# mmaker/c-lwe-snarks

Hardware: AMD Instinct MI355X
Metric: snark_proofs_per_sec (higher is better)
Workload: dtype u32 limbs (704-bit integers mod 2^704) + AES-256 bytes; int8 digits on the matrix cores, int32 accumulation (exact)

## Files before the change

### c-lwe-snarks_amd/__init__.py

```python
from __future__ import annotations

import ctypes
import os
from dataclasses import dataclass

import numpy as np

_HERE = os.path.dirname(os.path.abspath(__file__))
LIB_PATH = os.environ.get("MFHIP_LIB") or os.path.join(_HERE, "libmfhip.so")
P = 0xFFFFFFFB


class MfhError(RuntimeError):
    pass


@dataclass(frozen=True)
class Params:

    n: int = 1470
    logq: int = 736
    d: int = 1 << 15
    m: int = 21845

    @property
    def L(self):
        return (self.logq + 63) // 64

    @property
    def K(self):
        return self.logq // 64

    @property
    def lanes(self):
        return (64 * self.K + 55) // 56

    @property
    def ctb(self):
        return self.logq // 8

    @property
    def ctr_ct(self):
        return self.ctb * self.n

    @property
    def ctr_s(self):
        return 0

    @property
    def ctr_as(self):
        return self.ctr_ct * self.d

    @property
    def ctr_bt(self):
        return 2 * self.ctr_ct * self.d

    @property
    def ctr_bv(self):
        return 2 * self.ctr_ct * self.d + self.ctr_ct

    @property
    def ct_limbs(self):
        return (self.n + 1) * self.L


DEBUG = Params(d=256, m=64)
DEFAULT = Params()


class _CParams(ctypes.Structure):
    _fields_ = [("n", ctypes.c_uint32), ("logq", ctypes.c_uint32), ("d", ctypes.c_uint32), ("m", ctypes.c_uint32)]


_lib = None

EXPORTS = [
    "mfh_ctx_create", "mfh_ctx_destroy", "mfh_set_stream", "mfh_sync", "mfh_scrub_staging", "mfh_last_error", "mfh_set_seed",
    "mfh_keystream", "mfh_sample_rows", "mfh_ct_add", "mfh_ct_mul_ui", "mfh_ct_addmul_ui", "mfh_eval_rows",
    "mfh_encrypt_rows", "mfh_decrypt", "mfh_ct_smudge", "mfh_ssp_upload", "mfh_witness_poly", "mfh_version",
    "mfh_workspace_bytes", "mfh_last_kernel_ms", "mfh_set_timing", "mfh_set_overlap", "mfh_eval_rows_multi", "mfh_prove_batch", "mfh_crs_mm_image_bytes", "mfh_crs_expand_mm", "mfh_crs_set_resident_mm", "mfh_witness_poly_multi", "mfh_witness_poly_mm", "mfh_poly_h_multi", "mfh_poly_mul", "mfh_poly_add", "mfh_poly_prepare_t",
    "mfh_ssp_prepare", "mfh_poly_h", "mfh_setup_messages", "mfh_setup", "mfh_setup_image", "mfh_crs_image_set_b", "mfh_prove",
    "mfh_prove_partial", "mfh_prove_finish", "mfh_ct_to_lanes", "mfh_ct_from_lanes", "mfh_lanes_per_value", "mfh_digest128", "mfh_timing_drain", "mfh_timing_busy_ms", "mfh_timing_work_rows", "mfh_set_batch_image", "mfh_set_batch_slabs", "mfh_set_expand_path", "mfh_set_encrypt_path", "mfh_set_batch_launch", "mfh_set_batch_bw", "mfh_set_mm_chunk_rows", "mfh_set_mm_pack", "mfh_set_poly_exact", "mfh_poly_exact_fallbacks", "mfh_poly_exact_points", "mfh_set_poly_exact_points", "mfh_set_mm_stream", "mfh_add_dotp", "mfh_set_encrypt_chunks", "mfh_set_witness_per", "mfh_set_eval_path", "mfh_set_decrypt_path", "mfh_decrypt_rows",
    "mfh_crs_mm_share_bytes", "mfh_crs_expand_mm_share", "mfh_crs_set_resident_mm_share", "mfh_batch_chain", "mfh_batch_witness_cols", "mfh_batch_chain_from_w", "mfh_witness_poly_mm_cols", "mfh_prove_batch_partial", "mfh_prove_batch_finish",
    "mfh_resident_row_bytes", "mfh_crs_expand", "mfh_eval_rows_resident", "mfh_crs_set_resident",
    "mfh_witness_lanes", "mfh_witness_from_lanes", "mfh_prove_partial_w", "mfh_verify",
    "mfh_ssp_set_prg", "mfh_ssp_prg_make_t", "mfh_ssp_prg_fill",
    "mfh_resident_share_rows", "mfh_crs_expand_share", "mfh_crs_set_resident_share", "mfh_crs_set_resident_prefix",
    "mfh_prove_batch_supergroup", "mfh_prove_batch_stream_wait", "mfh_set_mm_width",
    "mfh_setup_public", "mfh_prove_public", "mfh_prove_batch_public", "mfh_vk_derive", "mfh_verify_public",
    "mfh_ssp_from_rows", "mfh_ssp_set_rows", "mfh_ssp_rows_fill", "mfh_circuit_create", "mfh_circuit_destroy", "mfh_circuit_assign",
    "mfh_circuit_create_global", "mfh_circuit_create_ex", "mfh_circuit_create_out", "mfh_circuit_create_sum",
]


def load_library():
    global _lib
    if _lib is not None:
        return _lib
    if not os.path.exists(LIB_PATH):
        raise MfhError(f"{LIB_PATH} is missing: run `python -c 'import __graft_entry__ as g; g.build()'` "
                       "(hipcc --offload-arch=gfx950).  There is no CPU fallback.")
    lib = ctypes.CDLL(LIB_PATH)
    vp, u64, sz, i32, u32 = ctypes.c_void_p, ctypes.c_uint64, ctypes.c_size_t, ctypes.c_int, ctypes.c_uint32
    sig = {
        "mfh_ctx_create": (i32, [ctypes.POINTER(vp), i32, ctypes.POINTER(_CParams)]),
        "mfh_ctx_destroy": (None, [vp]),
        "mfh_set_stream": (i32, [vp, vp]),
        "mfh_sync": (i32, [vp]),
        "mfh_scrub_staging": (i32, [vp]),
        "mfh_last_error": (ctypes.c_char_p, [vp]),
        "mfh_set_seed": (i32, [vp, ctypes.c_char_p]),
        "mfh_keystream": (i32, [vp, u64, vp, sz]),
        "mfh_sample_rows": (i32, [vp, u64, sz, vp]),
        "mfh_ct_add": (i32, [vp, vp, vp, vp, sz]),
        "mfh_ct_mul_ui": (i32, [vp, vp, vp, u32, sz]),
        "mfh_ct_addmul_ui": (i32, [vp, vp, vp, u32, sz]),
        "mfh_eval_rows": (i32, [vp, u64, sz, vp, vp, vp, vp, vp, i32]),
        "mfh_encrypt_rows": (i32, [vp, u64, sz, vp, vp, vp, vp]),
        "mfh_decrypt": (i32, [vp, vp, vp, sz, vp]),
        "mfh_ct_smudge": (i32, [vp, vp, sz, ctypes.c_char_p, sz, ctypes.c_char_p]),
        "mfh_ssp_upload": (i32, [vp, vp, vp, sz, sz]),
        "mfh_witness_poly": (i32, [vp, vp, ctypes.c_char_p, u32, vp]),
        "mfh_version": (ctypes.c_char_p, []),
        "mfh_workspace_bytes": (sz, [vp]),
        "mfh_last_kernel_ms": (ctypes.c_float, [vp, ctypes.c_char_p]),
        "mfh_set_timing": (i32, [vp, i32]),
        "mfh_set_overlap": (i32, [vp, i32]),
        "mfh_eval_rows_multi": (i32, [vp, u64, sz, vp, vp, u32, u32, vp, i32]),
        "mfh_poly_h_multi": (i32, [vp, vp, vp, u32]),
        "mfh_witness_poly_mm": (i32, [vp, vp, u32, ctypes.c_char_p, sz, vp, vp]),
        "mfh_witness_poly_multi": (i32, [vp, vp, u32, ctypes.c_char_p, sz, vp, vp]),
        "mfh_crs_mm_image_bytes": (sz, [vp]),
        "mfh_crs_expand_mm": (i32, [vp, vp, vp]),
        "mfh_crs_set_resident_mm": (i32, [vp, vp]),
        "mfh_prove_batch": (i32, [vp, vp, vp, u32, ctypes.c_char_p, sz, vp, ctypes.c_char_p, sz, ctypes.c_char_p, vp]),
        "mfh_prove_batch_supergroup": (u32, [vp]),
        "mfh_set_mm_width": (i32, [vp, u32, i32]),
        "mfh_prove_batch_stream_wait": (i32, [vp, u32, vp]),
        "mfh_poly_mul": (i32, [vp, vp, sz, vp, sz, vp]),
        "mfh_poly_add": (i32, [vp, vp, vp, sz, vp]),
        "mfh_poly_prepare_t": (i32, [vp, vp]),
        "mfh_ssp_prepare": (i32, [vp, vp]),
        "mfh_poly_h": (i32, [vp, vp, vp]),
        "mfh_setup_messages": (i32, [vp, vp, u32, u32, u32, vp]),
        "mfh_setup": (i32, [vp, vp, u32, u32, u32, vp, vp, vp]),
        "mfh_setup_image": (i32, [vp, vp, u32, u32, u32, vp, vp, vp, vp]),
        "mfh_prove": (i32, [vp, vp, vp, ctypes.c_char_p, u32, ctypes.c_char_p, sz, ctypes.c_char_p, vp]),
        "mfh_prove_partial": (i32, [vp, vp, vp, ctypes.c_char_p, u32, u32, u32, vp]),
        "mfh_prove_finish": (i32, [vp, vp, ctypes.c_char_p, sz, ctypes.c_char_p]),
        "mfh_lanes_per_value": (u32, [vp]),
        "mfh_digest128": (i32, [vp, vp, sz, vp]),
        "mfh_ct_to_lanes": (i32, [vp, vp, sz, vp]),
        "mfh_ct_from_lanes": (i32, [vp, vp, sz, vp]),
        "mfh_add_dotp": (i32, [vp, vp, vp, vp, sz]),
        "mfh_crs_set_resident_prefix": (i32, [vp, vp, sz]),
        "mfh_resident_share_rows": (sz, [vp, u32, u32]),
        "mfh_crs_expand_share": (i32, [vp, vp, u32, u32, vp]),
        "mfh_crs_set_resident_share": (i32, [vp, vp, u32, u32]),
        "mfh_ssp_set_prg": (i32, [vp, u64, vp]),
        "mfh_ssp_prg_make_t": (i32, [vp, u64, ctypes.c_char_p, vp]),
        "mfh_ssp_prg_fill": (i32, [vp, u64, sz, sz, vp]),
        "mfh_verify": (i32, [vp, vp, u32, u32, u32, vp, vp, sz, vp]),
        "mfh_witness_lanes": (i32, [vp, vp, ctypes.c_char_p, u32, u32, vp]),
        "mfh_witness_from_lanes": (i32, [vp, vp, vp, u32, vp]),
        "mfh_prove_partial_w": (i32, [vp, vp, vp, ctypes.c_char_p, u32, u32, u32, vp, vp]),
        "mfh_resident_row_bytes": (sz, [vp]),
        "mfh_crs_expand": (i32, [vp, u64, sz, vp, vp]),
        "mfh_crs_image_set_b": (i32, [vp, sz, sz, vp, vp]),
        "mfh_eval_rows_resident": (i32, [vp, vp, sz, sz, vp, vp, vp, vp, i32]),
        "mfh_crs_set_resident": (i32, [vp, vp]),
        "mfh_timing_drain": (i32, [vp, ctypes.c_char_p, ctypes.POINTER(u64), ctypes.POINTER(ctypes.c_double), ctypes.POINTER(u64),
                                   ctypes.POINTER(ctypes.c_float)]),
        "mfh_timing_busy_ms": (ctypes.c_double, [vp]),
        "mfh_timing_work_rows": (u64, [vp]),
        "mfh_set_batch_image": (i32, [vp, i32]),
        "mfh_set_mm_chunk_rows": (i32, [vp, u32]),
        "mfh_set_mm_pack": (i32, [vp, i32]),
        "mfh_set_poly_exact": (i32, [vp, i32]),
        "mfh_poly_exact_fallbacks": (ctypes.c_long, [vp]),
        "mfh_poly_exact_points": (i32, [vp, ctypes.POINTER(u32)]),
        "mfh_set_poly_exact_points": (i32, [vp, ctypes.POINTER(u32)]),
        "mfh_set_mm_stream": (i32, [vp, i32, i32, i32, u32]),
        "mfh_set_batch_launch": (i32, [vp, u32, i32]),
        "mfh_set_batch_bw": (i32, [vp, i32]),
        "mfh_set_encrypt_path": (i32, [vp, i32]),
        "mfh_set_expand_path": (i32, [vp, i32]),
        "mfh_set_batch_slabs": (i32, [vp, u32]),
        "mfh_set_encrypt_chunks": (i32, [vp, u32]),
        "mfh_set_eval_path": (i32, [vp, i32]),
        "mfh_set_decrypt_path": (i32, [vp, i32]),
        "mfh_decrypt_rows": (i32, [vp, u64, sz, vp, vp, vp]),
        "mfh_set_witness_per": (i32, [vp, u32]),
        "mfh_crs_mm_share_bytes": (sz, [vp, u32, u32]),
        "mfh_crs_expand_mm_share": (i32, [vp, vp, u32, u32, vp]),
        "mfh_crs_set_resident_mm_share": (i32, [vp, vp, u32, u32]),
        "mfh_batch_chain": (i32, [vp, vp, u32, ctypes.c_char_p, sz, vp, vp, vp, vp]),
        "mfh_batch_witness_cols": (i32, [vp, vp, u32, ctypes.c_char_p, sz, vp, u32, u32, vp, sz]),
        "mfh_batch_chain_from_w": (i32, [vp, vp, u32, vp, vp, vp]),
        "mfh_witness_poly_mm_cols": (i32, [vp, vp, u32, ctypes.c_char_p, sz, vp, u32, u32, vp, sz]),
        "mfh_prove_batch_partial": (i32, [vp, vp, u32, u32, u32, ctypes.c_char_p, sz, vp, vp, vp, sz, vp]),
        "mfh_prove_batch_finish": (i32, [vp, vp, u32, vp, ctypes.c_char_p, sz, ctypes.c_char_p, vp]),
        "mfh_setup_public": (i32, [vp, vp, u32, u32, u32, u32, vp, vp, vp, vp]),
        "mfh_prove_public": (i32, [vp, vp, vp, u32, ctypes.c_char_p, u32, ctypes.c_char_p, sz, ctypes.c_char_p, vp]),
        "mfh_prove_batch_public": (i32, [vp, vp, vp, u32, u32, ctypes.c_char_p, sz, vp, ctypes.c_char_p, sz, ctypes.c_char_p, vp]),
        "mfh_vk_derive": (i32, [vp, vp, u32, u32, vp]),
        "mfh_verify_public": (i32, [vp, vp, u32, u32, u32, vp, vp, ctypes.c_char_p, sz, sz, vp]),
        "mfh_ssp_from_rows": (i32, [vp, u32, vp, vp, vp, vp]),
        "mfh_ssp_set_rows": (i32, [vp, u32, vp, vp, vp, u32]),
        "mfh_ssp_rows_fill": (i32, [vp, sz, sz, vp]),
        "mfh_circuit_create": (i32, [vp, u32, u32, vp, u32, vp, ctypes.POINTER(vp)]),
        "mfh_circuit_create_global": (i32, [vp, u32, u32, vp, u32, vp, ctypes.POINTER(vp)]),
        "mfh_circuit_create_ex": (i32, [vp, u32, u32, vp, u32, vp, u32, vp, u32, ctypes.POINTER(vp)]),
        "mfh_circuit_create_out": (i32, [vp, u32, u32, vp, u32, vp, u32, vp, u32, vp, u32, ctypes.POINTER(vp)]),
        "mfh_circuit_create_sum": (i32, [vp, u32, u32, vp, u32, vp, u32, vp, u32, vp, u32, vp, u32, ctypes.POINTER(vp)]),
        "mfh_circuit_destroy": (None, [vp]),
        "mfh_circuit_assign": (i32, [vp, vp, u32, vp, sz, vp, sz, vp]),
    }
    for name, (res, args) in sig.items():
        fn = getattr(lib, name)
        fn.restype = res
        fn.argtypes = args
    _lib = lib
    return lib


def rows_to_csr(rows):
    if isinstance(rows, tuple) and len(rows) == 3 and all(isinstance(a, np.ndarray) for a in rows):
        row_ptr, wire, coef = rows
    else:
        lens = [len(r) for r in rows]
        row_ptr = np.zeros(len(lens) + 1, dtype=np.int64)
        np.cumsum(lens, out=row_ptr[1:])
        flat = [(int(w), int(a) % P) for r in rows for (w, a) in r]
        wire = np.array([w for w, _ in flat], dtype=np.int64)
        coef = np.array([a for _, a in flat], dtype=np.int64)
    if len(row_ptr) == 0 or min(np.min(row_ptr), np.min(wire, initial=0), np.min(coef, initial=0)) < 0:
        raise MfhError("rows: row_ptr needs nrows + 1 entries, and no entry may be negative")
    if max(np.max(row_ptr), np.max(wire, initial=0), np.max(coef, initial=0)) > 0xFFFFFFFF:
        raise MfhError("rows: entries must fit 32 bits")
    return tuple(np.ascontiguousarray(a, dtype=np.uint32) for a in (row_ptr, wire, coef))


def _ptr(t):
    return ctypes.c_void_p(t.data_ptr()) if t is not None else ctypes.c_void_p(0)


CIRCUIT_MAX_WIRES = 32767
CIRCUIT_GLOBAL = 1


class CircuitProgram:

    def __init__(self, ctx, nin, ngates, handle, state="lds", extended=False, outputs=0, sums=False):
        self._ctx, self.nin, self.ngates, self._h, self.state, self.extended, self.outputs = ctx, nin, ngates, handle, state, extended, outputs
        self.sums = sums

    def close(self):
        if self._h:
            self._ctx.lib.mfh_circuit_destroy(self._h)
            self._h = ctypes.c_void_p()

    def __del__(self):
        try:
            self.close()
        except Exception:
            pass


class Context:

    def __init__(self, params: Params = DEFAULT, device: int = 0):
        import torch

        if not torch.cuda.is_available():
            raise MfhError("no HIP device visible: the MI355X path has no CPU fallback")
        self.torch = torch
        self.lib = load_library()
        self.params = params
        self.device = torch.device("cuda", device)
        self._h = ctypes.c_void_p()
        cp = _CParams(params.n, params.logq, params.d, params.m)
        rc = self.lib.mfh_ctx_create(ctypes.byref(self._h), device, ctypes.byref(cp))
        if rc != 0:
            raise MfhError(f"mfh_ctx_create failed ({rc})")
        self._chk(self.lib.mfh_set_stream(self._h, ctypes.c_void_p(torch.cuda.current_stream(self.device).cuda_stream)))

    def close(self):
        if self._h:
            self.lib.mfh_ctx_destroy(self._h)
            self._h = ctypes.c_void_p()

    def __del__(self):
        try:
            self.close()
        except Exception:
            pass

    def _chk(self, rc):
        if rc != 0:
            raise MfhError(f"libmfhip error {rc}: {self.lib.mfh_last_error(self._h).decode()}")

    def empty(self, nbytes):
        return self.torch.empty(int(nbytes), dtype=self.torch.uint8, device=self.device)

    def zeros(self, nbytes):
        return self.torch.zeros(int(nbytes), dtype=self.torch.uint8, device=self.device)

    def to_device(self, arr):
        a = np.ascontiguousarray(arr)
        if not a.flags.writeable:
            import warnings

            with warnings.catch_warnings():
                warnings.simplefilter("ignore", UserWarning)
                return self.torch.from_numpy(a.view(np.uint8).reshape(-1)).to(self.device)
        return self.torch.from_numpy(a.view(np.uint8).reshape(-1)).to(self.device)

    def to_host(self, t, dtype=np.uint8):
        return t.cpu().numpy().view(dtype)

    def sync(self):
        self._chk(self.lib.mfh_sync(self._h))

    def set_timing(self, on=True):
        self._chk(self.lib.mfh_set_timing(self._h, 1 if on else 0))

    def set_overlap(self, mode=1):
        self._chk(self.lib.mfh_set_overlap(self._h, int(mode)))

    def set_batch_image(self, on=True):
        self._chk(self.lib.mfh_set_batch_image(self._h, 1 if on else 0))

    def set_batch_slabs(self, nslabs=0):
        self._chk(self.lib.mfh_set_batch_slabs(self._h, int(nslabs)))

    def set_expand_path(self, path=0):
        self._chk(self.lib.mfh_set_expand_path(self._h, int(path)))

    def set_encrypt_path(self, path=0):
        self._chk(self.lib.mfh_set_encrypt_path(self._h, int(path)))

    def set_eval_path(self, path=0):
        self._chk(self.lib.mfh_set_eval_path(self._h, int(path)))

    def set_encrypt_chunks(self, chunks=0):
        self._chk(self.lib.mfh_set_encrypt_chunks(self._h, int(chunks)))

    def set_witness_per(self, statements=0):
        self._chk(self.lib.mfh_set_witness_per(self._h, int(statements)))

    def set_batch_launch(self, groups_per_launch=4, merge_regions=True):
        self._chk(self.lib.mfh_set_batch_launch(self._h, int(groups_per_launch), 1 if merge_regions else 0))

    def set_batch_bw(self, merged=True):
        self._chk(self.lib.mfh_set_batch_bw(self._h, 1 if merged else 0))

    def set_mm_stream(self, map=0, persistent=False, sync_mode=0, spin_max=64):
        self._chk(self.lib.mfh_set_mm_stream(self._h, int(map), int(persistent), int(sync_mode), int(spin_max)))

    def set_mm_width(self, per_xcd=32, early_chain=False):
        self._chk(self.lib.mfh_set_mm_width(self._h, int(per_xcd), 1 if early_chain else 0))

    def set_mm_pack(self, on=True):
        self._chk(self.lib.mfh_set_mm_pack(self._h, 1 if on else 0))

    def set_poly_exact(self, mode=1):
        self._chk(self.lib.mfh_set_poly_exact(self._h, int(mode)))

    def poly_exact_fallbacks(self):
        return int(self.lib.mfh_poly_exact_fallbacks(self._h))

    def exact_points(self):
        out = (ctypes.c_uint32 * 4)()
        self._chk(self.lib.mfh_poly_exact_points(self._h, out))
        return [int(x) for x in out]

    def set_exact_points(self, pts):
        if pts is None:
            self._chk(self.lib.mfh_set_poly_exact_points(self._h, None))
            return
        pts = [int(x) for x in pts]
        if len(pts) != 4 or not all(0 <= x < 2**32 for x in pts):
            raise MfhError(f"set_exact_points: four uint32 values, got {pts!r}")
        self._chk(self.lib.mfh_set_poly_exact_points(self._h, (ctypes.c_uint32 * 4)(*pts)))

    def set_mm_chunk_rows(self, rows=0):
        self._chk(self.lib.mfh_set_mm_chunk_rows(self._h, int(rows)))

    def timing_drain(self, which):
        n, rows, ms, last = ctypes.c_uint64(), ctypes.c_uint64(), ctypes.c_double(), ctypes.c_float()
        self._chk(self.lib.mfh_timing_drain(self._h, which.encode(), ctypes.byref(n), ctypes.byref(ms), ctypes.byref(rows), ctypes.byref(last)))
        return n.value, ms.value, rows.value

    def timing_busy_ms(self):
        return float(self.lib.mfh_timing_busy_ms(self._h))

    def timing_work_rows(self):
        return int(self.lib.mfh_timing_work_rows(self._h))

    def last_kernel_ms(self, which):
        return float(self.lib.mfh_last_kernel_ms(self._h, which.encode()))

    def set_seed(self, seed: bytes):
        assert len(seed) == 40
        self._chk(self.lib.mfh_set_seed(self._h, bytes(seed)))

    def keystream(self, off, nbytes, out=None):
        out = self.empty(nbytes) if out is None else out
        self._chk(self.lib.mfh_keystream(self._h, off, _ptr(out), nbytes))
        return out

    def sample_rows(self, off, nrows):
        p = self.params
        out = self.empty(nrows * p.n * p.L * 8)
        self._chk(self.lib.mfh_sample_rows(self._h, off, nrows, _ptr(out)))
        return out

    def ct_add(self, a, b, count=1, out=None):
        out = self.empty(a.numel()) if out is None else out
        self._chk(self.lib.mfh_ct_add(self._h, _ptr(out), _ptr(a), _ptr(b), count))
        return out

    def ct_mul_ui(self, a, x, count=1, out=None):
        out = self.empty(a.numel()) if out is None else out
        self._chk(self.lib.mfh_ct_mul_ui(self._h, _ptr(out), _ptr(a), x, count))
        return out

    def ct_addmul_ui(self, rop, a, x, count=1):
        self._chk(self.lib.mfh_ct_addmul_ui(self._h, _ptr(rop), _ptr(a), x, count))
        return rop

    def eval_rows(self, off, nrows, c8, coeff0, coeff1=None, rop0=None, rop1=None, accumulate=False):
        p = self.params
        if rop0 is None:
            rop0 = self.empty(p.ct_limbs * 8)
        if coeff1 is not None and rop1 is None:
            rop1 = self.empty(p.ct_limbs * 8)
        self._chk(self.lib.mfh_eval_rows(self._h, off, nrows, _ptr(c8), _ptr(coeff0), _ptr(coeff1), _ptr(rop0), _ptr(rop1),
                                         1 if accumulate else 0))
        return rop0, rop1

    def eval_rows_multi(self, off, nrows, c8, coeffs, nvec, out=None, accumulate=False, coeff_bytes=4):
        out = self.empty(nvec * self.params.ct_limbs * 8) if out is None else out
        self._chk(self.lib.mfh_eval_rows_multi(self._h, off, nrows, _ptr(c8), _ptr(coeffs), nvec, coeff_bytes, _ptr(out), 1 if accumulate else 0))
        return out

    def encrypt_rows(self, off, nrows, sk, msg, err, out=None):
        p = self.params
        out = self.empty(nrows * p.ctb) if out is None else out
        self._chk(self.lib.mfh_encrypt_rows(self._h, off, nrows, _ptr(sk), _ptr(msg), _ptr(err), _ptr(out)))
        return out

    def decrypt(self, sk, cts, count, out=None):
        out = self.empty(4 * count) if out is None else out
        self._chk(self.lib.mfh_decrypt(self._h, _ptr(sk), _ptr(cts), count, _ptr(out)))
        return out

    def set_decrypt_path(self, path=0):
        self._chk(self.lib.mfh_set_decrypt_path(self._h, int(path)))

    def decrypt_rows(self, off, nrows, sk, c8, out=None):
        out = self.empty(4 * nrows) if out is None else out
        self._chk(self.lib.mfh_decrypt_rows(self._h, off, nrows, _ptr(sk), _ptr(c8), _ptr(out)))
        return out

    def ct_smudge(self, cts, count, mag: bytes, maglen, sign: bytes):
        self._chk(self.lib.mfh_ct_smudge(self._h, _ptr(cts), count, bytes(mag), maglen, bytes(sign)))
        return cts

    def ssp_upload(self, ssp_host_u64: np.ndarray, d_ssp=None, first_slot=0, nslots=None):
        p = self.params
        nslots = p.m + 3 if nslots is None else nslots
        if d_ssp is None:
            d_ssp = self.empty((p.m + 3) * p.d * 4)
        a = np.ascontiguousarray(ssp_host_u64)
        self._chk(self.lib.mfh_ssp_upload(self._h, ctypes.c_void_p(a.ctypes.data), _ptr(d_ssp), first_slot, nslots))
        return d_ssp

    def ssp_from_rows(self, rows, d_ssp=None):
        p = self.params
        row_ptr, wire, coef = rows_to_csr(rows)
        if d_ssp is None:
            d_ssp = self.empty((p.m + 3) * p.d * 4)
        self._chk(self.lib.mfh_ssp_from_rows(self._h, len(row_ptr) - 1, ctypes.c_void_p(row_ptr.ctypes.data), ctypes.c_void_p(wire.ctypes.data),
                                             ctypes.c_void_p(coef.ctypes.data), _ptr(d_ssp)))
        return d_ssp

    def ssp_set_rows(self, rows, lu_max=0):
        if rows is None:
            self._chk(self.lib.mfh_ssp_set_rows(self._h, 0, None, None, None, 0))
            return
        row_ptr, wire, coef = rows_to_csr(rows)
        self._chk(self.lib.mfh_ssp_set_rows(self._h, len(row_ptr) - 1, ctypes.c_void_p(row_ptr.ctypes.data), ctypes.c_void_p(wire.ctypes.data),
                                            ctypes.c_void_p(coef.ctypes.data), int(lu_max)))

    def ssp_rows_fill(self, first_slot, nslots):
        out = self.empty(max(nslots, 1) * self.params.d * 4)
        self._chk(self.lib.mfh_ssp_rows_fill(self._h, first_slot, nslots, _ptr(out)))
        return out

    def circuit_load(self, compiled, state="lds"):
        if state not in ("lds", "global", "auto"):
            raise MfhError(f"circuit_load: state must be 'lds', 'global' or 'auto', got {state!r}")
        gates = np.ascontiguousarray(compiled.gates, dtype=np.uint32).reshape(-1, 3)
        asserts = np.ascontiguousarray(compiled.asserts, dtype=np.uint32).reshape(-1, 2)
        program = np.ascontiguousarray(getattr(compiled, "program", np.zeros((0, 4))), dtype=np.uint32).reshape(-1, 4)
        equal = np.ascontiguousarray(getattr(compiled, "equal", np.zeros((0, 2))), dtype=np.uint32).reshape(-1, 2)
        outputs = np.ascontiguousarray(getattr(compiled, "outputs", np.zeros((0, 2))), dtype=np.uint32).reshape(-1, 2)
        terms = np.ascontiguousarray(getattr(compiled, "terms", np.zeros((0, 2))), dtype=np.uint32).reshape(-1, 2)
# ... 346 lines not shown
```

### c-lwe-snarks_amd/csrc/ctx.hpp

```cpp
#pragma once
#include <hip/hip_runtime.h>

#include <stdint.h>
#include <string.h>

#include <string>
#include <vector>

#include "aes_dev.hpp"
#include "mfhip.h"
#include "ssp_prg.hpp"

#define HIP_TRY(ctx, expr)                                                        \
  do {                                                                            \
    hipError_t e_ = (expr);                                                       \
    if (e_ != hipSuccess) {                                                       \
      (ctx)->err = std::string(#expr) + ": " + hipGetErrorString(e_);             \
      return MFH_EDEVICE;                                                         \
    }                                                                             \
  } while (0)

struct PolyState;
struct SspInterp;
struct SspRows;
struct RowsTree;

struct PinBuf {
  void *p = nullptr;
  size_t cap = 0;
  hipEvent_t ev = nullptr;
  bool pending = false;
  size_t used = 0;
};

struct DevBuf {
  void *p = nullptr;
  size_t cap = 0;
  template <class T> T *as() const { return static_cast<T *>(p); }
};

struct mfh_ctx {
  mfh_params P{};
  int device = 0;
  hipStream_t own_stream = nullptr;
  hipStream_t stream = nullptr;
  mf::AesKey key{};
  bool have_seed = false;
  uint32_t *d_t0 = nullptr;
  DevBuf ws;
  DevBuf ws2;
  int mm_ws_sel = 0;
  DevBuf ws3;
  std::vector<hipEvent_t> ev_cdone, ev_rdone, ev_wdone;
  std::vector<hipEvent_t> ev_round;
  std::vector<hipEvent_t> ev_sgdone;
  uint32_t last_batch_sg = 0, last_batch_n = 0;
  DevBuf wws;
  DevBuf lazy;
  uint32_t *lazy_cnt = nullptr;
  bool eval_dense = false;
  bool overlap = true;
  int overlap_mode = 1;
  hipStream_t side = nullptr, side2 = nullptr;
  hipEvent_t ev_fork = nullptr, ev_join = nullptr;
  hipEvent_t ev_chain = nullptr, ev_chain_done = nullptr;
  std::string err;
  bool timing = false;
  struct Timed {
    hipEvent_t e0, e1;
    int kind;
    uint64_t rows;
    uint64_t work;
    int sub;
  };
  std::vector<Timed> timed;
  double last_busy_ms = 0;
  uint64_t last_work_rows = 0;
  std::vector<hipEvent_t> ev_pool;
  PolyState *poly = nullptr;
  DevBuf aux;
  DevBuf d_msg;
  DevBuf d_prover;
  std::vector<uint32_t> h_cw;
  const uint8_t *mm_image = nullptr;
  uint32_t mm_rank = 0, mm_world = 1;
  uint64_t mm_off[3] = {0, 0, 0}, mm_rows[3] = {0, 0, 0};
  size_t mm_base[3] = {0, 0, 0};
  DevBuf ssp_frag;
  const uint32_t *ssp_frag_src = nullptr;
  SspInterp *interp = nullptr;
  DevBuf circ_io;
  DevBuf circ_state;
  DevBuf d_batch;
  DevBuf batch_img;
  int batch_image = 1;
  int mm_map = 1;
  bool mm_persist = true;
  bool mm_wave1 = false;
  uint32_t mm_sync_mode = 0, mm_spin = 64;
  uint32_t mm_width = 32;
  size_t early_ws_half = 0;
  bool batch_early_chain = false;
  uint32_t *mm_sync = nullptr;
  int poly_exact = 1;
  bool poly_pts_pinned = false;
  uint32_t poly_pts[4] = {0, 0, 0, 0};
  bool mm_pack = true;
  uint32_t mm_chunk_rows = 131071;
  int expand_path = 0;
  int enc_path = 0;
  uint32_t ncu = 256;
  int dec_path = 0;
  int eval_path = 0;
  uint32_t enc_chunks = 0;
  uint32_t witness_per = 0;
  uint32_t batch_slabs = 0;
  int batch_bw_merged = 1;
  int batch_merge = 1;
  uint32_t batch_ngl = 8;
  PinBuf pin_rows, pin_cw, pin_smudge;
  PinBuf pin_pub;
  DevBuf d_pub;
  PinBuf pin_wring[8];
  uint32_t pin_wnext = 0;
  hipEvent_t ev_sample = nullptr;
  DevBuf sample_tmp;
  void *uploader = nullptr;
  bool prg_on = false;
  uint64_t prg_seed = 0;
  const uint32_t *prg_t = nullptr;
  SspRows *rows = nullptr;
  RowsTree *rows_tree = nullptr;
  const uint32_t *rows_prefix = nullptr;
  uint32_t rows_lu_max = 0;
  const uint8_t *resident_rows = nullptr;
  uint64_t resident_nrows = ~0ull;
  bool resident_sharded = false;
  uint32_t res_rank = 0, res_world = 1;
};

struct Timer {
  mfh_ctx *c;
  mfh_ctx::Timed t{};
  bool on;
  Timer(mfh_ctx *c_, int kind, uint64_t rows, uint64_t work = 0, int sub = 0) : c(c_), on(c_->timing) {
    if (!on) return;
    auto get = [&]() {
      hipEvent_t e;
      if (!c->ev_pool.empty()) { e = c->ev_pool.back(); c->ev_pool.pop_back(); }
      else hipEventCreate(&e);
      return e;
    };
    t.e0 = get(); t.e1 = get(); t.kind = kind; t.rows = rows; t.work = work ? work : rows; t.sub = sub;
    hipEventRecord(t.e0, c->stream);
  }
  ~Timer() {
    if (!on) return;
    hipEventRecord(t.e1, c->stream);
    c->timed.push_back(t);
  }
};

inline void *pin_acquire(mfh_ctx *c, PinBuf &b, size_t bytes) {
  if (b.pending) { hipEventSynchronize(b.ev); b.pending = false; }
  if (bytes > b.cap) {
    if (b.p) hipHostFree(b.p);
    b.cap = (bytes + 4095) & ~(size_t)4095;
    if (hipHostMalloc(&b.p, b.cap, hipHostMallocDefault) != hipSuccess) { b.p = nullptr; b.cap = 0; c->err = "hipHostMalloc failed"; return nullptr; }
  }
  if (!b.ev) hipEventCreateWithFlags(&b.ev, hipEventDisableTiming);
  b.used = bytes;
  return b.p;
}
inline void pin_release(mfh_ctx *c, PinBuf &b) {
  hipEventRecord(b.ev, c->stream);
  b.pending = true;
}
inline void pin_scrub(PinBuf &b) {
  if (b.pending) { hipEventSynchronize(b.ev); b.pending = false; }
  if (b.p && b.used) {
    volatile unsigned char *q = (volatile unsigned char *)b.p;
    memset((void *)q, 0, b.used);
    __asm__ __volatile__("" : : "r"(b.p) : "memory");
  }
  b.used = 0;
}
inline void pin_free(PinBuf &b) {
  if (b.pending) hipEventSynchronize(b.ev);
  if (b.p) hipHostFree(b.p);
  if (b.ev) hipEventDestroy(b.ev);
  b = PinBuf();
}

enum class DevWait { stream, device };
inline void dev_free(DevBuf &b) {
  if (b.p) hipFree(b.p);
  b = DevBuf();
}
inline bool dev_alloc(DevBuf &b, size_t bytes) {
  if (hipMalloc(&b.p, bytes) != hipSuccess) {
    b = DevBuf();
    return false;
  }
  b.cap = bytes;
  return true;
}
inline int dev_reserve(mfh_ctx *c, DevBuf &b, size_t bytes, DevWait wait = DevWait::stream, size_t gran = 1) {
  if (bytes <= b.cap) return MFH_OK;
  if (b.p) {
    if (wait == DevWait::device) hipDeviceSynchronize();
    else hipStreamSynchronize(c->stream);
    dev_free(b);
  }
  if (!dev_alloc(b, (bytes + gran - 1) & ~(gran - 1))) {
    c->err = "hipMalloc(device scratch) failed";
    return MFH_ENOMEM;
  }
  return MFH_OK;
}
inline int batch_img_drop(mfh_ctx *c) {
  if (!c->batch_img.p) return MFH_OK;
  const hipError_t e = hipDeviceSynchronize();
  dev_free(c->batch_img);
  if (e != hipSuccess) {
    c->err = std::string("hipDeviceSynchronize(): ") + hipGetErrorString(e);
    return MFH_EDEVICE;
  }
  return MFH_OK;
}
inline int work_reserve(mfh_ctx *c, DevBuf &b, size_t bytes) { return dev_reserve(c, b, bytes, DevWait::stream, (size_t)1 << 20); }
inline int lazy_reserve(mfh_ctx *c, size_t bytes) {
  if (bytes + 256 <= c->lazy.cap || !bytes) return MFH_OK;
  bytes = ((bytes + 255) & ~(size_t)255) + 256;
  if (int rc = dev_reserve(c, c->lazy, bytes)) return rc;
  if (hipMemsetAsync(c->lazy.p, 0, bytes, c->stream) != hipSuccess) return MFH_EDEVICE;
  c->lazy_cnt = reinterpret_cast<uint32_t *>(c->lazy.as<uint8_t>() + bytes - 256);
  return MFH_OK;
}
inline int ws_reserve(mfh_ctx *c, size_t bytes) { return work_reserve(c, c->ws, bytes); }
inline int wws_reserve(mfh_ctx *c, size_t bytes) { return work_reserve(c, c->wws, bytes); }
inline int ws2_reserve(mfh_ctx *c, size_t bytes) { return work_reserve(c, c->ws2, bytes); }
inline int aux_reserve(mfh_ctx *c, size_t bytes) { return dev_reserve(c, c->aux, bytes); }

inline int ssp_src(mfh_ctx *c, const uint32_t *d_ssp, mf::SspSrc &src, bool rows_ok = false) {
  if (d_ssp) { src = mf::SspSrc{d_ssp, d_ssp, 0}; return MFH_OK; }
  if (c->rows_prefix) {
    if (!rows_ok) { c->err = "this entry point does not take the row SSP (mfh_ssp_set_rows): pass a dense d_ssp"; return MFH_EUNSUPPORTED; }
    src = mf::SspSrc{c->rows_prefix, c->rows_prefix, 0, c->rows_lu_max + 2};
    return MFH_OK;
  }
  if (!c->prg_on || !c->prg_t) { c->err = "d_ssp is NULL and no generator-defined SSP is registered (mfh_ssp_set_prg)"; return MFH_EINVAL; }
  src = mf::SspSrc{nullptr, c->prg_t, c->prg_seed};
  return MFH_OK;
}

void mfh_poly_destroy(mfh_ctx *c);
void ssp_interp_free(mfh_ctx *c);
void ssp_rows_free(mfh_ctx *c, bool tree);
int ssp_rows_check(mfh_ctx *c, const char *who, uint32_t nrows, const uint32_t *h_row_ptr, const uint32_t *h_wire, const uint32_t *h_coef);
int ssp_rows_tree(mfh_ctx *c, const char *who, const uint32_t *&d_t, const uint32_t *&h_w);
int ssp_rows_witness(mfh_ctx *c, uint32_t nstmt, const uint8_t *h_bits, size_t bits_stride, const uint32_t *h_delta, uint32_t *d_w, size_t w_stride);
int ssp_rows_msg_evals(mfh_ctx *c, uint32_t s, uint32_t beta, uint32_t *d_msg_evals);
inline bool ssp_is_rows(const mfh_ctx *c, const uint32_t *d_ssp) { return !d_ssp && c->rows_prefix; }
inline int ssp_rows_lu_check(mfh_ctx *c, const uint32_t *d_ssp, uint32_t lu) {
  if (ssp_is_rows(c, d_ssp) && lu > c->rows_lu_max) { c->err = "lu exceeds the lu_max the row SSP was registered with (mfh_ssp_set_rows)"; return MFH_EINVAL; }
  return MFH_OK;
}
extern "C" int mfh_witness_poly_mm(mfh_ctx *c, const uint32_t *d_ssp, uint32_t nstmt, const uint8_t *h_bits, size_t bits_stride, const uint32_t *h_delta,
                                   uint32_t *d_w);
extern "C" int mfh_witness_poly_mm_cols(mfh_ctx *c, const uint32_t *d_ssp, uint32_t nstmt, const uint8_t *h_bits, size_t bits_stride, const uint32_t *h_delta,
                                        uint32_t col0, uint32_t ncols, uint32_t *d_w, size_t w_stride);
extern "C" int mfh_poly_h_multi(mfh_ctx *c, const uint32_t *d_v, uint32_t *d_h, uint32_t nb);
int expand_mm_region(mfh_ctx *c, uint64_t off, uint32_t nrows, const uint8_t *c8, uint8_t *image);
int encrypt_rows_mm(mfh_ctx *c, uint64_t off, size_t nrows, const uint64_t *sk, const uint32_t *msg, const uint64_t *err, uint8_t *c8);
int decrypt_mm(mfh_ctx *c, const uint64_t *sk, const uint64_t *cts, size_t count, uint32_t *out);
int decrypt_rows_mm(mfh_ctx *c, uint64_t off, size_t nrows, const uint64_t *sk, const uint8_t *c8, uint32_t *out);

struct MmIo {
  const uint32_t *coef[2];
  uint32_t csplit;
  uint64_t *out[2];
  uint32_t osplit;
  uint64_t ostride;
  const uint8_t *bits;
  uint32_t bits_stride;
  int64_t *sc_zeroed;
  uint64_t cstride;
  uint32_t bits_row0;
  const uint64_t *add_ct;
  const uint32_t *add_scale;
  uint32_t sa_from1;
};
int eval_rows_multi_io(mfh_ctx *c, uint64_t off, size_t nrows, const uint8_t *d_c8, const MmIo &io, uint32_t nvec, uint32_t coeff_bytes, int accumulate);
int eval_rows_multi_io_set(mfh_ctx *c, uint64_t off, size_t nrows, const uint8_t *d_c8, const MmIo *ios, const uint32_t *nvecs, uint32_t ng,
                           uint32_t coeff_bytes);
struct MmRegion { uint64_t off; const uint8_t *c8; };
int eval_rows_multi_io_regions(mfh_ctx *c, const MmRegion *regs, uint32_t nreg, size_t nrows, const MmIo *ios, const uint32_t *nvecs, uint32_t ng,
                               uint32_t coeff_bytes, int accumulate);
bool mm_image_covers(const mfh_ctx *c, uint64_t off, size_t nrows);
struct MmsPlan {
  uint32_t ng, ngt, ND, nrows, nchunks, rpc, rpad, ntiles, mtiles;
  size_t cd_bytes, part_bytes;
  const uint8_t *img[2];
  int8_t *cd;
  int *part;
};
bool mms_plan(mfh_ctx *c, const MmRegion *regs, uint32_t nreg, size_t nrows, const MmIo *ios, const uint32_t *nvecs, uint32_t ng, uint32_t coeff_bytes,
              MmsPlan &P);
size_t mms_ws_bytes(const MmsPlan &P);
void mms_bind(MmsPlan &P, void *ws);
int mms_digits(mfh_ctx *c, const MmsPlan &P, const MmIo *ios, const uint32_t *nvecs);
int mms_stream(mfh_ctx *c, const MmsPlan &P);
int mms_finish(mfh_ctx *c, const MmsPlan &P, const MmIo *ios, const uint32_t *nvecs, int accumulate);
```

### c-lwe-snarks_amd/csrc/evalmm.hip

```cpp
#include <algorithm>
#include <cstring>

#include "ctx.hpp"

namespace {

using mf::AesKey;

constexpr int CT = 4;
constexpr int SB = 88;
constexpr int VB = 92;
constexpr int MB = CT * SB;
constexpr int MT = MB / 32;
constexpr int RT = 128;
constexpr int TSTRIDE = 384;
constexpr int BLK_PER_ROW = 24;
static_assert(MB % 32 == 0 && CT * VB + 15 <= TSTRIDE, "tile geometry");

typedef int v4i __attribute__((ext_vector_type(4)));
typedef int v16i __attribute__((ext_vector_type(16)));

__device__ __forceinline__ uint32_t coef_at(const MmIo &io, uint32_t v, uint32_t nrows, uint32_t i) {
  if (io.bits) {
    const uint32_t a = io.bits_row0 + i;
// ... 778 lines not shown
  for (uint32_t k = 0; k < nblk * nchunks; k++) {
    uint32_t grp, tg;
    mms_item(xcd, (k % nblk) * 32 + cu, ngt, ngr, map, grp, tg);
    mmstream_body_w(imgs, mtiles, KS, nrows, rows_per_chunk, cdv, part, grp, tg, k / nblk, cd_stride, part_stride);
  }
}

template <int ND, int KWM ,
          bool PK >
__device__ __forceinline__ void evalmm_finish_body(const int *__restrict__ part, const int64_t *__restrict__ sc, uint32_t nchunks, uint32_t ntiles, uint32_t N,
                                                   uint32_t nvec, uint32_t n, uint32_t nrows, uint32_t ct, uint32_t MBv, uint32_t sby, uint32_t LL,
                                                   const MmIo &io, int accumulate, const int *__restrict__ sa_part, uint32_t sa_col) {
  __shared__ uint32_t sv[KWM][3][64];
  const uint32_t vl = threadIdx.x & 63, lq = threadIdx.x >> 6;
  const uint32_t v = blockIdx.y * 64 + vl, j = blockIdx.x;
  const uint32_t tile = j / ct, jj = j % ct;
  const uint32_t KWv = sby / 4;
  if (v < nvec) {
    int64_t corr[ND];
#pragma unroll
    for (int w = 0; w < ND; w++) corr[w] = 128 * sc[ND * v + w] + 16384ll * nrows;
    if (PK) {
      const uint64_t M4 = (uint64_t)ntiles * MBv / 4;
      unsigned __int128 corrsum = 0;
#pragma unroll
      for (int w = 0; w < ND; w++) corrsum += (unsigned __int128)((uint64_t)corr[w] * 0x01010101ull) << (8 * w);
      for (uint32_t l = lq; l < KWv; l += 4) {
        const uint64_t m4 = ((uint64_t)tile * MBv + jj * sby) / 4 + l;
        __int128 U = 0, SA = 0;
        for (uint32_t ch = 0; ch < nchunks; ch++) {
          const uint64_t at = (uint64_t)ch * M4 + m4;
          if (ND == 4) {
            const uint4 r = reinterpret_cast<const uint4 *>(part)[at * (N / 4) + v], q = reinterpret_cast<const uint4 *>(sa_part)[at * (N / 4) + sa_col / 4];
            U += (__int128)(((unsigned __int128)(uint64_t)(int64_t)(int32_t)r.z << 64) | ((uint64_t)r.y << 32) | r.x);
            SA += (__int128)(((unsigned __int128)(uint64_t)(int64_t)(int32_t)q.z << 64) | ((uint64_t)q.y << 32) | q.x);
          } else {
            U += reinterpret_cast<const long long *>(part)[at * N + v];
            SA += reinterpret_cast<const long long *>(sa_part)[at * N + sa_col];
          }
        }
        const unsigned __int128 val = (unsigned __int128)(U + SA * (__int128)(ND == 4 ? 128ll * 0x01010101ll : 128ll)) + corrsum;
        sv[l][0][vl] = (uint32_t)val;
        sv[l][1][vl] = (uint32_t)(val >> 32);
        sv[l][2][vl] = (uint32_t)(val >> 64);
      }
    } else
    for (uint32_t l = lq; l < KWv; l += 4) {
      unsigned __int128 val = 0;
      int g0[4][ND], sa0[4];
#pragma unroll
      for (int k = 0; k < 4; k++) {
        const int *row = part + ((uint64_t)tile * MBv + (jj * sby + 4 * l + k)) * N;
#pragma unroll
        for (int w = 0; w < ND; w++) g0[k][w] = row[ND * v + w];
        sa0[k] = (sa_part + ((uint64_t)tile * MBv + (jj * sby + 4 * l + k)) * N)[sa_col];
      }
#pragma unroll
      for (int k = 0; k < 4; k++) {
        const uint32_t mm = jj * sby + 4 * l + k;
        int64_t g[ND], sa = sa0[k];
#pragma unroll
        for (int w = 0; w < ND; w++) g[w] = g0[k][w];
        for (uint32_t ch = 1; ch < nchunks; ch++) {
          const int *row = part + (((uint64_t)ch * ntiles + tile) * MBv + mm) * N;
#pragma unroll
          for (int w = 0; w < ND; w++) g[w] += row[ND * v + w];
          sa += (sa_part + (((uint64_t)ch * ntiles + tile) * MBv + mm) * N)[sa_col];
        }
        uint64_t t = 0;
#pragma unroll
        for (int w = 0; w < ND; w++) t += (uint64_t)(g[w] + 128 * sa + corr[w]) << (8 * w);
        val += (unsigned __int128)t << (8 * k);
      }
      sv[l][0][vl] = (uint32_t)val;
      sv[l][1][vl] = (uint32_t)(val >> 32);
      sv[l][2][vl] = (uint32_t)(val >> 64);
    }
  }
  __syncthreads();
  if (lq != 0 || v >= nvec) return;
  uint32_t *out = reinterpret_cast<uint32_t *>((v < io.osplit ? io.out[0] + (uint64_t)v * io.ostride : io.out[1] + (uint64_t)(v - io.osplit) * io.ostride) +
                                               (uint64_t)j * LL);
  const bool wide4 = (LL & 1) == 0 && (io.ostride & 1) == 0 && ((reinterpret_cast<uintptr_t>(io.out[0]) | reinterpret_cast<uintptr_t>(io.out[1])) & 15) == 0;
  uint32_t pend[4] = {0, 0, 0, 0};
  uint64_t carry = 0;
  const uint32_t *actw = io.add_ct ? reinterpret_cast<const uint32_t *>(io.add_ct + (uint64_t)j * LL) : nullptr;
  const uint64_t ax = io.add_ct ? io.add_scale[v] : 0;
  uint64_t acarry = 0;
  for (uint32_t l = 0; l < KWv; l++) {
    uint64_t word = carry + sv[l][0][vl];
    if (l >= 1) word += sv[l - 1][1][vl];
    if (l >= 2) word += sv[l - 2][2][vl];
    if (accumulate) word += out[l];
    if (actw) {
      const uint64_t t = (uint64_t)actw[l] * ax + acarry;
      word += (uint32_t)t;
      acarry = t >> 32;
    }
    carry = word >> 32;
    pend[l & 3] = (uint32_t)word;
    if (wide4 ? (l & 3) == 3 : (l & 1) == 1) {
      if (wide4) *reinterpret_cast<uint4 *>(out + (l & ~3u)) = uint4{pend[0], pend[1], pend[2], pend[3]};
      else *reinterpret_cast<uint2 *>(out + (l & ~1u)) = uint2{pend[(l & 2)], pend[(l & 2) + 1]};
    }
  }
  if (wide4) {
    if (KWv & 3) *reinterpret_cast<uint4 *>(out + (KWv & ~3u)) = uint4{pend[0], (KWv & 3) > 1 ? pend[1] : 0u, (KWv & 3) > 2 ? pend[2] : 0u, 0u};
    for (uint32_t l = (KWv + 3) & ~3u; l < 2 * LL; l += 4) *reinterpret_cast<uint4 *>(out + l) = uint4{0u, 0u, 0u, 0u};
  } else {
    if (KWv & 1) *reinterpret_cast<uint2 *>(out + (KWv & ~1u)) = uint2{pend[(KWv & 2)], 0u};
    for (uint32_t l = (KWv + 1) & ~1u; l < 2 * LL; l += 2) *reinterpret_cast<uint2 *>(out + l) = uint2{0u, 0u};
  }
}

template <int ND, int KWM, bool PK>
__global__ __launch_bounds__(256) void k_evalmm_finish(const int *__restrict__ part, const int64_t *__restrict__ sc, uint32_t nchunks, uint32_t ntiles,
                                                        uint32_t N, uint32_t nvec, uint32_t n, uint32_t nrows, uint32_t ct, uint32_t MBv, uint32_t sby,
                                                        uint32_t LL, MmIo io, int accumulate) {
  evalmm_finish_body<ND, KWM, PK>(part, sc, nchunks, ntiles, N, nvec, n, nrows, ct, MBv, sby, LL, io, accumulate, part, ND * nvec);
}
template <int ND, int KWM, bool PK>
__global__ __launch_bounds__(256) void k_evalmm_finish_groups(const int *__restrict__ part, uint64_t part_stride, uint32_t nchunks, uint32_t ntiles, uint32_t N,
                                                               uint32_t n, uint32_t nrows, uint32_t ct, uint32_t MBv, uint32_t sby, uint32_t LL, MmGroupArgs A,
                                                               int accumulate) {
  const uint32_t g = blockIdx.z, lender = A.io[g].sa_from1 ? A.io[g].sa_from1 - 1 : g;
  evalmm_finish_body<ND, KWM, PK>(part + g * part_stride, A.io[g].sc_zeroed, nchunks, ntiles, N, A.nvec[g], n, nrows, ct, MBv, sby, LL, A.io[g], accumulate,
                                  part + lender * part_stride, ND * A.nvec[lender]);
}

__global__ void k_ssp_frag(const uint32_t *__restrict__ ssp, uint32_t nrowsel, uint32_t d, uint32_t *__restrict__ frag) {
  const uint64_t gid = (uint64_t)blockIdx.x * blockDim.x + threadIdx.x;
  const uint32_t KT = d / 32;
  const uint32_t lane = gid & 63, eg = (gid >> 6) & 3;
  const uint64_t tile = gid >> 8;
  const uint32_t kt = (uint32_t)(tile % KT), K = (uint32_t)(tile / KT);
  const uint32_t KSt = (nrowsel + 31) / 32;
  if (K >= KSt) return;
  const uint32_t k = kt * 32 + (lane & 31), rb = K * 32 + 16 * (lane >> 5) + 4 * eg;
  uint32_t x[4];
#pragma unroll
  for (int e = 0; e < 4; e++) x[e] = rb + e < nrowsel ? ssp[(uint64_t)(rb + e + 2) * d + k] ^ 0x80808080u : 0u;
#pragma unroll
  for (int w = 0; w < 4; w++) {
    const uint32_t lo = __builtin_amdgcn_perm(x[1], x[0], 0x0c0c0400u + 0x00000101u * w);
    const uint32_t hi = __builtin_amdgcn_perm(x[3], x[2], 0x04000c0cu + 0x01010000u * w);
    frag[(((((uint64_t)kt * KSt + K) * 4 + w) * 64 + lane) << 2) + eg] = lo | hi;
  }
}
struct WCols {
  uint32_t kt0;
  uint32_t KS;
  uint64_t wstride;
};
template <int MT>
__global__ __launch_bounds__(256) void k_witness_mm(const v4i *__restrict__ sspfrag, const v4i *__restrict__ bitfrag, uint32_t nrowsel ,
                                                    uint32_t ksteps_per_chunk, uint32_t d, int *__restrict__ part, WCols wc) {
  const uint32_t lane = threadIdx.x & 63, wave = threadIdx.x >> 6;
  const uint32_t r32 = lane & 31, h = lane >> 5;
  const uint32_t ktl = blockIdx.x * 4 + wave, kt = wc.kt0 + ktl;
  const uint32_t k = ktl * 32 + r32;
  const uint32_t K0 = blockIdx.y * ksteps_per_chunk, K1 = min((nrowsel + 31) / 32, K0 + ksteps_per_chunk);
  v16i acc[MT][4];
#pragma unroll
  for (int t = 0; t < MT; t++)
#pragma unroll
    for (int w = 0; w < 4; w++)
#pragma unroll
      for (int e = 0; e < 16; e++) acc[t][w][e] = 0;
  if (K0 >= K1) return;
  constexpr int PF = 3;
  v4i bq[PF][4], aq[PF][MT];
  auto fetch = [&](int slot, uint32_t K) {
    K = min(K, K1 - 1);
    const v4i *src = sspfrag + (((uint64_t)kt * wc.KS + K) * 4) * 64 + lane;
#pragma unroll
    for (int w = 0; w < 4; w++) bq[slot][w] = src[64 * w];
#pragma unroll
    for (int t = 0; t < MT; t++) aq[slot][t] = bitfrag[((uint64_t)K * MT + t) * 64 + lane];
  };
#pragma unroll
  for (int i = 0; i < PF; i++) fetch(i, K0 + i);
  for (uint32_t K = K0; K < K1; K += PF) {
#pragma unroll
    for (int i = 0; i < PF; i++) {
      if (K + i < K1) {
#pragma unroll
        for (int t = 0; t < MT; t++)
#pragma unroll
          for (int w = 0; w < 4; w++) acc[t][w] = __builtin_amdgcn_mfma_i32_32x32x32_i8(aq[i][t], bq[i][w], acc[t][w], 0, 0, 0);
        fetch(i, K + i + PF);
      }
    }
  }
#pragma unroll
  for (int t = 0; t < MT; t++)
#pragma unroll
    for (int w = 0; w < 4; w++)
#pragma unroll
      for (int e = 0; e < 16; e++) {
        const uint32_t stmt = 32 * t + (e & 3) + 8 * (e >> 2) + 4 * h;
        part[(((uint64_t)blockIdx.y * 4 + w) * (32 * MT) + stmt) * d + k] = acc[t][w][e];
      }
}
__global__ void k_prg_rowkeys(uint64_t seed, uint32_t nrows_pad, uint32_t *__restrict__ rk) {
  const uint32_t r = blockIdx.x * blockDim.x + threadIdx.x;
  if (r < nrows_pad) rk[r] = mf::ssp_prg_rowkey(seed, r + 2);
}
template <int MT>
__global__ __launch_bounds__(256) void k_witness_mm_prg(const uint32_t *__restrict__ rowkeys, const v4i *__restrict__ bitfrag, uint32_t nrowsel ,
                                                        uint32_t ksteps_per_chunk, uint32_t d, int *__restrict__ part, WCols wc) {
  const uint32_t lane = threadIdx.x & 63, wave = threadIdx.x >> 6;
  const uint32_t r32 = lane & 31, h = lane >> 5;
  const uint32_t kt = blockIdx.x * 4 + wave;
  const uint32_t k = kt * 32 + r32;
  const uint32_t K0 = blockIdx.y * ksteps_per_chunk, K1 = min((nrowsel + 31) / 32, K0 + ksteps_per_chunk);
  v16i acc[MT][4];
#pragma unroll
  for (int t = 0; t < MT; t++)
#pragma unroll
    for (int w = 0; w < 4; w++)
#pragma unroll
      for (int e = 0; e < 16; e++) acc[t][w][e] = 0;
  if (K0 >= K1) return;
  const uint32_t kc = wc.kt0 * 32 + k + 0x632BE5ABu;
  constexpr int PF = 2;
  v4i aqr[PF][MT];
  uint4 rkr[PF][4];
  auto fetch = [&](uint32_t K, int slot) {
    K = min(K, K1 - 1);
#pragma unroll
    for (int t = 0; t < MT; t++) aqr[slot][t] = bitfrag[((uint64_t)K * MT + t) * 64 + lane];
    const uint4 *rk4 = reinterpret_cast<const uint4 *>(rowkeys + 32 * (uint64_t)K + 16 * h);
#pragma unroll
    for (int q = 0; q < 4; q++) rkr[slot][q] = rk4[q];
  };
  fetch(K0, 0);
  fetch(K0 + 1, 1);
  auto step = [&](uint32_t K, int slot) {
    v4i aq[MT];
#pragma unroll
    for (int t = 0; t < MT; t++) aq[t] = aqr[slot][t];
    uint32_t x[16];
#pragma unroll
    for (int q = 0; q < 4; q++) {
      const uint4 r = rkr[slot][q];
      x[4 * q] = r.x; x[4 * q + 1] = r.y; x[4 * q + 2] = r.z; x[4 * q + 3] = r.w;
    }
    fetch(K + PF, slot);
#pragma unroll
    for (int e = 0; e < 16; e++) {
      uint32_t y = kc * x[e];
      y ^= y >> 16;
      y *= 0x7FEB352Du;
      y ^= y >> 15;
      y *= 0x846CA68Bu;
      y ^= y >> 16;
      x[e] = y;
    }
    v4i bq[4];
#pragma unroll
    for (int w = 0; w < 4; w++)
#pragma unroll
      for (int j = 0; j < 4; j++) {
        const uint32_t lo = __builtin_amdgcn_perm(x[4 * j + 1], x[4 * j], 0x0c0c0400u + 0x00000101u * w);
        const uint32_t hi = __builtin_amdgcn_perm(x[4 * j + 3], x[4 * j + 2], 0x04000c0cu + 0x01010000u * w);
        bq[w][j] = (int)((lo | hi) ^ 0x80808080u);
      }
#pragma unroll
    for (int t = 0; t < MT; t++)
#pragma unroll
      for (int w = 0; w < 4; w++) acc[t][w] = __builtin_amdgcn_mfma_i32_32x32x32_i8(aq[t], bq[w], acc[t][w], 0, 0, 0);
  };
  uint32_t K = K0;
  for (; K + 2 <= K1; K += 2) {
    step(K, 0);
    step(K + 1, 1);
  }
  if (K < K1) step(K, 0);
#pragma unroll
  for (int t = 0; t < MT; t++)
#pragma unroll
    for (int w = 0; w < 4; w++)
#pragma unroll
      for (int e = 0; e < 16; e++) {
        const uint32_t stmt = 32 * t + (e & 3) + 8 * (e >> 2) + 4 * h;
        part[(((uint64_t)blockIdx.y * 4 + w) * (32 * MT) + stmt) * d + k] = acc[t][w][e];
      }
}
__global__ __launch_bounds__(512) void k_witness_mm8q_prg(const uint32_t *__restrict__ rowkeys, const v4i *__restrict__ bitfrag, uint32_t nrowsel ,
                                                          uint32_t ksteps_per_chunk, uint32_t d, int *__restrict__ part, WCols wc) {
  constexpr int MT = 8, RING = 4;
  __shared__ v4i bits[RING][MT][64];
  __shared__ uint32_t xch[3][2][4][64][4];
  const uint32_t tid = threadIdx.x, lane = tid & 63, wave = tid >> 6;
  const uint32_t r32 = lane & 31, h = lane >> 5;
  const uint32_t tile = wave >> 2, pl = wave & 3;
  const uint32_t sh = pl >> 1, pp = pl & 1;
  const uint32_t pos = (pl + (lane >> 4)) & 3;
  const uint32_t ktl = blockIdx.x * 2 + tile, kt = wc.kt0 + ktl;
  const uint32_t kc = kt * 32 + r32 + 0x632BE5ABu;
  const uint32_t K0 = blockIdx.y * ksteps_per_chunk, K1 = min((nrowsel + 31) / 32, K0 + ksteps_per_chunk);
  v16i acc[4][2];
#pragma unroll
  for (int t = 0; t < 4; t++)
#pragma unroll
    for (int q = 0; q < 2; q++)
#pragma unroll
      for (int e = 0; e < 16; e++) acc[t][q][e] = 0;
  if (K0 >= K1) return;
  auto bits_load = [&](uint32_t K) -> v4i { return bitfrag[(uint64_t)min(K, K1 - 1) * MT * 64 + tid]; };
  auto bits_store = [&](uint32_t K, v4i st) { (&bits[K % RING][0][0])[tid] = st; };
  auto rk_load = [&](uint32_t K) -> uint4 { return *reinterpret_cast<const uint4 *>(rowkeys + 32 * (uint64_t)min(K, K1 - 1) + 16 * h + 4 * pos); };
  auto hash1 = [&](uint32_t rowkey) -> uint32_t {
#ifdef WPRG_NOHASH
    return kc ^ rowkey;
#endif
    uint32_t y = kc * rowkey;
    y ^= y >> 16;
    y *= 0x7FEB352Du;
    y ^= y >> 15;
    y *= 0x846CA68Bu;
    y ^= y >> 16;
    return y;
  };
  auto publish = [&](uint32_t K, const uint32_t (&x)[4]) {
#pragma unroll
    for (int w = 0; w < 4; w++) {
      const uint32_t lo = __builtin_amdgcn_perm(x[1], x[0], 0x0c0c0400u + 0x00000101u * w);
      const uint32_t hi = __builtin_amdgcn_perm(x[3], x[2], 0x04000c0cu + 0x01010000u * w);
      xch[K % 3][tile][w][lane][pos] = (lo | hi) ^ 0x80808080u;
    }
  };
  auto fragment = [&](uint32_t K, uint32_t q) -> v4i { return *reinterpret_cast<const v4i *>(&xch[K % 3][tile][2 * pp + q][lane][0]); };
  uint4 rkr[4];
  v4i sta, stb;
  sta = bits_load(K0);
  bits_store(K0, sta);
  sta = bits_load(K0 + 1);
  stb = bits_load(K0 + 2);
  {
    const uint4 r0 = rk_load(K0), r1 = rk_load(K0 + 1);
    const uint32_t x0[4] = {hash1(r0.x), hash1(r0.y), hash1(r0.z), hash1(r0.w)};
    const uint32_t x1[4] = {hash1(r1.x), hash1(r1.y), hash1(r1.z), hash1(r1.w)};
    publish(K0, x0);
    publish(K0 + 1, x1);
  }
#pragma unroll
  for (int i = 2; i <= 5; i++) rkr[i & 3] = rk_load(K0 + i);
  __syncthreads();
  v4i bq0 = fragment(K0, 0), bq1 = fragment(K0, 1);
  uint32_t K = K0;
  auto step = [&](int slot, v4i &st) {
    const v4i bn0 = fragment(K + 1, 0), bn1 = fragment(K + 1, 1);
    const uint4 rk = rkr[(slot + 2) & 3];
    const uint32_t hr[4] = {rk.x, rk.y, rk.z, rk.w};
    uint32_t hx[4];
    bits_store(K + 1, st);
    const v4i *aq = &bits[K % RING][4 * sh][lane];
#pragma unroll
    for (int t = 0; t < 4; t++) {
      const v4i a = aq[t * 64];
#ifdef WPRG_NOMFMA
      acc[t][0][0] += a[0] ^ bq0[t];
      acc[t][1][0] += a[1] ^ bq1[t];
#else
      acc[t][0] = __builtin_amdgcn_mfma_i32_32x32x32_i8(a, bq0, acc[t][0], 0, 0, 0);
      acc[t][1] = __builtin_amdgcn_mfma_i32_32x32x32_i8(a, bq1, acc[t][1], 0, 0, 0);
#endif
      hx[t] = hash1(hr[t]);
    }
    publish(K + 2, hx);
    rkr[(slot + 2) & 3] = rk_load(K + 6);
    bq0 = bn0;
    bq1 = bn1;
    st = bits_load(K + 3);
#ifndef WPRG_NOSYNC
    __syncthreads();
#endif
    K++;
  };
  while (K + 4 <= K1) {
    step(0, sta);
    step(1, stb);
    step(2, sta);
    step(3, stb);
  }
  if (K < K1) step(0, sta);
  if (K < K1) step(1, stb);
  if (K < K1) step(2, sta);
  uint32_t dd = d;
  asm volatile("" : "+s"(dd));
#pragma unroll
  for (int q = 0; q < 2; q++) {
    int *dst = part + (((uint64_t)blockIdx.y * 4 + 2 * pp + q) * (32 * MT) + 128 * sh) * dd + ktl * 32 + r32 + (uint64_t)(4 * h) * dd;
#pragma unroll
    for (int t = 0; t < 4; t++) {
#pragma unroll
      for (int e = 0; e < 16; e++) dst[(uint64_t)((e & 3) + 8 * (e >> 2)) * dd] = acc[t][q][e];
      dst += (uint64_t)32 * dd;
    }
  }
}
__global__ __launch_bounds__(512) void k_witness_mm8q(const v4i *__restrict__ sspfrag, const v4i *__restrict__ bitfrag, uint32_t nrowsel ,
                                                      uint32_t ksteps_per_chunk, uint32_t d, int *__restrict__ part, const uint32_t *__restrict__ tpoly ,
                                                      const uint32_t *__restrict__ cnt_delta, uint32_t nstmt, uint32_t *__restrict__ w_out, WCols wc) {
  constexpr int MT = 8, RING = 4, PF = 4;
  __shared__ v4i bits[RING][MT][64];
  __shared__ uint32_t xch[2][3][16][64];
  const uint32_t tid = threadIdx.x, lane = tid & 63, wave = tid >> 6;
  const uint32_t r32 = lane & 31, h = lane >> 5;
  const uint32_t tile = wave >> 2, pl = wave & 3;
  const uint32_t ktl = blockIdx.x * 2 + tile, kt = wc.kt0 + ktl;
  const uint32_t K0 = blockIdx.y * ksteps_per_chunk, K1 = min((nrowsel + 31) / 32, K0 + ksteps_per_chunk);
  v16i acc[MT];
#pragma unroll
  for (int t = 0; t < MT; t++)
#pragma unroll
    for (int e = 0; e < 16; e++) acc[t][e] = 0;
  if (K0 >= K1) return;
  auto bits_load = [&](uint32_t K) -> v4i { return bitfrag[(uint64_t)min(K, K1 - 1) * MT * 64 + tid]; };
  auto bits_store = [&](uint32_t K, v4i st) { (&bits[K % RING][0][0])[tid] = st; };
  auto ssp_load = [&](uint32_t K) -> v4i { return sspfrag[(((uint64_t)kt * wc.KS + min(K, K1 - 1)) * 4 + pl) * 64 + lane]; };
  v4i stg[PF], bq[PF];
  {
    const v4i s0 = bits_load(K0), s1 = bits_load(K0 + 1);
    __builtin_amdgcn_sched_barrier(0);
#pragma unroll
    for (int i = 0; i < PF; i++) {
      bq[i] = ssp_load(K0 + i);
      stg[i] = bits_load(K0 + 2 + i);
      __builtin_amdgcn_sched_barrier(0);
    }
    bits_store(K0, s0);
    bits_store(K0 + 1, s1);
  }
  __syncthreads();
  v4i acur[MT];
#pragma unroll
  for (int t = 0; t < MT; t++) acur[t] = bits[K0 % RING][t][lane];
  uint32_t K = K0;
  auto step = [&](int slot) {
    bits_store(K + 2, stg[slot]);
    v4i anext[MT];
    const v4i *aq = &bits[(K + 1) % RING][0][lane];
#pragma unroll
    for (int t = 0; t < MT; t++) anext[t] = aq[t * 64];
    __builtin_amdgcn_sched_barrier(0);
#pragma unroll
    for (int t = 0; t < MT; t++) acc[t] = __builtin_amdgcn_mfma_i32_32x32x32_i8(acur[t], bq[slot], acc[t], 0, 0, 0);
    __builtin_amdgcn_sched_barrier(0);
    bq[slot] = ssp_load(K + PF);
    stg[slot] = bits_load(K + 2 + PF);
#pragma unroll
    for (int t = 0; t < MT; t++) acur[t] = anext[t];
    __syncthreads();
    K++;
  };
  while (K + PF <= K1) {
#pragma unroll
    for (int i = 0; i < PF; i++) step(i);
  }
#pragma unroll
  for (int i = 0; i + 1 < PF; i++)
    if (K < K1) step(i);
  uint32_t dd = d;
  asm volatile("" : "+s"(dd));
  if (part) {
    int *dst = part + ((uint64_t)blockIdx.y * 4 + pl) * (32 * MT) * dd + ktl * 32 + r32 + (uint64_t)(4 * h) * dd;
#pragma unroll
    for (int t = 0; t < MT; t++) {
#pragma unroll
      for (int e = 0; e < 16; e++) dst[(uint64_t)((e & 3) + 8 * (e >> 2)) * dd] = acc[t][e];
      dst += (uint64_t)32 * dd;
    }
    return;
  }
  asm volatile("" : "+s"(cnt_delta), "+s"(tpoly));
  const uint32_t k = ktl * 32 + r32;
  const uint64_t tk = tpoly[k], ws = wc.wstride, P = MFH_P;
#pragma unroll
  for (int t = 0; t < MT; t++) {
    const uint32_t owner = t >> 1;
    uint32_t mine[16];
#pragma unroll
    for (int e = 0; e < 16; e++) {
      const uint32_t b = 32 * t + (e & 3) + 8 * (e >> 2) + 4 * h;
      mine[e] = (uint32_t)acc[t][e] + (b < nstmt ? 128u * cnt_delta[2 * b] : 0u);
    }
    if (pl != owner) {
      const uint32_t sidx = pl - (pl > owner);
#pragma unroll
      for (int e = 0; e < 16; e++) xch[tile][sidx][e][lane] = mine[e];
    }
    __syncthreads();
    if (pl == owner) {
#pragma unroll
      for (int e = 0; e < 16; e++) {
        const uint32_t b = 32 * t + (e & 3) + 8 * (e >> 2) + 4 * h;
        if (b < nstmt) {
          uint64_t val = (uint64_t)mine[e] << (8 * owner);
#pragma unroll
          for (int o = 0; o < 4; o++)
            if (o != (int)owner) val += (uint64_t)xch[tile][o - (o > (int)owner)][e][lane] << (8 * o);
          w_out[(uint64_t)b * ws + k] = (uint32_t)((val % P + tk * cnt_delta[2 * b + 1] % P) % P);
        }
      }
    }
    __syncthreads();
  }
}
__global__ void k_witness_bits(const uint8_t *__restrict__ bits, size_t bits_stride, uint32_t nstmt, uint32_t nrowsel, uint32_t ksteps, uint32_t MT,
                               int8_t *__restrict__ bitfrag) {
  const uint32_t i = blockIdx.x * blockDim.x + threadIdx.x;
  if (i >= ksteps * MT * 64) return;
  const uint32_t lane = i & 63, t = (i >> 6) % MT, K = (i >> 6) / MT, stmt = 32 * t + (lane & 31), h = lane >> 5;
  const uint32_t r0 = K * 32 + 16 * h;
  uint32_t w = 0;
  if (stmt < nstmt && r0 < nrowsel) {
    const uint8_t *b = bits + (size_t)stmt * bits_stride + (r0 >> 3);
    w = b[0];
    if (r0 + 8 < nrowsel) w |= (uint32_t)b[1] << 8;
    if (nrowsel - r0 < 16) w &= (1u << (nrowsel - r0)) - 1;
  }
  uint32_t o[4];
#pragma unroll
  for (int q = 0; q < 4; q++) {
    const uint32_t n4 = (w >> (4 * q)) & 15;
    o[q] = (n4 & 1) | ((n4 & 2) << 7) | ((n4 & 4) << 14) | ((n4 & 8) << 21);
  }
  reinterpret_cast<uint4 *>(bitfrag)[i] = uint4{o[0], o[1], o[2], o[3]};
}
__global__ void k_witness_mm_finish(const int *__restrict__ part, uint32_t nchunks, const uint32_t *__restrict__ t, const uint32_t *__restrict__ cnt_delta,
                                    uint32_t nstmt, uint32_t mrows , uint32_t d, uint32_t *__restrict__ w_out, uint64_t wstride) {
  const uint32_t k = blockIdx.x * blockDim.x + threadIdx.x, b = blockIdx.y;
  if (k >= d || b >= nstmt) return;
  const uint64_t corr = 128ull * cnt_delta[2 * b];
  const uint32_t delta = cnt_delta[2 * b + 1];
  uint64_t val = 0;
#pragma unroll
  for (int w = 0; w < 4; w++) {
    int64_t g = 0;
    for (uint32_t ch = 0; ch < nchunks; ch++) g += part[(((uint64_t)ch * 4 + w) * mrows + b) * d + k];
    val += (uint64_t)(g + (int64_t)corr) << (8 * w);
  }
  const uint64_t P = MFH_P;
  w_out[(uint64_t)b * wstride + k] = (uint32_t)((val % P + (uint64_t)t[k] * delta % P) % P);
}

}

extern "C" {

struct WideGeom { uint32_t ct, sby, vby, mt, mbp, LL; };
static WideGeom wide_geom(const mfh_ctx *c) {
  if (c->P.logq == 736) return {W16<736>::CT, W16<736>::SBY, W16<736>::VBY, W16<736>::MT, W16<736>::MBP, W16<736>::LL};
  return {W16<1472>::CT, W16<1472>::SBY, W16<1472>::VBY, W16<1472>::MT, W16<1472>::MBP, W16<1472>::LL};
}

#define FINISH_LAUNCH(kern, ND_, PK_, grid, ...)                                                                         \
  do {                                                                                                                   \
    if ((PK_) && wg.sby / 4 <= 22) hipLaunchKernelGGL((kern<ND_, 22, true>), grid, dim3(256), 0, c->stream, __VA_ARGS__);  \
    else if (PK_) hipLaunchKernelGGL((kern<ND_, 46, true>), grid, dim3(256), 0, c->stream, __VA_ARGS__);                 \
    else if (wg.sby / 4 <= 22) hipLaunchKernelGGL((kern<ND_, 22, false>), grid, dim3(256), 0, c->stream, __VA_ARGS__);   \
    else hipLaunchKernelGGL((kern<ND_, 46, false>), grid, dim3(256), 0, c->stream, __VA_ARGS__);                         \
  } while (0)

int mfh_eval_rows_multi(mfh_ctx *c, uint64_t off, size_t nrows, const uint8_t *d_c8, const uint32_t *d_coeffs, uint32_t nvec, uint32_t coeff_bytes,
                        uint64_t *d_rops, int accumulate) {
  if (!c || !d_rops || !nvec || (nrows && (!d_c8 || !d_coeffs)) || (coeff_bytes != 1 && coeff_bytes != 4)) return MFH_EINVAL;
  const MmIo io = {{d_coeffs, nullptr}, nvec, {d_rops, nullptr}, nvec, (uint64_t)(c->P.n + 1) * wide_geom(c).LL, nullptr, 0, nullptr};
  return eval_rows_multi_io(c, off, nrows, d_c8, io, nvec, coeff_bytes, accumulate);
}

}

int eval_rows_multi_io(mfh_ctx *c, uint64_t off, size_t nrows, const uint8_t *d_c8, const MmIo &io, uint32_t nvec, uint32_t coeff_bytes, int accumulate) {
  if (!c || !nvec || !io.out[0] || (io.osplit < nvec && !io.out[1]) || (coeff_bytes != 1 && coeff_bytes != 4)) return MFH_EINVAL;
  if (nrows && (!d_c8 || (!io.bits && (!io.coef[0] || (io.csplit < nvec && !io.coef[1]))) || (io.bits && coeff_bytes != 1))) return MFH_EINVAL;
  const uint32_t ND = coeff_bytes;
  const uint32_t n = c->P.n;
  const bool q736 = c->P.logq == 736;
  const WideGeom wg = wide_geom(c);
  const uint8_t *img_region = nullptr;
  for (int r = 0; r < 3 && c->mm_image; r++)
    if (c->mm_off[r] == off && c->mm_rows[r] == nrows && nrows) img_region = c->mm_image + c->mm_base[r];
  const bool wide = img_region || !q736 || nvec * ND + 1 > 128;
  if (nvec * ND + 1 > 256) { c->err = "mfh_eval_rows_multi: at most 63 four-byte (255 one-byte) coefficient vectors per call (256 digit columns)"; return MFH_EINVAL; }
  if (wide && ((off & 7) || (((uint64_t)n * wg.vby) & 7))) {
    c->err = "mfh_eval_rows_multi: the 256-column kernel needs off and the row length to be multiples of 8";
    return MFH_EINVAL;
  }
  if (!c->have_seed) { c->err = "mfh_set_seed has not been called"; return MFH_EINVAL; }
  if (nrows > 0xffffffffu - 256) return MFH_EINVAL;
  HIP_TRY(c, hipSetDevice(c->device));
  const size_t ctl = (size_t)(n + 1) * wg.LL;
  if (io.ostride < ctl) return MFH_EINVAL;
  if (nrows == 0) {
    const uint32_t n0 = std::min(nvec, io.osplit);
    if (!accumulate) {
      HIP_TRY(c, hipMemset2DAsync(io.out[0], io.ostride * 8, 0, ctl * 8, n0, c->stream));
      if (n0 < nvec) HIP_TRY(c, hipMemset2DAsync(io.out[1], io.ostride * 8, 0, ctl * 8, nvec - n0, c->stream));
    }
    return MFH_OK;
  }
  const uint32_t ct = wide ? wg.ct : CT, mb = wide ? wg.mbp : CT * SB, rt = wide ? RT2 : RT;
  const uint32_t NT = wide ? NQ2 : (nvec * ND + 1 <= 64 ? 2 : 4), N = wide ? N2 : 32 * NT;
  const uint32_t ntiles = (n + 1 + ct - 1) / ct;
  uint32_t nchunks = (!wide && nrows >= 8 * rt) ? 2 : 1;
  const uint32_t lim = std::max(rt, c->mm_chunk_rows / rt * rt);
  nchunks = std::max<uint32_t>(nchunks, ((uint32_t)nrows + lim - 1) / lim);
  uint32_t rpc = ((uint32_t)nrows + nchunks - 1) / nchunks;
  rpc = (rpc + rt - 1) / rt * rt;
  nchunks = ((uint32_t)nrows + rpc - 1) / rpc;
  const uint32_t rpad = nchunks * rpc;
  const size_t cd_bytes = ((size_t)N * rpad + 255) & ~(size_t)255;
  const size_t sc_bytes = 256 * 8;
  const size_t part_bytes = (size_t)nchunks * ntiles * mb * N * 4;
  int rc = c->mm_ws_sel ? ws2_reserve(c, cd_bytes + sc_bytes + part_bytes) : ws_reserve(c, cd_bytes + sc_bytes + part_bytes);
  if (rc) return rc;
  uint8_t *wsp = (c->mm_ws_sel ? c->ws2 : c->ws).as<uint8_t>();
  int8_t *cd = (int8_t *)wsp;
  int64_t *sc = io.sc_zeroed ? io.sc_zeroed : (int64_t *)(wsp + cd_bytes);
  int *part = (int *)(wsp + cd_bytes + sc_bytes);
  if (!io.sc_zeroed) HIP_TRY(c, hipMemsetAsync(sc, 0, sc_bytes, c->stream));
  if (wide && ND == 4 && !io.bits)
    hipLaunchKernelGGL(k_mm_digits4w, dim3((rpad / 16 + DG4 - 1) / DG4), dim3(256), 0, c->stream, io, nvec, (uint32_t)nrows, rpad, cd, sc);
  else
    hipLaunchKernelGGL(k_mm_digits, dim3((rpad / 16 + DG_RG - 1) / DG_RG), dim3(N), 0, c->stream, io, nvec, ND, (uint32_t)nrows, rpad, NT, wide ? 1 : 0, cd, sc);
  AesKey keyx = c->key;
  for (int i = 56; i < 60; i++) keyx.rk[i] ^= 0x80808080u;
  const uint32_t pk = img_region && c->mm_pack ? ND : 0u;
  {
    Timer t(c, img_region ? 8 : 7, nrows);
    if (img_region) {
      const uint32_t mtiles = ntiles * wg.mt, KS = ((uint32_t)nrows + RT2 - 1) / RT2 * (RT2 / 64);
      MmsImages imgs{};
      imgs.image[0] = (const v4i *)img_region;
      hipLaunchKernelGGL(k_mmstream1, dim3(((mtiles + TPW - 1) / TPW + 7) / 8 * 8, nchunks), dim3(SW * 64), 0, c->stream, imgs,
                         mtiles, KS, (uint32_t)nrows, rpc, (const v4i *)cd, part, pk);
    } else if (wide && q736)
      hipLaunchKernelGGL((k_evalmm16<0, 736>), dim3(ntiles, nchunks), dim3(1024), 0, c->stream, keyx, c->d_t0, off, n, (uint32_t)nrows, rpc, d_c8, cd, part,
                         (uint8_t *)nullptr);
    else if (wide)
      hipLaunchKernelGGL((k_evalmm16<0, 1472>), dim3(ntiles, nchunks), dim3(1024), 0, c->stream, keyx, c->d_t0, off, n, (uint32_t)nrows, rpc, d_c8, cd, part,
                         (uint8_t *)nullptr);
    else if (NT == 2)
      hipLaunchKernelGGL(k_evalmm<2>, dim3(ntiles, nchunks), dim3(1024), 0, c->stream, keyx, c->d_t0, off, n, (uint32_t)nrows, rpc, d_c8, cd, rpad,
                         part);
    else
      hipLaunchKernelGGL(k_evalmm<4>, dim3(ntiles, nchunks), dim3(1024), 0, c->stream, keyx, c->d_t0, off, n, (uint32_t)nrows, rpc, d_c8, cd, rpad,
                         part);
  }
  HIP_TRY(c, hipGetLastError());
  const uint32_t sby = wide ? wg.sby : SB;
  const dim3 fgrid(n + 1, (nvec + 63) / 64);
  if (ND == 4)
    FINISH_LAUNCH(k_evalmm_finish, 4, pk, fgrid, part, sc, nchunks, ntiles, N, nvec, n, (uint32_t)nrows, ct, mb, sby, wg.LL, io, accumulate);
  else
    FINISH_LAUNCH(k_evalmm_finish, 1, pk, fgrid, part, sc, nchunks, ntiles, N, nvec, n, (uint32_t)nrows, ct, mb, sby, wg.LL, io, accumulate);
  HIP_TRY(c, hipGetLastError());
  return MFH_OK;
}

bool mms_plan(mfh_ctx *c, const MmRegion *regs, uint32_t nreg, size_t nrows, const MmIo *ios, const uint32_t *nvecs, uint32_t ng, uint32_t coeff_bytes,
              MmsPlan &P) {
  if (!c || !regs || !ios || !nvecs || !ng || !nreg || nreg > 2 || nreg * ng > 16) return false;
  bool ok = nreg * ng > 1 && c->have_seed && nrows && nrows <= 0xffffffffu - 256;
  for (uint32_t q = 0; q < nreg && ok; q++) {
    P.img[q] = nullptr;
    for (int r = 0; r < 3 && c->mm_image; r++)
      if (c->mm_off[r] == regs[q].off && c->mm_rows[r] == nrows) P.img[q] = c->mm_image + c->mm_base[r];
    ok = P.img[q] != nullptr;
  }
  P.ng = ng;
  P.ngt = nreg * ng;
  for (uint32_t g = 0; g < P.ngt && ok; g++) {
    ok = nvecs[g] && nvecs[g] * coeff_bytes + (ios[g].sa_from1 ? 0 : 1) <= 256 && ios[g].out[0] && ios[g].sc_zeroed && (ios[g].bits || ios[g].coef[0]);
    if (ok && ios[g].sa_from1) {
      const uint32_t l = ios[g].sa_from1 - 1;
      ok = l < P.ngt && l / ng == g / ng && !ios[l].sa_from1 && coeff_bytes == 4;
      for (uint32_t x = 0; x < P.ngt && ok; x++) ok = !ios[x].bits;
    }
  }
  if (!ok) return false;
  const WideGeom wg = wide_geom(c);
  P.ND = coeff_bytes;
  P.nrows = (uint32_t)nrows;
  P.ntiles = (c->P.n + 1 + wg.ct - 1) / wg.ct;
  P.mtiles = P.ntiles * wg.mt;
  const uint32_t lim = std::max<uint32_t>(RT2, c->mm_chunk_rows / RT2 * RT2);
  uint32_t nchunks = ((uint32_t)nrows + lim - 1) / lim;
  P.rpc = (((uint32_t)nrows + nchunks - 1) / nchunks + RT2 - 1) / RT2 * RT2;
  P.nchunks = ((uint32_t)nrows + P.rpc - 1) / P.rpc;
  P.rpad = P.nchunks * P.rpc;
  P.cd_bytes = ((size_t)N2 * P.rpad + 255) & ~(size_t)255;
  P.part_bytes = ((size_t)P.nchunks * P.ntiles * wg.mbp * N2 * 4 + 255) & ~(size_t)255;
  P.cd = nullptr;
  P.part = nullptr;
  return true;
// ... 75 lines not shown
  if (mms_group_args(P, ios, nvecs, A)) {
    uint32_t nvmax = 0;
    for (uint32_t g = 0; g < P.ngt; g++) nvmax = std::max(nvmax, nvecs[g]);
    FINISH_LAUNCH(k_evalmm_finish_groups, 4, pk, dim3(n + 1, (nvmax + 63) / 64, P.ngt), P.part, (uint64_t)(P.part_bytes / 4), P.nchunks, P.ntiles, (uint32_t)N2, n, P.nrows,
                  wg.ct, wg.mbp, wg.sby, wg.LL, A, accumulate);
    HIP_TRY(c, hipGetLastError());
    return MFH_OK;
  }
  for (uint32_t g = 0; g < P.ngt; g++) {
    const dim3 fgrid(n + 1, (nvecs[g] + 63) / 64);
    int *pg = P.part + g * (P.part_bytes / 4);
    if (P.ND == 4)
      FINISH_LAUNCH(k_evalmm_finish, 4, pk, fgrid, pg, ios[g].sc_zeroed, P.nchunks, P.ntiles, (uint32_t)N2, nvecs[g], n, P.nrows, wg.ct, wg.mbp, wg.sby, wg.LL, ios[g],
                    accumulate);
    else
      FINISH_LAUNCH(k_evalmm_finish, 1, pk, fgrid, pg, ios[g].sc_zeroed, P.nchunks, P.ntiles, (uint32_t)N2, nvecs[g], n, P.nrows, wg.ct, wg.mbp, wg.sby, wg.LL, ios[g],
                    accumulate);
  }
  HIP_TRY(c, hipGetLastError());
  return MFH_OK;
}
int eval_rows_multi_io_regions(mfh_ctx *c, const MmRegion *regs, uint32_t nreg, size_t nrows, const MmIo *ios, const uint32_t *nvecs, uint32_t ng,
                               uint32_t coeff_bytes, int accumulate) {
  if (!c || !regs || !ios || !nvecs || !ng || !nreg || nreg * ng > 16) return MFH_EINVAL;
  MmsPlan P;
  if (!mms_plan(c, regs, nreg, nrows, ios, nvecs, ng, coeff_bytes, P)) {
    for (uint32_t g = 0; g < nreg * ng; g++) {
      int rc = eval_rows_multi_io(c, regs[g / ng].off, nrows, regs[g / ng].c8, ios[g], nvecs[g], coeff_bytes, accumulate);
      if (rc) return rc;
    }
    return MFH_OK;
  }
  HIP_TRY(c, hipSetDevice(c->device));
  int rc = c->mm_ws_sel ? ws2_reserve(c, mms_ws_bytes(P)) : ws_reserve(c, mms_ws_bytes(P));
  if (rc) return rc;
  mms_bind(P, (c->mm_ws_sel ? c->ws2 : c->ws).p);
  rc = mms_digits(c, P, ios, nvecs);
  if (!rc) rc = mms_stream(c, P);
  if (!rc) rc = mms_finish(c, P, ios, nvecs, accumulate);
  return rc;
}
int eval_rows_multi_io_set(mfh_ctx *c, uint64_t off, size_t nrows, const uint8_t *d_c8, const MmIo *ios, const uint32_t *nvecs, uint32_t ng,
                           uint32_t coeff_bytes) {
  const MmRegion reg = {off, d_c8};
  return eval_rows_multi_io_regions(c, &reg, 1, nrows, ios, nvecs, ng, coeff_bytes, 0);
}
bool mm_image_covers(const mfh_ctx *c, uint64_t off, size_t nrows) {
  for (int r = 0; r < 3 && c->mm_image; r++)
    if (c->mm_off[r] == off && c->mm_rows[r] == nrows && nrows) return true;
  return false;
}

extern "C" {

static size_t mm_region_bytes(const mfh_ctx *c, uint64_t rows) {
  const WideGeom wg = wide_geom(c);
  const uint64_t mtiles = (uint64_t)((c->P.n + 1 + wg.ct - 1) / wg.ct) * wg.mt, ksteps = (rows + RT2 - 1) / RT2 * (RT2 / 64);
  return (size_t)(mtiles * ksteps * 1024);
}
struct MmShare { uint64_t row0[3], rows[3]; };
static MmShare mm_share(const mfh_ctx *c, uint32_t rank, uint32_t world) {
  const uint64_t d = c->P.d, m = c->P.m;
  const uint64_t loS = d * rank / world, cS = d * (rank + 1) / world - loS, lo = m * rank / world, cnt = m * (rank + 1) / world - lo;
  return MmShare{{loS, d + loS, 2 * d + lo}, {cS, cS, cnt}};
}
size_t mfh_crs_mm_share_bytes(const mfh_ctx *c, uint32_t rank, uint32_t world) {
  if (!c || !world || rank >= world) return 0;
  const MmShare sh = mm_share(c, rank, world);
  return mm_region_bytes(c, sh.rows[0]) + mm_region_bytes(c, sh.rows[1]) + mm_region_bytes(c, sh.rows[2]);
}
size_t mfh_crs_mm_image_bytes(const mfh_ctx *c) { return mfh_crs_mm_share_bytes(c, 0, 1); }
int mfh_crs_expand_mm_share(mfh_ctx *c, const uint8_t *d_crs_c8, uint32_t rank, uint32_t world, uint8_t *d_image) {
  if (!c || !d_crs_c8 || !d_image || !world || rank >= world) return MFH_EINVAL;
  if (!c->have_seed) { c->err = "mfh_set_seed has not been called"; return MFH_EINVAL; }
  const WideGeom wg = wide_geom(c);
  const uint32_t n = c->P.n;
  if (((uint64_t)n * wg.vby) & 7) { c->err = "mfh_crs_expand_mm: the row length must be a multiple of 8"; return MFH_EUNSUPPORTED; }
  HIP_TRY(c, hipSetDevice(c->device));
  const uint64_t ctr_ct = (uint64_t)wg.vby * n;
  const MmShare sh = mm_share(c, rank, world);
  AesKey keyx = c->key;
  for (int i = 56; i < 60; i++) keyx.rk[i] ^= 0x80808080u;
  const uint32_t ntiles = (n + 1 + wg.ct - 1) / wg.ct;
  size_t base = 0;
  for (int r = 0; r < 3; r++) {
    if (!sh.rows[r]) continue;
    const uint32_t units = (uint32_t)((sh.rows[r] + RT2 - 1) / RT2);
    const uint32_t nchunks = std::max(1u, std::min(units, 4u));
    const uint32_t rpc = (units + nchunks - 1) / nchunks * RT2;
    Timer t(c, 9, sh.rows[r]);
    const dim3 grid(ntiles, (uint32_t)((sh.rows[r] + rpc - 1) / rpc));
    const uint8_t *c8 = d_crs_c8 + (size_t)sh.row0[r] * wg.vby;
    if (c->expand_path == 0 && ((ctr_ct * sh.row0[r]) & 7) == 0) {
      int rc = expand_mm_region(c, ctr_ct * sh.row0[r], (uint32_t)sh.rows[r], c8, d_image + base);
      if (rc) return rc;
      base += mm_region_bytes(c, sh.rows[r]);
      continue;
    }
    if (c->P.logq == 736)
      hipLaunchKernelGGL((k_evalmm16<1, 736>), grid, dim3(1024), 0, c->stream, keyx, c->d_t0, ctr_ct * sh.row0[r], n, (uint32_t)sh.rows[r], rpc, c8,
                         (const int8_t *)nullptr, (int *)nullptr, d_image + base);
    else
      hipLaunchKernelGGL((k_evalmm16<1, 1472>), grid, dim3(1024), 0, c->stream, keyx, c->d_t0, ctr_ct * sh.row0[r], n, (uint32_t)sh.rows[r], rpc, c8,
                         (const int8_t *)nullptr, (int *)nullptr, d_image + base);
    base += mm_region_bytes(c, sh.rows[r]);
  }
  HIP_TRY(c, hipGetLastError());
  return MFH_OK;
}
int mfh_crs_expand_mm(mfh_ctx *c, const uint8_t *d_crs_c8, uint8_t *d_image) { return mfh_crs_expand_mm_share(c, d_crs_c8, 0, 1, d_image); }
int mfh_set_mm_stream(mfh_ctx *c, int map, int persistent, int sync_mode, uint32_t spin_max) {
  if (!c || map < 0 || map > 1 || sync_mode < 0 || sync_mode > 2 || persistent < 0 || persistent > 2) return MFH_EINVAL;
  c->mm_map = map;
  c->mm_persist = persistent != 0;
  c->mm_wave1 = persistent == 2;
  c->mm_sync_mode = (uint32_t)sync_mode;
  c->mm_spin = spin_max;
  return MFH_OK;
}
int mfh_set_mm_width(mfh_ctx *c, uint32_t per_xcd, int early_chain) {
  if (!c || per_xcd < 1 || per_xcd > 32) return MFH_EINVAL;
  c->mm_width = per_xcd;
  c->batch_early_chain = early_chain != 0;
  return MFH_OK;
}
int mfh_set_mm_pack(mfh_ctx *c, int on) {
  if (!c) return MFH_EINVAL;
  c->mm_pack = on != 0;
  return MFH_OK;
}
int mfh_set_mm_chunk_rows(mfh_ctx *c, uint32_t rows) {
  if (!c || rows > 131071) return MFH_EINVAL;
  c->mm_chunk_rows = rows ? rows : 131071;
  return MFH_OK;
}
int mfh_crs_set_resident_mm_share(mfh_ctx *c, const uint8_t *d_image, uint32_t rank, uint32_t world) {
  if (!c || !world || rank >= world) return MFH_EINVAL;
  c->mm_image = d_image;
  c->mm_rank = rank;
  c->mm_world = world;
  const uint64_t ctr_ct = (uint64_t)wide_geom(c).vby * c->P.n;
  const MmShare sh = mm_share(c, rank, world);
  size_t base = 0;
  for (int r = 0; r < 3; r++) {
    c->mm_off[r] = ctr_ct * sh.row0[r];
    c->mm_rows[r] = sh.rows[r];
    c->mm_base[r] = base;
    base += mm_region_bytes(c, sh.rows[r]);
  }
  return MFH_OK;
}
int mfh_crs_set_resident_mm(mfh_ctx *c, const uint8_t *d_image) { return mfh_crs_set_resident_mm_share(c, d_image, 0, 1); }

int mfh_witness_poly_mm_cols(mfh_ctx *c, const uint32_t *d_ssp, uint32_t nstmt, const uint8_t *h_bits, size_t bits_stride, const uint32_t *h_delta,
                             uint32_t col0, uint32_t ncols, uint32_t *d_w, size_t w_stride) {
  if (!c || !h_bits || !h_delta || !d_w || nstmt == 0 || nstmt > 256) return MFH_EINVAL;
  mf::SspSrc src;
  {
    int rc0 = ssp_src(c, d_ssp, src);
    if (rc0) return rc0;
  }
  const uint32_t MT = nstmt > 128 ? 8 : nstmt > 64 ? 4 : nstmt > 32 ? 2 : 1;
  const uint32_t d = c->P.d, m = c->P.m;
  if (d % 128 || m < 2) { c->err = "mfh_witness_poly_mm: d must be a multiple of 128"; return MFH_EUNSUPPORTED; }
  if ((uint64_t)col0 + ncols > d || w_stride < ncols) return MFH_EINVAL;
  if (ncols == 0) return MFH_OK;
  if (col0 % 128 || ncols % 128) { c->err = "mfh_witness_poly_mm_cols: the coefficient range must start and end at multiples of 128"; return MFH_EUNSUPPORTED; }
  const uint32_t nc = ncols;
  const WCols wc = {col0 / 32, (m - 1 + 31) / 32, (uint64_t)w_stride};
  const uint32_t *tpoly = src.t + col0;
  for (uint32_t b = 0; b < nstmt; b++)
    if (h_delta[b] >= MFH_P) { c->err = "delta must be < p"; return MFH_EINVAL; }
  HIP_TRY(c, hipSetDevice(c->device));
  const uint32_t nrowsel = m - 1, ksteps = (nrowsel + 31) / 32;
  const bool fused = MT == 8 && src.dense && m < 65536 && (nc >= 16384 || ksteps <= 64);
  const uint32_t nchunks = fused ? 1u : std::min(ksteps, 4u), kpc = (ksteps + nchunks - 1) / nchunks;
  const size_t sfrag_b = (size_t)ksteps * 32 * d * 4;
  if (src.dense && (c->ssp_frag_src != d_ssp || c->ssp_frag.cap < sfrag_b)) {
    if (int rc0 = dev_reserve(c, c->ssp_frag, sfrag_b)) return rc0;
    const uint64_t nthreads = (uint64_t)ksteps * (d / 32) * 256;
    hipLaunchKernelGGL(k_ssp_frag, dim3((uint32_t)((nthreads + 255) / 256)), dim3(256), 0, c->stream, d_ssp, nrowsel, d, c->ssp_frag.as<uint32_t>());
    HIP_TRY(c, hipGetLastError());
    c->ssp_frag_src = d_ssp;
  }
  const size_t packed = (size_t)nstmt * bits_stride, head_b = ((packed + 8 + 256 * 8 + 255) & ~(size_t)255);
  const size_t frag_b = (size_t)ksteps * MT * 1024, part_b = (size_t)nchunks * 4 * 32 * MT * nc * 4;
  const size_t rk_b = src.dense ? 0 : (((size_t)ksteps * 32 * 4 + 255) & ~(size_t)255);
  int rc = wws_reserve(c, head_b + frag_b + part_b + rk_b);
  if (rc) return rc;
  PinBuf &wpin = c->pin_wring[c->pin_wnext++ % 8];
  uint8_t *stage = (uint8_t *)pin_acquire(c, wpin, head_b);
  if (!stage) return MFH_ENOMEM;
  memcpy(stage, h_bits, packed);
  uint32_t *cd = (uint32_t *)(stage + packed + ((8 - packed % 8) % 8));
  for (uint32_t b = 0; b < nstmt; b++) {
    uint32_t cnt = 0;
    const uint8_t *hb = h_bits + (size_t)b * bits_stride;
    for (uint32_t r = 0; r + 8 <= nrowsel; r += 8) cnt += (uint32_t)__builtin_popcount(hb[r >> 3]);
    for (uint32_t r = nrowsel & ~7u; r < nrowsel; r++) cnt += (hb[r >> 3] >> (r & 7)) & 1;
    cd[2 * b] = cnt;
    cd[2 * b + 1] = h_delta[b];
  }
  uint8_t *dev = c->wws.as<uint8_t>();
  HIP_TRY(c, hipMemcpyAsync(dev, stage, head_b, hipMemcpyHostToDevice, c->stream));
  pin_release(c, wpin);
  const uint32_t *d_cd = (const uint32_t *)(dev + packed + ((8 - packed % 8) % 8));
  int8_t *d_frag = (int8_t *)(dev + head_b);
  int *d_part = (int *)(dev + head_b + frag_b);
  hipLaunchKernelGGL(k_witness_bits, dim3((uint32_t)((frag_b / 16 + 255) / 256)), dim3(256), 0, c->stream, dev, bits_stride, nstmt, nrowsel, ksteps, MT, d_frag);
  if (!src.dense) {
    uint32_t *d_rk = (uint32_t *)(dev + head_b + frag_b + part_b);
    const dim3 grid(nc / 128, (ksteps + kpc - 1) / kpc);
    hipLaunchKernelGGL(k_prg_rowkeys, dim3((ksteps * 32 + 255) / 256), dim3(256), 0, c->stream, src.seed, ksteps * 32, d_rk);
    if (MT == 8)
      hipLaunchKernelGGL(k_witness_mm8q_prg, dim3(nc / 64, (ksteps + kpc - 1) / kpc), dim3(512), 0, c->stream, d_rk, (const v4i *)d_frag, nrowsel, kpc, nc, d_part, wc);
    else if (MT == 1) hipLaunchKernelGGL(k_witness_mm_prg<1>, grid, dim3(256), 0, c->stream, d_rk, (const v4i *)d_frag, nrowsel, kpc, nc, d_part, wc);
    else if (MT == 2) hipLaunchKernelGGL(k_witness_mm_prg<2>, grid, dim3(256), 0, c->stream, d_rk, (const v4i *)d_frag, nrowsel, kpc, nc, d_part, wc);
    else hipLaunchKernelGGL(k_witness_mm_prg<4>, grid, dim3(256), 0, c->stream, d_rk, (const v4i *)d_frag, nrowsel, kpc, nc, d_part, wc);
  } else if (MT == 8) {
    hipLaunchKernelGGL(k_witness_mm8q, dim3(nc / 64, (ksteps + kpc - 1) / kpc), dim3(512), 0, c->stream, c->ssp_frag.as<const v4i>(), (const v4i *)d_frag, nrowsel, kpc, nc,
                       fused ? (int *)nullptr : d_part, tpoly, d_cd, nstmt, d_w, wc);
    if (fused) {
      HIP_TRY(c, hipGetLastError());
      return MFH_OK;
    }
  } else if (MT == 1)
    hipLaunchKernelGGL(k_witness_mm<1>, dim3(nc / 128, (ksteps + kpc - 1) / kpc), dim3(256), 0, c->stream, c->ssp_frag.as<const v4i>(), (const v4i *)d_frag,
                       nrowsel, kpc, nc, d_part, wc);
  else if (MT == 2)
    hipLaunchKernelGGL(k_witness_mm<2>, dim3(nc / 128, (ksteps + kpc - 1) / kpc), dim3(256), 0, c->stream, c->ssp_frag.as<const v4i>(), (const v4i *)d_frag,
                       nrowsel, kpc, nc, d_part, wc);
  else
    hipLaunchKernelGGL(k_witness_mm<4>, dim3(nc / 128, (ksteps + kpc - 1) / kpc), dim3(256), 0, c->stream, c->ssp_frag.as<const v4i>(), (const v4i *)d_frag,
                       nrowsel, kpc, nc, d_part, wc);
  hipLaunchKernelGGL(k_witness_mm_finish, dim3((nc + 255) / 256, nstmt), dim3(256), 0, c->stream, d_part, (ksteps + kpc - 1) / kpc, tpoly, d_cd, nstmt, 32 * MT,
                     nc, d_w, (uint64_t)w_stride);
  HIP_TRY(c, hipGetLastError());
  return MFH_OK;
}

int mfh_witness_poly_mm(mfh_ctx *c, const uint32_t *d_ssp, uint32_t nstmt, const uint8_t *h_bits, size_t bits_stride, const uint32_t *h_delta,
                        uint32_t *d_w) {
  if (!c) return MFH_EINVAL;
  if (ssp_is_rows(c, d_ssp)) {
    if (!h_bits || !h_delta || !d_w || nstmt == 0 || nstmt > 256) return MFH_EINVAL;
    return ssp_rows_witness(c, nstmt, h_bits, bits_stride, h_delta, d_w, c->P.d);
  }
  return mfh_witness_poly_mm_cols(c, d_ssp, nstmt, h_bits, bits_stride, h_delta, 0, c->P.d, d_w, c->P.d);
}

}
```

### c-lwe-snarks_amd/csrc/mfhip.hip

```cpp
#include <hip/hip_runtime.h>

#include <stdint.h>
#include <stdio.h>
#include <string.h>

#include <algorithm>
#include <string>
#include <thread>
#include <vector>

#include "aes_dev.hpp"
#include "mfhip.h"

using mf::AesKey;

template <int LOGQ>
struct PS {
  static constexpr int CTB = LOGQ / 8;
  static constexpr int EW = CTB / 4;
  static constexpr int L = (LOGQ + 63) / 64;
  static constexpr int K = LOGQ / 64;
  static constexpr int KW = 2 * K;
  static constexpr int TILE = LOGQ == 736 ? 512 : 256;
  static constexpr int ROWS = 2;
// ... 924 lines not shown
  uint64_t s = 0;
  for (uint32_t g = 0; g < G; g++) s = (s + partial[(uint64_t)g * d + k] % MFH_P) % MFH_P;
  lanes[k] = s;
}

extern "C" {

const char *mfh_version(void) { return "mfhip 0.1 (gfx950)"; }

int mfh_ctx_create(mfh_ctx **out, int device, const mfh_params *P) {
  if (!out || !P) return MFH_EINVAL;
  *out = nullptr;
  if (P->logq != 736 && P->logq != 1472) return MFH_EUNSUPPORTED;
  if (P->n == 0 || P->n > (1u << 20)) return MFH_EINVAL;
  int ndev = 0;
  if (hipGetDeviceCount(&ndev) != hipSuccess || ndev <= 0 || device < 0 || device >= ndev) return MFH_EDEVICE;
  if (hipSetDevice(device) != hipSuccess) return MFH_EDEVICE;
  mfh_ctx *c = new mfh_ctx();
  c->P = *P;
  c->device = device;
  {
    int ncu = 0;
    if (hipDeviceGetAttribute(&ncu, hipDeviceAttributeMultiprocessorCount, device) == hipSuccess && ncu > 0) c->ncu = (uint32_t)ncu;
  }
  if (hipStreamCreateWithFlags(&c->own_stream, hipStreamNonBlocking) != hipSuccess) {
    delete c;
    return MFH_EDEVICE;
  }
  c->stream = c->own_stream;
  uint32_t t0[512];
  mf::make_t0_le(t0);
  for (int a = 0; a < 256; a++) t0[256 + a] = (t0[a] << 24) | (t0[a] >> 8);
  if (hipMalloc(&c->d_t0, sizeof t0) != hipSuccess || hipMemcpy(c->d_t0, t0, sizeof t0, hipMemcpyHostToDevice) != hipSuccess) {
    mfh_ctx_destroy(c);
    return MFH_EDEVICE;
  }
  *out = c;
  return MFH_OK;
}

void mfh_ctx_destroy(mfh_ctx *c) {
  if (!c) return;
  hipSetDevice(c->device);
  if (c->stream) hipStreamSynchronize(c->stream);
  mfh_poly_destroy(c);
  ssp_interp_free(c);
  ssp_rows_free(c, true);
  upload_free(c);
  if (c->ev_sample) hipEventDestroy(c->ev_sample);
  pin_free(c->pin_rows);
  for (auto &b : c->pin_wring) pin_free(b);
  pin_free(c->pin_cw);
  pin_free(c->pin_smudge);
  pin_free(c->pin_pub);
  if (c->side) hipStreamSynchronize(c->side);
  if (c->mm_sync) hipFree(c->mm_sync);
  for (hipEvent_t e : c->ev_round) hipEventDestroy(e);
  for (hipEvent_t e : c->ev_sgdone) hipEventDestroy(e);
  for (hipEvent_t e : c->ev_cdone) hipEventDestroy(e);
  for (hipEvent_t e : c->ev_rdone) hipEventDestroy(e);
  for (hipEvent_t e : c->ev_wdone) hipEventDestroy(e);
  if (c->ev_fork) hipEventDestroy(c->ev_fork);
  if (c->ev_join) hipEventDestroy(c->ev_join);
  if (c->ev_chain) hipEventDestroy(c->ev_chain);
  if (c->ev_chain_done) hipEventDestroy(c->ev_chain_done);
  if (c->side) hipStreamDestroy(c->side);
  if (c->side2) hipStreamDestroy(c->side2);
  for (DevBuf *b : {&c->ws, &c->ws2, &c->ws3, &c->wws, &c->lazy, &c->aux, &c->d_msg, &c->d_prover, &c->d_pub, &c->d_batch, &c->batch_img, &c->circ_io,
                    &c->circ_state, &c->ssp_frag, &c->sample_tmp})
    dev_free(*b);
  if (c->d_t0) hipFree(c->d_t0);
  for (auto &t : c->timed) { hipEventDestroy(t.e0); hipEventDestroy(t.e1); }
  for (auto e : c->ev_pool) hipEventDestroy(e);
  if (c->own_stream) hipStreamDestroy(c->own_stream);
  delete c;
}

int mfh_set_stream(mfh_ctx *c, void *s) {
  if (!c) return MFH_EINVAL;
  c->stream = (hipStream_t)s;
  return MFH_OK;
}

int mfh_sync(mfh_ctx *c) {
  if (!c) return MFH_EINVAL;
  HIP_TRY(c, hipStreamSynchronize(c->stream));
  return MFH_OK;
}

int mfh_scrub_staging(mfh_ctx *c) {
  if (!c) return MFH_EINVAL;
  pin_scrub(c->pin_rows);
  pin_scrub(c->pin_cw);
  pin_scrub(c->pin_smudge);
  for (auto &b : c->pin_wring) pin_scrub(b);
  return MFH_OK;
}

const char *mfh_last_error(const mfh_ctx *c) { return c ? c->err.c_str() : "null context"; }
size_t mfh_workspace_bytes(const mfh_ctx *c) { return c ? c->ws.cap : 0; }
int mfh_set_overlap(mfh_ctx *c, int en) {
  if (!c) return MFH_EINVAL;
  c->overlap = en != 0;
  c->overlap_mode = en > 1 ? en : 1;
  return MFH_OK;
}

int mfh_set_expand_path(mfh_ctx *c, int path) {
  if (!c || path < 0 || path > 1) return MFH_EINVAL;
  c->expand_path = path;
  return MFH_OK;
}

int mfh_set_encrypt_path(mfh_ctx *c, int path) {
  if (!c || path < 0 || path > 2) return MFH_EINVAL;
  c->enc_path = path;
  return MFH_OK;
}

int mfh_set_eval_path(mfh_ctx *c, int path) {
  if (!c || path < 0 || path > 1) return MFH_EINVAL;
  c->eval_path = path;
  return MFH_OK;
}
int mfh_set_encrypt_chunks(mfh_ctx *c, uint32_t chunks) {
  if (!c || chunks > 64) return MFH_EINVAL;
  c->enc_chunks = chunks;
  return MFH_OK;
}
int mfh_set_witness_per(mfh_ctx *c, uint32_t statements) {
  if (!c || (statements && (statements < 32 || statements > 256))) return MFH_EINVAL;
  c->witness_per = statements;
  return MFH_OK;
}
int mfh_set_batch_slabs(mfh_ctx *c, uint32_t nslabs) {
  if (!c || nslabs > 256) return MFH_EINVAL;
  c->batch_slabs = nslabs;
  return MFH_OK;
}

int mfh_set_batch_launch(mfh_ctx *c, uint32_t groups_per_launch, int merge_regions) {
  if (!c || groups_per_launch < 1 || groups_per_launch > 8) return MFH_EINVAL;
  c->batch_ngl = groups_per_launch;
  c->batch_merge = merge_regions != 0;
  return MFH_OK;
}

int mfh_set_batch_bw(mfh_ctx *c, int merged) {
  if (!c) return MFH_EINVAL;
  c->batch_bw_merged = merged != 0;
  return MFH_OK;
}

int mfh_set_batch_image(mfh_ctx *c, int en) {
  if (!c) return MFH_EINVAL;
  c->batch_image = en != 0;
  return en ? MFH_OK : batch_img_drop(c);
}

int mfh_set_timing(mfh_ctx *c, int en) {
  if (!c) return MFH_EINVAL;
  c->timing = en != 0;
  return MFH_OK;
}
static int timing_kind(const char *which) {
  if (!strcmp(which, "keystream")) return 0;
  if (!strcmp(which, "eval1")) return 1;
  if (!strcmp(which, "eval2")) return 2;
  if (!strcmp(which, "encrypt")) return 3;
  if (!strcmp(which, "eval")) return 12;
  if (!strcmp(which, "expand")) return 4;
  if (!strcmp(which, "mac1")) return 5;
  if (!strcmp(which, "mac2")) return 6;
  if (!strcmp(which, "evalmm")) return 7;
  if (!strcmp(which, "evalmm_resident")) return 8;
  if (!strcmp(which, "expandmm")) return 9;
  if (!strcmp(which, "decrypt")) return 11;
  if (!strcmp(which, "decrypt_rows")) return 13;
  if (!strcmp(which, "mmstream_bw")) return 14;
  if (!strcmp(which, "mmstream_rounds")) return 10;
  if (!strcmp(which, "mmstream_rounds_persistent")) return 110;
  if (!strcmp(which, "mmstream_bw_persistent")) return 114;
  if (!strcmp(which, "ssp_interp")) return 15;
  if (!strcmp(which, "circuit_assign")) return 16;
  if (!strcmp(which, "circuit_assign_global")) return 17;
  if (!strcmp(which, "circuit_assign_ex")) return 18;
  if (!strcmp(which, "circuit_assign_global_ex")) return 19;
  if (!strcmp(which, "circuit_assign_out")) return 20;
  if (!strcmp(which, "circuit_assign_global_out")) return 21;
  if (!strcmp(which, "circuit_assign_sum")) return 22;
  if (!strcmp(which, "circuit_assign_global_sum")) return 23;
  return -1;
}

int mfh_timing_drain(mfh_ctx *c, const char *which, uint64_t *count, double *total_ms, uint64_t *total_rows, float *last_ms) {
  if (!c || !which) return MFH_EINVAL;
  const int kind = timing_kind(which);
  if (kind < 0) return MFH_EINVAL;
  HIP_TRY(c, hipStreamSynchronize(c->stream));
  if (c->side) HIP_TRY(c, hipStreamSynchronize(c->side));
  uint64_t n = 0, rows = 0, work = 0;
  double tot = 0;
  float last = -1.f;
  std::vector<mfh_ctx::Timed> keep;
  std::vector<std::pair<float, float>> spans;
  hipEvent_t base = nullptr;
  for (auto &t : c->timed) {
    const bool match = t.kind == kind || (kind == 12 && (t.kind == 1 || t.kind == 2)) || (kind == 8 && (t.kind == 10 || t.kind == 14)) || (kind >= 100 && t.kind == kind - 100 && t.sub == 1);
    if (!match) { keep.push_back(t); continue; }
    float ms = 0;
    if (hipEventElapsedTime(&ms, t.e0, t.e1) == hipSuccess) {
      n++; tot += ms; rows += t.rows; work += t.work; last = ms;
      if (!base) base = t.e0;
      float s0 = 0;
      if (hipEventElapsedTime(&s0, base, t.e0) == hipSuccess) spans.emplace_back(s0, s0 + ms);
    }
  }
  std::sort(spans.begin(), spans.end());
  double busy = 0;
  float hi = -1e30f;
  for (auto &sp : spans) {
    if (sp.second <= hi) continue;
    busy += sp.second - std::max(sp.first, hi);
    hi = sp.second;
  }
  c->last_busy_ms = busy;
  c->last_work_rows = work;
  for (auto &t : c->timed) {
    const bool match = t.kind == kind || (kind == 12 && (t.kind == 1 || t.kind == 2)) || (kind == 8 && (t.kind == 10 || t.kind == 14)) || (kind >= 100 && t.kind == kind - 100 && t.sub == 1);
    if (!match) continue;
    c->ev_pool.push_back(t.e0);
    c->ev_pool.push_back(t.e1);
  }
  c->timed.swap(keep);
  if (count) *count = n;
  if (total_ms) *total_ms = tot;
  if (total_rows) *total_rows = rows;
  if (last_ms) *last_ms = last;
  return MFH_OK;
}

double mfh_timing_busy_ms(const mfh_ctx *c) { return c ? c->last_busy_ms : -1.0; }
uint64_t mfh_timing_work_rows(const mfh_ctx *c) { return c ? c->last_work_rows : 0; }

float mfh_last_kernel_ms(mfh_ctx *c, const char *which) {
  float last = -1.f;
  if (mfh_timing_drain(c, which, nullptr, nullptr, nullptr, &last) != MFH_OK) return -1.f;
  return last;
}

int mfh_set_seed(mfh_ctx *c, const uint8_t seed[40]) {
  if (!c || !seed) return MFH_EINVAL;
  mf::expand_key(c->key, seed);
  c->have_seed = true;
  return MFH_OK;
}

#define NEED_SEED(c)                                  \
  do {                                                \
    if (!(c)->have_seed) {                            \
      (c)->err = "mfh_set_seed has not been called";  \
      return MFH_EINVAL;                              \
    }                                                 \
  } while (0)

#define DISPATCH_LOGQ(c, CALL736, CALL1472) \
  do {                                      \
    if ((c)->P.logq == 736) {               \
      CALL736;                              \
    } else {                                \
      CALL1472;                             \
    }                                       \
  } while (0)

int mfh_digest128(mfh_ctx *c, const void *d_buf, size_t nbytes, uint64_t h_digest[2]) {
  if (!c || (!d_buf && nbytes) || !h_digest || (reinterpret_cast<uintptr_t>(d_buf) & 3)) return MFH_EINVAL;
  HIP_TRY(c, hipSetDevice(c->device));
  int rc = aux_reserve(c, 16);
  if (rc) return rc;
  HIP_TRY(c, hipMemsetAsync(c->aux.p, 0, 16, c->stream));
  const uint64_t nwords = (nbytes + 3) / 4;
  const uint32_t grid = (uint32_t)std::min<uint64_t>(2048, (nwords + 255) / 256);
  if (grid) hipLaunchKernelGGL(k_digest128, dim3(grid), dim3(256), 0, c->stream, (const uint8_t *)d_buf, (uint64_t)nbytes, c->aux.as<unsigned long long>());
  HIP_TRY(c, hipGetLastError());
  HIP_TRY(c, hipMemcpyAsync(h_digest, c->aux.p, 16, hipMemcpyDeviceToHost, c->stream));
  HIP_TRY(c, hipStreamSynchronize(c->stream));
  return MFH_OK;
}

int mfh_keystream(mfh_ctx *c, uint64_t off, void *d_out, size_t nbytes) {
  if (!c || (!d_out && nbytes)) return MFH_EINVAL;
  NEED_SEED(c);
  if (!nbytes) return MFH_OK;
  HIP_TRY(c, hipSetDevice(c->device));
  uint64_t nblk = ((off & 15) + nbytes + 15) >> 4;
  uint32_t grid = (uint32_t)std::min<uint64_t>((nblk + 1023) / 1024, 256 * 2);
  {
    Timer t(c, 0, nblk);
    hipLaunchKernelGGL(k_keystream, dim3(grid), dim3(1024), 0, c->stream, c->key, c->d_t0, off, (uint8_t *)d_out, (uint64_t)nbytes);
  }
  HIP_TRY(c, hipGetLastError());
  return MFH_OK;
}

int mfh_sample_rows(mfh_ctx *c, uint64_t off, size_t nrows, uint64_t *d_out) {
  if (!c || (!d_out && nrows)) return MFH_EINVAL;
// ... 665 lines not shown
```

### c-lwe-snarks_amd/csrc/snark.hip

```cpp
#include <algorithm>
#include <cstdlib>
#include <cstring>
#include <vector>

#include "ctx.hpp"
#include "p32.hpp"

namespace {

__device__ __forceinline__ uint32_t ssp_coef(const mf::SspSrc &src, uint32_t slot, uint32_t rowkey, uint32_t d, uint32_t k) {
  if (src.dense) return src.dense[(uint64_t)slot * d + k];
  return slot == 0 ? src.t[k] : mf::ssp_prg_coeff(rowkey, k);
}

__global__ void k_powers(uint32_t s, uint32_t d, uint32_t *__restrict__ pw) {
  uint32_t k = blockIdx.x * blockDim.x + threadIdx.x;
  if (k >= d) return;
  uint32_t r = 1, b = s, e = k;
  while (e) {
    if (e & 1) r = mulp(r, b);
    b = mulp(b, b);
    e >>= 1;
  }
  pw[k] = r;
// ... 385 lines not shown
  pin_release(c, c->pin_cw);
  const uint64_t ctr_ct = (uint64_t)ctb * n;
  uint32_t lo, cnt;
  share(m, lo, cnt);
  const void *res = c->resident_rows;
  if (res && c->resident_sharded && (c->res_rank != rank || c->res_world != world)) {
    c->err = "the resident CRS image holds the shares of a different (rank, world)";
    return MFH_EINVAL;
  }
  auto eval_region = [&](size_t abs_row, size_t img_row, uint32_t cnt, const uint32_t *c0, const uint32_t *c1, uint64_t *r0, uint64_t *r1) -> int {
    size_t nres = 0;
    if (res) nres = c->resident_sharded ? cnt : (abs_row >= c->resident_nrows ? 0 : std::min<uint64_t>(cnt, c->resident_nrows - abs_row));
    int rc2 = MFH_OK;
    if (nres) rc2 = mfh_eval_rows_resident(c, res, c->resident_sharded ? img_row : abs_row, nres, c0, c1, r0, r1, 0);
    if (rc2 || nres == cnt) return rc2;
    return mfh_eval_rows(c, ctr_ct * (abs_row + nres), cnt - nres, d_crs_c8 + (abs_row + nres) * ctb, c0 + nres, c1 ? c1 + nres : nullptr, r0, r1,
                         nres ? 1 : 0);
  };
  uint32_t loS, cS;
  share(d, loS, cS);
  auto run_bw = [&]() -> int { return eval_region((size_t)2 * d + lo, (size_t)2 * cS, cnt, cw + lo, nullptr, pi_b_w, nullptr); };
  auto run_chain = [&]() -> int {
    StreamSwap on_side(c, fork ? c->side : main_stream);
    int r = d_wlanes ? mfh_witness_from_lanes(c, d_ssp, d_wlanes, delta, w) : mfh_witness_poly(c, d_ssp, h_witness_bits, delta, w);
    if (r) return r;
    if (lu) {
      const uint32_t ub = (lu + 7) / 8;
      uint8_t *st = (uint8_t *)pin_acquire(c, c->pin_pub, ub);
      if (!st) return MFH_ENOMEM;
      memcpy(st, h_stmt, ub);
      HIP_TRY(c, hipMemcpyAsync(ubits, st, ub, hipMemcpyHostToDevice, c->stream));
      pin_release(c, c->pin_pub);
      hipLaunchKernelGGL(k_add_public<1>, g1(d), dim3(256), 0, c->stream, w, src, d, lu, ubits, ub, 1u, nullptr, v);
    } else {
      hipLaunchKernelGGL(k_add_slot, g1(d), dim3(256), 0, c->stream, w, src, 1u, d, v);
    }
    HIP_TRY(c, hipGetLastError());
    r = mfh_poly_h(c, v, h);
    if (r) return r;
    if (fork) HIP_TRY(c, hipEventRecord(c->ev_join, c->side));
    return MFH_OK;
  };
  const bool bw_first = c->overlap_mode == 2 || (c->overlap_mode == 1 && !res && (uint64_t)cnt * 2 >= m);
  if (bw_first) {
    rc = run_bw();
    if (!rc) rc = run_chain();
  } else {
    rc = run_chain();
    if (!rc) rc = run_bw();
  }
  if (rc) return rc;
  if (fork) HIP_TRY(c, hipStreamWaitEvent(main_stream, c->ev_join, 0));
  c->eval_dense = true;
  rc = eval_region(loS, 0, cS, w + loS, h + loS, pi_v_w, pi_h);
  if (!rc) rc = eval_region((size_t)d + loS, cS, cS, v + loS, h + loS, pi_hat_v, pi_hat_h);
  c->eval_dense = false;
  return rc;
}

int mfh_prove_partial(mfh_ctx *c, const uint8_t *d_crs_c8, const uint32_t *d_ssp, const uint8_t *h_witness_bits, uint32_t delta,
                      uint32_t rank, uint32_t world, uint64_t *d_partial) {
  return prove_partial_impl(c, d_crs_c8, d_ssp, h_witness_bits, delta, rank, world, nullptr, d_partial);
}

int mfh_prove_partial_w(mfh_ctx *c, const uint8_t *d_crs_c8, const uint32_t *d_ssp, const uint8_t *h_witness_bits, uint32_t delta,
                        uint32_t rank, uint32_t world, const uint64_t *d_wlanes, uint64_t *d_partial) {
  if (!d_wlanes) return MFH_EINVAL;
  return prove_partial_impl(c, d_crs_c8, d_ssp, h_witness_bits, delta, rank, world, d_wlanes, d_partial);
}

int mfh_prove_finish(mfh_ctx *c, uint64_t *d_proof, const uint8_t *h_smudge_mag, size_t maglen, const uint8_t *h_smudge_sign) {
  if (!c || !d_proof || !h_smudge_mag || !h_smudge_sign) return MFH_EINVAL;
  const size_t ctl = (size_t)(c->P.n + 1) * ((c->P.logq + 63) / 64);
  int rc = mfh_ct_smudge(c, d_proof, 4, h_smudge_mag, maglen, h_smudge_sign);
  if (rc) return rc;
  return mfh_ct_smudge(c, d_proof + 3 * ctl, 1, h_smudge_mag + 4 * maglen, maglen, h_smudge_sign + 4);
}

int mfh_prove_public(mfh_ctx *c, const uint8_t *d_crs_c8, const uint32_t *d_ssp, uint32_t lu, const uint8_t *h_bits, uint32_t delta,
                     const uint8_t *h_smudge_mag, size_t maglen, const uint8_t *h_smudge_sign, uint64_t *d_proof) {
  if (!c || !h_smudge_mag || !h_smudge_sign) return MFH_EINVAL;
  if (lu >= c->P.m) { c->err = "lu must be < m (the m - 1 wires of the SSP)"; return MFH_EINVAL; }
  int rc = prove_partial_impl(c, d_crs_c8, d_ssp, h_bits, delta, 0, 1, nullptr, d_proof, lu);
  if (rc) return rc;
  return mfh_prove_finish(c, d_proof, h_smudge_mag, maglen, h_smudge_sign);
}

int mfh_prove(mfh_ctx *c, const uint8_t *d_crs_c8, const uint32_t *d_ssp, const uint8_t *h_witness_bits, uint32_t delta,
              const uint8_t *h_smudge_mag, size_t maglen, const uint8_t *h_smudge_sign, uint64_t *d_proof) {
  if (!h_smudge_mag || !h_smudge_sign) return MFH_EINVAL;
  int rc = mfh_prove_partial(c, d_crs_c8, d_ssp, h_witness_bits, delta, 0, 1, d_proof);
  if (rc) return rc;
  return mfh_prove_finish(c, d_proof, h_smudge_mag, maglen, h_smudge_sign);
}

}

namespace {

constexpr uint32_t BG = 31;
constexpr uint32_t BSG = 255;
constexpr uint32_t BSG_REGEN = 248;

struct OnStream {
  mfh_ctx *c;
  hipStream_t keep;
  OnStream(mfh_ctx *c_, hipStream_t s) : c(c_), keep(c_->stream) { c->stream = s; }
  ~OnStream() { c->stream = keep; }
};
struct OnSide {
  mfh_ctx *c;
  hipStream_t keep;
  OnSide(mfh_ctx *c_, hipStream_t s) : c(c_), keep(c_->stream) { c->stream = s; c->mm_ws_sel = 1; }
  ~OnSide() { c->stream = keep; c->mm_ws_sel = 0; }
};

struct BatchScratch {
  uint32_t *WHV;
  uint8_t *CW;
  size_t cw_stride, cw_delta_off;
  uint32_t *SMU;
  uint8_t *SMS;
  uint32_t *ONE;
  uint64_t *CT_T;
  int64_t *SCZ;
  size_t nslots;
};
int batch_scratch(mfh_ctx *c, uint32_t nproofs, uint32_t whv , BatchScratch &B, uint32_t ncw = 1,
                  uint32_t nsmudge = 0 ) {
  const uint32_t d = c->P.d, m = c->P.m, n = c->P.n;
  const size_t ctl = (size_t)(n + 1) * ((c->P.logq + 63) / 64);
  const size_t nsg = ((size_t)nproofs + BSG_REGEN - 1) / BSG_REGEN;
  B.nslots = nsg * (2 + 2 * ((BSG + BG - 1) / BG));
  const size_t whv_b = (size_t)whv * 3 * BSG * d * 4;
  const size_t packed = ((size_t)BSG * ((m + 6) / 8) + 3) & ~(size_t)3;
  const size_t cw_b = packed + (size_t)BSG * 4;
  const size_t cw_pad = (cw_b + 255) & ~(size_t)255;
  const size_t KW = 2 * (c->P.logq / 64);
  const size_t sm_b = ((size_t)nsmudge * 5 * (KW * 4 + 1) + 255) & ~(size_t)255;
  const size_t need = whv_b + cw_pad * ncw + sm_b + 256 + ctl * 8 + B.nslots * 2048;
  if (int rc = dev_reserve(c, c->d_batch, need, DevWait::device)) return rc;
  uint8_t *base = c->d_batch.as<uint8_t>();
  B.WHV = (uint32_t *)base;
  B.CW = base + whv_b;
  B.cw_stride = cw_pad;
  B.cw_delta_off = packed;
  B.SMU = (uint32_t *)(base + whv_b + cw_pad * ncw);
  B.SMS = (uint8_t *)B.SMU + (size_t)nsmudge * 5 * KW * 4;
  B.ONE = (uint32_t *)(base + whv_b + cw_pad * ncw + sm_b);
  B.CT_T = (uint64_t *)(base + whv_b + cw_pad * ncw + sm_b + 256);
  B.SCZ = (int64_t *)(base + whv_b + cw_pad * ncw + sm_b + 256 + ctl * 8);
  return MFH_OK;
}
int batch_stage_host(mfh_ctx *c, const BatchScratch &B, uint32_t nproofs, const uint8_t *h_bits, size_t bits_stride, const uint32_t *h_delta,
                     const uint8_t *h_mag, size_t maglen, const uint8_t *h_sign, uint32_t SG) {
  const uint32_t m = c->P.m, nsg = (nproofs + SG - 1) / SG;
  const uint32_t bstride = (m + 6) / 8, KW = 2 * (c->P.logq / 64);
  if (maglen + 4 > (size_t)KW * 4) { c->err = "smudge magnitude too wide"; return MFH_EINVAL; }
  const size_t total = (size_t)((uint8_t *)B.SMS - B.CW) + (size_t)nproofs * 5;
  uint8_t *st = (uint8_t *)pin_acquire(c, c->pin_cw, total);
  if (!st) return MFH_ENOMEM;
  for (uint32_t g = 0; g < nsg; g++) {
    const uint32_t s0 = g * SG, sg = std::min(SG, nproofs - s0);
    uint8_t *a = st + (size_t)g * B.cw_stride;
    for (uint32_t b = 0; b < sg; b++) memcpy(a + (size_t)b * bstride, h_bits + (size_t)(s0 + b) * bits_stride, bstride);
    memcpy(a + B.cw_delta_off, h_delta + s0, (size_t)sg * 4);
  }
  uint32_t *up = (uint32_t *)(st + ((uint8_t *)B.SMU - B.CW));
  for (size_t i = 0; i < (size_t)nproofs * 5; i++) {
    uint64_t carry = 0;
    for (uint32_t l = 0; l < KW; l++) {
      uint32_t w = 0;
      const size_t o = (size_t)l * 4;
      if (o < maglen) memcpy(&w, h_mag + i * maglen + o, std::min<size_t>(4, maglen - o));
      const uint64_t t = (uint64_t)w * P32 + carry;
      up[i * KW + l] = (uint32_t)t;
      carry = t >> 32;
    }
  }
  memcpy(st + ((uint8_t *)B.SMS - B.CW), h_sign, (size_t)nproofs * 5);
  HIP_TRY(c, hipMemcpyAsync(B.CW, st, total, hipMemcpyHostToDevice, c->stream));
  pin_release(c, c->pin_cw);
  return MFH_OK;
}
__global__ void k_smudge_batch(uint64_t *cts, uint32_t n, uint32_t L, uint32_t KW, const uint32_t *__restrict__ up, const uint8_t *__restrict__ sign,
                               uint32_t count, uint32_t per, uint32_t slot0, uint32_t uslot0) {
  const uint32_t i = blockIdx.x * blockDim.x + threadIdx.x;
  if (i >= count) return;
  const uint32_t pb = i / per, j = i % per;
  uint32_t *b = reinterpret_cast<uint32_t *>(cts + ((uint64_t)(pb * 5 + slot0 + j) * (n + 1) + n) * L);
  const uint32_t *u = up + (uint64_t)(pb * 5 + uslot0 + j) * KW;
  if (sign[pb * 5 + uslot0 + j] & 1) {
    uint32_t borrow = 0;
    for (uint32_t l = 0; l < KW; l++) {
      const uint64_t t = (uint64_t)b[l] - u[l] - borrow;
      b[l] = (uint32_t)t;
      borrow = (uint32_t)(t >> 63);
    }
  } else {
    uint32_t carry = 0;
    for (uint32_t l = 0; l < KW; l++) {
      const uint64_t t = (uint64_t)b[l] + u[l] + carry;
      b[l] = (uint32_t)t;
      carry = (uint32_t)(t >> 32);
    }
  }
  for (uint32_t l = KW; l < 2 * L; l++) b[l] = 0;
}
int batch_smudge_staged(mfh_ctx *c, const BatchScratch &B, uint64_t *sproofs, uint32_t s0, uint32_t sg) {
  const uint32_t L = (c->P.logq + 63) / 64, KW = 2 * (c->P.logq / 64);
  const uint32_t *up = B.SMU + (size_t)s0 * 5 * KW;
  const uint8_t *sn = B.SMS + (size_t)s0 * 5;
  hipLaunchKernelGGL(k_smudge_batch, dim3((sg * 4 + 63) / 64), dim3(64), 0, c->stream, sproofs, c->P.n, L, KW, up, sn, sg * 4, 4u, 0u, 0u);
  hipLaunchKernelGGL(k_smudge_batch, dim3((sg + 63) / 64), dim3(64), 0, c->stream, sproofs, c->P.n, L, KW, up, sn, sg, 1u, 3u, 4u);
  HIP_TRY(c, hipGetLastError());
  return MFH_OK;
}
int batch_streams(mfh_ctx *c) {
  if (!c->side) {
    HIP_TRY(c, hipStreamCreateWithFlags(&c->side, hipStreamNonBlocking));
    HIP_TRY(c, hipEventCreateWithFlags(&c->ev_fork, hipEventDisableTiming));
    HIP_TRY(c, hipEventCreateWithFlags(&c->ev_join, hipEventDisableTiming));
  }
  if (!c->ev_chain) {
    HIP_TRY(c, hipStreamCreateWithFlags(&c->side2, hipStreamNonBlocking));
    HIP_TRY(c, hipEventCreateWithFlags(&c->ev_chain, hipEventDisableTiming));
    HIP_TRY(c, hipEventCreateWithFlags(&c->ev_chain_done, hipEventDisableTiming));
  }
  return MFH_OK;
}

constexpr uint32_t kPubDirect = 64;
constexpr int kPubNB = 16;
struct PubBatch {
  uint32_t lu;
  const uint8_t *d_ubits;
  uint32_t ub;
  const uint8_t *h_pub;
  size_t pub_stride;
  const uint32_t *h_zero;
  PubBatch at(uint32_t s0) const {
    PubBatch p = *this;
    p.d_ubits += (size_t)s0 * ub;
    if (h_pub) p.h_pub += (size_t)s0 * pub_stride;
    if (h_zero) p.h_zero += s0;
    return p;
  }
};

int batch_chain_launch(mfh_ctx *c, const mf::SspSrc &src, const uint32_t *d_ssp, uint32_t sg, const uint8_t *h_bits, size_t bits_stride,
                       const uint32_t *h_delta, uint32_t *W, uint32_t *H, uint32_t *V, hipEvent_t ev_witness = nullptr, const PubBatch *pub = nullptr) {
  const uint32_t d = c->P.d;
  int rc = MFH_OK;
  auto witness_pass = [&](const uint8_t *bits, size_t stride, const uint32_t *delta, uint32_t *out) -> int {
    if (d % 128 == 0) {
      const uint32_t per = c->witness_per ? c->witness_per : 256u;
      for (uint32_t b0 = 0; b0 < sg; b0 += per) {
        int r = mfh_witness_poly_mm(c, d_ssp, std::min(per, sg - b0), bits + (size_t)b0 * stride, stride, delta + b0, out + (size_t)b0 * d);
        if (r) return r;
      }
    } else {
      for (uint32_t b0 = 0; b0 < sg; b0 += 12) {
        int r = mfh_witness_poly_multi(c, d_ssp, std::min(12u, sg - b0), bits + (size_t)b0 * stride, stride, delta + b0, out + (size_t)b0 * d);
        if (r) return r;
      }
    }
    return MFH_OK;
  };
  rc = witness_pass(h_bits, bits_stride, h_delta, W);
  if (rc) return rc;
  const bool pub_pass = pub && pub->lu > kPubDirect;
  if (pub_pass) {
    rc = witness_pass(pub->h_pub, pub->pub_stride, pub->h_zero, H);
    if (rc) return rc;
  }
  if (ev_witness) HIP_TRY(c, hipEventRecord(ev_witness, c->stream));
  if (pub)
    hipLaunchKernelGGL(k_add_public<kPubNB>, dim3((d + 255) / 256, (sg + kPubNB - 1) / kPubNB), dim3(256), 0, c->stream, W, src, d, pub_pass ? 0u : pub->lu,
                       pub->d_ubits, pub->ub, sg, pub_pass ? H : nullptr, V);
  else
    hipLaunchKernelGGL(k_add_slot_multi, dim3((d + 255) / 256, sg), dim3(256), 0, c->stream, W, src, 1u, d, V);
  HIP_TRY(c, hipGetLastError());
  return mfh_poly_h_multi(c, V, H, sg);
}

struct BatchCoef {
  const uint32_t *w, *h, *v;
  uint64_t stride;
};

int batch_bw(mfh_ctx *c, const uint8_t *d_crs_c8, uint32_t rank, uint32_t world, uint32_t sg, const uint8_t *d_cw, bool has_delta, uint64_t *sproofs,
             const BatchScratch &B, size_t &slot, int accumulate) {
  const uint32_t d = c->P.d, m = c->P.m, n = c->P.n;
  const uint32_t ctb = c->P.logq / 8;
  const size_t ctl = (size_t)(n + 1) * ((c->P.logq + 63) / 64);
  const uint64_t ctr_ct = (uint64_t)ctb * n;
  const uint64_t pstride = 5 * ctl;
  const uint32_t lo = (uint32_t)((uint64_t)m * rank / world), cnt = (uint32_t)((uint64_t)m * (rank + 1) / world) - lo;
  const uint32_t bstride = (m + 6) / 8;
  MmIo io_bw = {{nullptr, nullptr}, sg, {sproofs + 4 * ctl, nullptr}, sg, pstride, d_cw, bstride, B.SCZ + 256 * slot++};
  io_bw.bits_row0 = lo;
  if (has_delta) {
    io_bw.add_ct = B.CT_T;
    io_bw.add_scale = (const uint32_t *)(d_cw + B.cw_delta_off);
  }
  return eval_rows_multi_io(c, ctr_ct * ((uint64_t)2 * d + lo), cnt, d_crs_c8 + ((size_t)2 * d + lo) * ctb, io_bw, sg, 1, accumulate);
}
int batch_rows_supergroup(mfh_ctx *c, const uint8_t *d_crs_c8, uint32_t rank, uint32_t world, uint32_t sg, const uint8_t *h_bits,
                          size_t bits_stride, const BatchCoef &co, uint64_t *sproofs, const BatchScratch &B, size_t &slot,
                          const uint32_t *h_delta, hipEvent_t wait_ev, int accumulate = 0, const uint8_t *d_cw = nullptr, bool bw_done = false,
                          uint32_t ws_slot = 0 , bool *tail_on_side = nullptr ) {
  const uint32_t d = c->P.d, m = c->P.m, n = c->P.n;
  const uint32_t ctb = c->P.logq / 8;
  const size_t ctl = (size_t)(n + 1) * ((c->P.logq + 63) / 64);
  const uint64_t ctr_ct = (uint64_t)ctb * n;
  const uint64_t pstride = 5 * ctl;
  hipStream_t const main_stream = c->stream, side_stream = c->side;
  const uint32_t loS = (uint32_t)((uint64_t)d * rank / world), cS = (uint32_t)((uint64_t)d * (rank + 1) / world) - loS;
  int rc = MFH_OK;
  if (!bw_done) {
    if (!d_cw) {
      const uint32_t bstride = (m + 6) / 8;
      const size_t staged = B.cw_delta_off + (h_delta ? (size_t)sg * 4 : 0);
      uint8_t *h_cw = (uint8_t *)pin_acquire(c, c->pin_cw, staged);
      if (!h_cw) return MFH_ENOMEM;
      for (uint32_t b = 0; b < sg; b++) memcpy(h_cw + (size_t)b * bstride, h_bits + (size_t)b * bits_stride, bstride);
      if (h_delta) memcpy(h_cw + B.cw_delta_off, h_delta, (size_t)sg * 4);
      HIP_TRY(c, hipMemcpyAsync(B.CW, h_cw, staged, hipMemcpyHostToDevice, c->stream));
      pin_release(c, c->pin_cw);
      d_cw = B.CW;
    }
    rc = batch_bw(c, d_crs_c8, rank, world, sg, d_cw, h_delta != nullptr, sproofs, B, slot, accumulate);
    if (rc) return rc;
  }
  if (wait_ev) HIP_TRY(c, hipStreamWaitEvent(main_stream, wait_ev, 0));
  HIP_TRY(c, hipEventRecord(c->ev_fork, main_stream));
  HIP_TRY(c, hipStreamWaitEvent(side_stream, c->ev_fork, 0));
  constexpr uint32_t NGLMAX = 8;
  const uint32_t NGL = c->mm_image ? c->batch_ngl : 1u;
  const MmRegion regs[2] = {{ctr_ct * loS, d_crs_c8 + (size_t)loS * ctb}, {ctr_ct * ((uint64_t)d + loS), d_crs_c8 + ((size_t)d + loS) * ctb}};
  const bool merged = mm_image_covers(c, regs[0].off, cS) && mm_image_covers(c, regs[1].off, cS) && c->batch_merge;
  if (merged) {
    constexpr uint32_t RMAX = (2 * BSG + 62) / 63;
    MmIo io[RMAX][2 * NGLMAX];
    uint32_t nv[RMAX][2 * NGLMAX];
    MmsPlan plan[RMAX];
    uint32_t R = 0;
    size_t ws_need = 0;
    const uint32_t nvtot = 2 * sg;
    auto run_io = [&](int region, uint32_t p, uint32_t cnt, uint32_t lender1) -> MmIo {
      const uint32_t x0 = std::min(p, sg), x1 = std::min(p + cnt, sg), y0 = std::max(p, sg) - sg;
      const uint32_t *X = region == 0 ? co.w : co.h, *Y = region == 0 ? co.h : co.v;
      uint64_t *OX = sproofs + (region == 0 ? 3 : 1) * ctl, *OY = sproofs + (region == 0 ? 0 : 2) * ctl;
      MmIo m = MmIo{{X + (uint64_t)x0 * co.stride, Y + (uint64_t)y0 * co.stride}, x1 - x0, {OX + (uint64_t)x0 * pstride, OY + (uint64_t)y0 * pstride}, x1 - x0, pstride,
                    nullptr, 0, B.SCZ + 256 * slot++, co.stride, 0};
      m.sa_from1 = lender1;
      return m;
    };
    for (uint32_t p0 = 0; p0 < nvtot; R++) {
      uint32_t cnt[NGLMAX], pos[NGLMAX], ng = 0, p = p0;
      for (; ng < NGL && p < nvtot; ng++) {
        pos[ng] = p;
        cnt[ng] = std::min(ng == 0 ? 63u : 64u, nvtot - p);
        p += cnt[ng];
      }
      for (uint32_t k = 0; k < ng; k++) {
        io[R][k] = run_io(0, pos[k], cnt[k], k ? 1 : 0);
        io[R][ng + k] = run_io(1, pos[k], cnt[k], k ? ng + 1 : 0);
        nv[R][k] = nv[R][ng + k] = cnt[k];
      }
      p0 = p;
      if (!mms_plan(c, regs, 2, cS, io[R], nv[R], ng, 4, plan[R])) { c->err = "mfh_prove_batch: the registered image does not serve the S / AS regions"; return MFH_EINVAL; }
      ws_need += (mms_ws_bytes(plan[R]) + 255) & ~(size_t)255;
    }
    const bool early = c->batch_early_chain && tail_on_side;
    if (early && (ws_slot == 0 || c->early_ws_half < ws_need)) {
      if (ws_slot != 0) { c->err = "early chain: a later super-group needs more scratch than the call's first"; return MFH_EINVAL; }
      c->early_ws_half = ws_need;
    }
    rc = work_reserve(c, c->ws3, early ? 2 * c->early_ws_half : ws_need);
    if (rc) return rc;
    size_t wo = early ? (size_t)(ws_slot & 1) * c->early_ws_half : 0;
    for (uint32_t r = 0; r < R; r++) {
      mms_bind(plan[r], c->ws3.as<uint8_t>() + wo);
      wo += (mms_ws_bytes(plan[r]) + 255) & ~(size_t)255;
      rc = mms_digits(c, plan[r], io[r], nv[r]);
      if (rc) return rc;
    }
    for (uint32_t r = 0; r < R; r++) {
      rc = mms_stream(c, plan[r]);
      if (rc) return rc;
      if (early) {
        while (c->ev_round.size() <= r) {
          hipEvent_t e;
          HIP_TRY(c, hipEventCreateWithFlags(&e, hipEventDisableTiming));
          c->ev_round.push_back(e);
        }
        HIP_TRY(c, hipEventRecord(c->ev_round[r], main_stream));
        HIP_TRY(c, hipStreamWaitEvent(side_stream, c->ev_round[r], 0));
        OnStream side(c, side_stream);
        rc = mms_finish(c, plan[r], io[r], nv[r], accumulate);
        if (rc) return rc;
        continue;
      }
      rc = mms_finish(c, plan[r], io[r], nv[r], accumulate);
      if (rc) return rc;
    }
    if (early) {
      *tail_on_side = true;
      return MFH_OK;
    }
  } else {
    for (uint32_t g0 = 0; g0 < sg; g0 += NGL * BG) {
      MmIo io[2 * NGLMAX];
      uint32_t nv[2 * NGLMAX], ng = 0;
      for (uint32_t k = 0; k < NGL && g0 + k * BG < sg; k++) ng++;
      for (uint32_t k = 0; k < ng; k++) {
        const uint32_t gg = g0 + k * BG, g = std::min(BG, sg - gg);
        uint64_t *proofs = sproofs + (size_t)gg * 5 * ctl;
        const uint64_t o = (uint64_t)gg * co.stride;
        io[k] = MmIo{{co.w + o, co.h + o}, g, {proofs + 3 * ctl, proofs}, g, pstride, nullptr, 0, B.SCZ + 256 * slot++, co.stride, 0};
        io[ng + k] = MmIo{{co.h + o, co.v + o}, g, {proofs + ctl, proofs + 2 * ctl}, g, pstride, nullptr, 0, B.SCZ + 256 * slot++, co.stride, 0};
        nv[k] = nv[ng + k] = 2 * g;
      }
      rc = eval_rows_multi_io_regions(c, regs, 1, cS, io, nv, ng, 4, accumulate);
      if (rc) return rc;
      {
        OnSide side(c, side_stream);
        rc = eval_rows_multi_io_regions(c, regs + 1, 1, cS, io + ng, nv + ng, ng, 4, accumulate);
        if (rc) return rc;
      }
    }
  }
  HIP_TRY(c, hipEventRecord(c->ev_join, side_stream));
  HIP_TRY(c, hipStreamWaitEvent(main_stream, c->ev_join, 0));
  return MFH_OK;
}

int batch_smudge(mfh_ctx *c, uint64_t *sproofs, uint32_t sg, const uint8_t *h_smudge_mag, size_t maglen, const uint8_t *h_smudge_sign) {
  std::vector<uint8_t> mags((size_t)sg * 5 * maglen), signs((size_t)sg * 5);
  for (int pass = 0; pass < 2; pass++) {
    std::fill(mags.begin(), mags.end(), 0);
    std::fill(signs.begin(), signs.end(), 0);
    for (uint32_t b = 0; b < sg; b++) {
      const uint8_t *pm = h_smudge_mag + (size_t)b * 5 * maglen, *ps = h_smudge_sign + (size_t)b * 5;
      if (pass == 0) {
        memcpy(&mags[(size_t)b * 5 * maglen], pm, 4 * maglen);
        memcpy(&signs[(size_t)b * 5], ps, 4);
      } else {
        memcpy(&mags[((size_t)b * 5 + 3) * maglen], pm + 4 * maglen, maglen);
        signs[(size_t)b * 5 + 3] = ps[4];
      }
    }
    int rc = mfh_ct_smudge(c, sproofs, (size_t)sg * 5, mags.data(), maglen, signs.data());
    if (rc) return rc;
  }
  return MFH_OK;
}

int batch_ct_t(mfh_ctx *c, const uint8_t *d_crs_c8, const BatchScratch &B) {
  const uint32_t d = c->P.d, ctb = c->P.logq / 8;
  HIP_TRY(c, hipMemsetD32Async((hipDeviceptr_t)B.ONE, 1, 1, c->stream));
  return mfh_eval_rows(c, (uint64_t)ctb * c->P.n * 2 * d, 1, d_crs_c8 + (size_t)2 * d * ctb, B.ONE, nullptr, B.CT_T, nullptr, 0);
}

struct ImageGuard {
  mfh_ctx *c;
  bool on;
  ~ImageGuard() { if (on) mfh_crs_set_resident_mm(c, nullptr); }
};
int batch_transient_image(mfh_ctx *c, const uint8_t *d_crs_c8, uint32_t nproofs, uint32_t rank, uint32_t world, ImageGuard &guard) {
  const uint32_t ctb = c->P.logq / 8;
  if (c->mm_image || !c->batch_image || nproofs <= BG || (((uint64_t)c->P.n * ctb) & 7)) return MFH_OK;
  const size_t ib = mfh_crs_mm_share_bytes(c, rank, world);
  if (c->batch_img.cap < ib) {
    (void)batch_img_drop(c);
    size_t mem_free = 0, mem_total = 0;
    if (hipMemGetInfo(&mem_free, &mem_total) != hipSuccess) mem_free = 0;
    if (ib > mem_free / 4 * 3 || !dev_alloc(c->batch_img, ib)) (void)hipGetLastError();
  }
  if (!c->batch_img.p) return MFH_OK;
  int rc = mfh_crs_expand_mm_share(c, d_crs_c8, rank, world, c->batch_img.as<uint8_t>());
  if (rc) return rc;
  mfh_crs_set_resident_mm_share(c, c->batch_img.as<uint8_t>(), rank, world);
  guard.on = true;
  return MFH_OK;
}

int prove_batch_impl(mfh_ctx *c, const uint8_t *d_crs_c8, const uint32_t *d_ssp, uint32_t nproofs, const uint8_t *h_witness_bits,
                     size_t bits_stride, const uint32_t *h_delta, const uint8_t *h_smudge_mag, size_t maglen, const uint8_t *h_smudge_sign,
                     uint64_t *d_proofs, const PubBatch *pub) {
  if (!c) return MFH_EINVAL;
  if (!nproofs) return MFH_OK;
  if (!d_crs_c8 || !h_witness_bits || !h_delta || !h_smudge_mag || !h_smudge_sign || !d_proofs) return MFH_EINVAL;
  if (c->resident_rows) { c->err = "mfh_prove_batch regenerates the keystream: clear the resident CRS image first"; return MFH_EUNSUPPORTED; }
  if (c->mm_image && c->mm_world != 1) { c->err = "mfh_prove_batch: the registered matrix-core image holds one rank's row shares (use mfh_prove_batch_partial)"; return MFH_EINVAL; }
  mf::SspSrc src;
  {
    int rc0 = ssp_src(c, d_ssp, src, true);
    if (rc0) return rc0;
    if (pub && (rc0 = ssp_rows_lu_check(c, d_ssp, pub->lu))) return rc0;
  }
  const uint32_t d = c->P.d, m = c->P.m, n = c->P.n;
  if (bits_stride < (m + 6) / 8) { c->err = "bits_stride shorter than the m - 1 witness bits"; return MFH_EINVAL; }
  for (uint32_t b = 0; b < nproofs; b++)
    if (h_delta[b] >= P32) { c->err = "delta must be < p"; return MFH_EINVAL; }
  if (maglen + 4 > (size_t)(c->P.logq / 64) * 8) { c->err = "smudge magnitude too wide"; return MFH_EINVAL; }
  const size_t ctl = (size_t)(n + 1) * ((c->P.logq + 63) / 64);
  HIP_TRY(c, hipSetDevice(c->device));
  const bool will_stream = c->mm_image || (c->batch_image && nproofs > BG && (((uint64_t)n * (c->P.logq / 8)) & 7) == 0);
  const uint32_t SG = will_stream ? BSG : BSG_REGEN;
  const uint32_t nsg = (nproofs + SG - 1) / SG;
  uint32_t nsl = 1;
  const uint32_t ctb0 = c->P.logq / 8;
  const bool slabs_ok = !c->mm_image && c->batch_image && nproofs > BG && (((uint64_t)n * ctb0) & 7) == 0;
  if (slabs_ok && c->batch_slabs) nsl = std::min(c->batch_slabs, std::max(1u, std::min(d, m)));
  else if (slabs_ok) {
    size_t mem_free = 0, mem_total = 0;
    if (hipMemGetInfo(&mem_free, &mem_total) == hipSuccess) {
      const size_t ib = mfh_crs_mm_image_bytes(c), avail = mem_free + c->batch_img.cap + c->d_batch.cap;
      if (ib > avail / 4 * 3) {
        const size_t budget = std::max<size_t>(avail / 3, (size_t)1 << 30);
        nsl = (uint32_t)std::min<size_t>(256, (ib + budget - 1) / budget);
        const size_t area = (size_t)3 * BSG * d * 4, maxsg = std::max<size_t>(1, avail / 4 / area);
        if (nsg > maxsg) {
          const size_t ctl0 = (size_t)(n + 1) * ((c->P.logq + 63) / 64);
          for (uint32_t s0 = 0; s0 < nproofs; s0 += (uint32_t)maxsg * SG) {
            const uint32_t cnt = std::min<uint32_t>((uint32_t)maxsg * SG, nproofs - s0);
            const PubBatch sub = pub ? pub->at(s0) : PubBatch{};
            int r = prove_batch_impl(c, d_crs_c8, d_ssp, cnt, h_witness_bits + (size_t)s0 * bits_stride, bits_stride, h_delta + s0,
                                     h_smudge_mag + (size_t)s0 * 5 * maglen, maglen, h_smudge_sign + (size_t)s0 * 5, d_proofs + (size_t)s0 * 5 * ctl0,
                                     pub ? &sub : nullptr);
            if (r) return r;
          }
          c->last_batch_sg = 0;
          return MFH_OK;
        }
      }
    }
  }
  const uint32_t nbuf = nsl > 1 ? nsg : 2;
  while (c->ev_sgdone.size() < nsg) {
    hipEvent_t e;
    HIP_TRY(c, hipEventCreateWithFlags(&e, hipEventDisableTiming));
    c->ev_sgdone.push_back(e);
  }
  c->last_batch_sg = 0;
  BatchScratch B;
  int rc = batch_scratch(c, nproofs, nbuf, B, nsl > 1 ? 1 : nsg, nsl > 1 ? 0 : nproofs);
  if (rc) return rc;
  size_t slot = 0;
  HIP_TRY(c, hipMemsetAsync(B.SCZ, 0, B.nslots * 2048, c->stream));
  rc = batch_streams(c);
  if (rc) return rc;
  while (c->ev_cdone.size() < nbuf) {
    hipEvent_t e0, e1, e2;
    HIP_TRY(c, hipEventCreateWithFlags(&e0, hipEventDisableTiming));
    HIP_TRY(c, hipEventCreateWithFlags(&e1, hipEventDisableTiming));
    HIP_TRY(c, hipEventCreateWithFlags(&e2, hipEventDisableTiming));
    c->ev_cdone.push_back(e0);
    c->ev_rdone.push_back(e1);
    c->ev_wdone.push_back(e2);
  }
  hipStream_t const main_stream = c->stream, chain_stream = c->side2;
  auto whv_of = [&](uint32_t sgi, uint32_t *&W, uint32_t *&H, uint32_t *&V) {
    W = B.WHV + (size_t)(sgi % nbuf) * 3 * BSG * d;
    H = W + (size_t)BSG * d;
    V = H + (size_t)BSG * d;
  };
  auto launch_chain = [&](uint32_t sgi) -> int {
    const uint32_t s0 = sgi * SG, sg = std::min(SG, nproofs - s0);
    uint32_t *WALL, *HALL, *VALL;
    whv_of(sgi, WALL, HALL, VALL);
    OnStream chain(c, chain_stream);
    const PubBatch psg = pub ? pub->at(s0) : PubBatch{};
    int r = batch_chain_launch(c, src, d_ssp, sg, h_witness_bits + (size_t)s0 * bits_stride, bits_stride, h_delta + s0, WALL, HALL, VALL, c->ev_wdone[sgi % nbuf],
                               pub ? &psg : nullptr);
    if (r) return r;
    HIP_TRY(c, hipEventRecord(c->ev_cdone[sgi % nbuf], chain_stream));
    return MFH_OK;
  };
  HIP_TRY(c, hipEventRecord(c->ev_chain, main_stream));
  HIP_TRY(c, hipStreamWaitEvent(chain_stream, c->ev_chain, 0));
  rc = launch_chain(0);
  if (rc) return rc;
  if (nsl > 1) {
    for (uint32_t k = 1; k < nsg; k++) {
      rc = launch_chain(k);
      if (rc) return rc;
    }
    for (;;) {
      size_t ib = 0;
      for (uint32_t r = 0; r < nsl; r++) ib = std::max(ib, mfh_crs_mm_share_bytes(c, r, nsl));
      if (c->batch_img.cap >= ib) break;
      (void)batch_img_drop(c);
      size_t mem_free = 0, mem_total = 0;
      const bool fits = hipMemGetInfo(&mem_free, &mem_total) != hipSuccess || ib + ((size_t)8 << 30) <= mem_free;
      if (fits && dev_alloc(c->batch_img, ib)) break;
      (void)hipGetLastError();
      const uint32_t cap = std::min<uint32_t>(256u, std::max(1u, std::min(d, m)));
      if (nsl >= cap || c->batch_slabs) { c->err = "mfh_prove_batch: no room for a row slab of the CRS image"; return MFH_ENOMEM; }
      nsl = std::min(cap, nsl * 2);
    }
    rc = batch_ct_t(c, d_crs_c8, B);
    if (rc) return rc;
    ImageGuard slab{c, true};
    for (uint32_t r = 0; r < nsl; r++) {
      rc = mfh_crs_expand_mm_share(c, d_crs_c8, r, nsl, c->batch_img.as<uint8_t>());
      if (rc) return rc;
      mfh_crs_set_resident_mm_share(c, c->batch_img.as<uint8_t>(), r, nsl);
      HIP_TRY(c, hipMemsetAsync(B.SCZ, 0, B.nslots * 2048, c->stream));
      slot = 0;
      const uint32_t loS = (uint32_t)((uint64_t)d * r / nsl);
      for (uint32_t s0 = 0, sgi = 0; s0 < nproofs; s0 += SG, sgi++) {
        const uint32_t sg = std::min(SG, nproofs - s0);
        uint32_t *WALL, *HALL, *VALL;
        whv_of(sgi, WALL, HALL, VALL);
        const BatchCoef co = {WALL + loS, HALL + loS, VALL + loS, d};
        rc = batch_rows_supergroup(c, d_crs_c8, r, nsl, sg, h_witness_bits + (size_t)s0 * bits_stride, bits_stride, co, d_proofs + (size_t)s0 * 5 * ctl, B, slot,
                                   r == 0 ? h_delta + s0 : nullptr, r == 0 ? c->ev_cdone[sgi % nbuf] : nullptr, r > 0);
        if (rc) return rc;
      }
    }
    for (uint32_t s0 = 0; s0 < nproofs; s0 += SG) {
      rc = batch_smudge(c, d_proofs + (size_t)s0 * 5 * ctl, std::min(SG, nproofs - s0), h_smudge_mag + (size_t)s0 * 5 * maglen, maglen, h_smudge_sign + (size_t)s0 * 5);
      if (rc) return rc;
      HIP_TRY(c, hipEventRecord(c->ev_sgdone[s0 / SG], c->stream));
    }
    c->last_batch_sg = SG;
    c->last_batch_n = nproofs;
    return MFH_OK;
  }
  ImageGuard transient{c, false};
  rc = batch_transient_image(c, d_crs_c8, nproofs, 0, 1, transient);
  if (rc) return rc;
  rc = batch_stage_host(c, B, nproofs, h_witness_bits, bits_stride, h_delta, h_smudge_mag, maglen, h_smudge_sign, SG);
  if (rc) return rc;
  rc = batch_ct_t(c, d_crs_c8, B);
  if (rc) return rc;
  bool bw_done = false;
  if (c->batch_bw_merged && nsg > 1 && mm_image_covers(c, (uint64_t)ctb0 * n * 2 * d, m)) {
    const uint64_t ctr_ct = (uint64_t)ctb0 * n, pstride = 5 * ctl;
    const uint32_t bstride = (m + 6) / 8;
    const MmRegion reg = {ctr_ct * 2 * d, d_crs_c8 + (size_t)2 * d * ctb0};
    for (uint32_t g0 = 0; g0 < nsg; g0 += 8) {
      MmIo ios[8];
      uint32_t nvs[8];
      const uint32_t ng = std::min(8u, nsg - g0);
      for (uint32_t k = 0; k < ng; k++) {
        const uint32_t sgi = g0 + k, s0 = sgi * SG, sg = std::min(SG, nproofs - s0);
        const uint8_t *d_cw = B.CW + (size_t)sgi * B.cw_stride;
        ios[k] = MmIo{{nullptr, nullptr}, sg, {d_proofs + (size_t)s0 * 5 * ctl + 4 * ctl, nullptr}, sg, pstride, d_cw, bstride, B.SCZ + 256 * slot++};
        ios[k].add_ct = B.CT_T;
        ios[k].add_scale = (const uint32_t *)(d_cw + B.cw_delta_off);
        nvs[k] = sg;
      }
      rc = ng > 1 ? eval_rows_multi_io_regions(c, &reg, 1, m, ios, nvs, ng, 1, 0) : eval_rows_multi_io(c, reg.off, m, reg.c8, ios[0], nvs[0], 1, 0);
      if (rc) return rc;
    }
    bw_done = true;
  }
  const bool early = c->batch_early_chain && bw_done;
  bool any_on_side = false;
  for (uint32_t s0 = 0, sgi = 0; s0 < nproofs; s0 += SG, sgi++) {
    const uint32_t sg = std::min(SG, nproofs - s0);
    uint64_t *sproofs = d_proofs + (size_t)s0 * 5 * ctl;
    uint32_t *WALL, *HALL, *VALL;
    whv_of(sgi, WALL, HALL, VALL);
    const BatchCoef co = {WALL, HALL, VALL, d};
    if (early && sgi + 1 < nsg) {
      if (sgi >= 1) HIP_TRY(c, hipStreamWaitEvent(chain_stream, c->ev_rdone[(sgi - 1) % nbuf], 0));
      rc = launch_chain(sgi + 1);
      if (rc) return rc;
    }
    if (early && sgi >= 2) HIP_TRY(c, hipStreamWaitEvent(main_stream, c->ev_sgdone[sgi - 2], 0));
    HIP_TRY(c, hipStreamWaitEvent(main_stream, c->ev_wdone[sgi % nbuf], 0));
    bool on_side = false;
    rc = batch_rows_supergroup(c, d_crs_c8, 0, 1, sg, h_witness_bits + (size_t)s0 * bits_stride, bits_stride, co, sproofs, B, slot, h_delta + s0,
                               c->ev_cdone[sgi % nbuf], 0, B.CW + (size_t)sgi * B.cw_stride, bw_done, sgi, early ? &on_side : nullptr);
    if (rc) return rc;
    if (early) HIP_TRY(c, hipEventRecord(c->ev_rdone[sgi % nbuf], main_stream));
    else if (sgi + 1 < nsg) {
      HIP_TRY(c, hipEventRecord(c->ev_rdone[sgi % nbuf], main_stream));
      HIP_TRY(c, hipStreamWaitEvent(chain_stream, c->ev_rdone[sgi % nbuf], 0));
      rc = launch_chain(sgi + 1);
      if (rc) return rc;
    }
    {
      OnStream tail(c, on_side ? c->side : main_stream);
      rc = batch_smudge_staged(c, B, sproofs, s0, sg);
      if (rc) return rc;
      HIP_TRY(c, hipEventRecord(c->ev_sgdone[sgi], c->stream));
    }
    any_on_side = any_on_side || on_side;
  }
  if (any_on_side) {
    HIP_TRY(c, hipEventRecord(c->ev_join, c->side));
    HIP_TRY(c, hipStreamWaitEvent(main_stream, c->ev_join, 0));
  }
  c->last_batch_sg = SG;
  c->last_batch_n = nproofs;
  return MFH_OK;
}

}

extern "C" {

int mfh_prove_batch(mfh_ctx *c, const uint8_t *d_crs_c8, const uint32_t *d_ssp, uint32_t nproofs, const uint8_t *h_witness_bits,
                    size_t bits_stride, const uint32_t *h_delta, const uint8_t *h_smudge_mag, size_t maglen, const uint8_t *h_smudge_sign,
                    uint64_t *d_proofs) {
  return prove_batch_impl(c, d_crs_c8, d_ssp, nproofs, h_witness_bits, bits_stride, h_delta, h_smudge_mag, maglen, h_smudge_sign, d_proofs, nullptr);
}

int mfh_prove_batch_public(mfh_ctx *c, const uint8_t *d_crs_c8, const uint32_t *d_ssp, uint32_t lu, uint32_t nproofs, const uint8_t *h_bits,
                           size_t bits_stride, const uint32_t *h_delta, const uint8_t *h_smudge_mag, size_t maglen, const uint8_t *h_smudge_sign,
                           uint64_t *d_proofs) {
  if (!c) return MFH_EINVAL;
  if (lu >= c->P.m) { c->err = "lu must be < m (the m - 1 wires of the SSP)"; return MFH_EINVAL; }
  if (!lu) return mfh_prove_batch(c, d_crs_c8, d_ssp, nproofs, h_bits, bits_stride, h_delta, h_smudge_mag, maglen, h_smudge_sign, d_proofs);
  if (!nproofs) return MFH_OK;
  if (!h_bits) return MFH_EINVAL;
  const uint32_t m = c->P.m, bstride = (m + 6) / 8, ub = (lu + 7) / 8;
  if (bits_stride < bstride) { c->err = "bits_stride shorter than the m - 1 witness bits"; return MFH_EINVAL; }
  std::vector<uint8_t> priv((size_t)nproofs * bstride), pubb;
  std::vector<uint32_t> zero;
  for (uint32_t b = 0; b < nproofs; b++) {
    uint8_t *x = priv.data() + (size_t)b * bstride;
    memcpy(x, h_bits + (size_t)b * bits_stride, bstride);
    memset(x, 0, lu >> 3);
    if (lu & 7) x[lu >> 3] &= (uint8_t)(0xffu << (lu & 7));
  }
  if (lu > kPubDirect) {
    pubb.assign((size_t)nproofs * bstride, 0);
    zero.assign(nproofs, 0);
    for (uint32_t b = 0; b < nproofs; b++) {
      uint8_t *x = pubb.data() + (size_t)b * bstride;
      memcpy(x, h_bits + (size_t)b * bits_stride, ub);
      if (lu & 7) x[ub - 1] &= (uint8_t)((1u << (lu & 7)) - 1);
    }
  }
  HIP_TRY(c, hipSetDevice(c->device));
  const size_t need = (size_t)nproofs * ub;
  if (int rc = dev_reserve(c, c->d_pub, need, DevWait::device)) return rc;
  uint8_t *st = (uint8_t *)pin_acquire(c, c->pin_pub, need);
  if (!st) return MFH_ENOMEM;
  for (uint32_t b = 0; b < nproofs; b++) memcpy(st + (size_t)b * ub, h_bits + (size_t)b * bits_stride, ub);
  HIP_TRY(c, hipMemcpyAsync(c->d_pub.p, st, need, hipMemcpyHostToDevice, c->stream));
  pin_release(c, c->pin_pub);
  const PubBatch pb{lu, c->d_pub.as<uint8_t>(), ub, lu > kPubDirect ? pubb.data() : nullptr, bstride, lu > kPubDirect ? zero.data() : nullptr};
  return prove_batch_impl(c, d_crs_c8, d_ssp, nproofs, priv.data(), bstride, h_delta, h_smudge_mag, maglen, h_smudge_sign, d_proofs, &pb);
}

uint32_t mfh_prove_batch_supergroup(const mfh_ctx *c) { return c ? c->last_batch_sg : 0; }

int mfh_prove_batch_stream_wait(mfh_ctx *c, uint32_t upto, void *hip_stream) {
  if (!c) return MFH_EINVAL;
  if (!c->last_batch_sg || !upto || upto > c->last_batch_n) { c->err = "mfh_prove_batch_stream_wait: no such statements in the last mfh_prove_batch call"; return MFH_EINVAL; }
  HIP_TRY(c, hipStreamWaitEvent((hipStream_t)hip_stream, c->ev_sgdone[(upto - 1) / c->last_batch_sg], 0));
  return MFH_OK;
}

int mfh_batch_chain(mfh_ctx *c, const uint32_t *d_ssp, uint32_t nstmt, const uint8_t *h_witness_bits, size_t bits_stride, const uint32_t *h_delta,
                    uint32_t *d_w, uint32_t *d_h, uint32_t *d_v) {
  if (!c) return MFH_EINVAL;
  if (!nstmt) return MFH_OK;
  if (!h_witness_bits || !h_delta || !d_w || !d_h || !d_v) return MFH_EINVAL;
  mf::SspSrc src;
  int rc = ssp_src(c, d_ssp, src, true);
  if (rc) return rc;
  const uint32_t d = c->P.d, m = c->P.m;
  if (bits_stride < (m + 6) / 8) { c->err = "bits_stride shorter than the m - 1 witness bits"; return MFH_EINVAL; }
  for (uint32_t b = 0; b < nstmt; b++)
    if (h_delta[b] >= P32) { c->err = "delta must be < p"; return MFH_EINVAL; }
  HIP_TRY(c, hipSetDevice(c->device));
  for (uint32_t s0 = 0; s0 < nstmt; s0 += BSG) {
    const size_t o = (size_t)s0 * d;
    rc = batch_chain_launch(c, src, d_ssp, std::min(BSG, nstmt - s0), h_witness_bits + (size_t)s0 * bits_stride, bits_stride, h_delta + s0, d_w + o, d_h + o,
                            d_v + o);
    if (rc) return rc;
  }
  return MFH_OK;
}

int mfh_batch_witness_cols(mfh_ctx *c, const uint32_t *d_ssp, uint32_t nstmt, const uint8_t *h_witness_bits, size_t bits_stride, const uint32_t *h_delta,
                           uint32_t col0, uint32_t ncols, uint32_t *d_w, size_t w_stride) {
  if (!c) return MFH_EINVAL;
  if (!nstmt || !ncols) return MFH_OK;
  if (!h_witness_bits || !h_delta || !d_w) return MFH_EINVAL;
// ... 121 lines not shown
```

### include/mfhip.h

```cpp
#pragma once
#include <stddef.h>
#include <stdint.h>

#ifdef __cplusplus
extern "C" {
#endif

#define MFH_P 0xfffffffbu

enum {
  MFH_OK = 0,
  MFH_EINVAL = -1,
  MFH_EDEVICE = -2,
  MFH_ENOMEM = -3,
  MFH_EUNSUPPORTED = -4
};

typedef struct {
  uint32_t n;
  uint32_t logq;
  uint32_t d;
  uint32_t m;
} mfh_params;

typedef struct mfh_ctx mfh_ctx;

int mfh_ctx_create(mfh_ctx **out, int device, const mfh_params *P);
void mfh_ctx_destroy(mfh_ctx *ctx);
int mfh_set_stream(mfh_ctx *ctx, void *hip_stream);
int mfh_sync(mfh_ctx *ctx);
int mfh_scrub_staging(mfh_ctx *ctx);
const char *mfh_last_error(const mfh_ctx *ctx);
int mfh_set_seed(mfh_ctx *ctx, const uint8_t h_seed[40]);

int mfh_keystream(mfh_ctx *ctx, uint64_t off, void *d_out, size_t nbytes);
int mfh_sample_rows(mfh_ctx *ctx, uint64_t off, size_t nrows, uint64_t *d_out);

int mfh_ct_add(mfh_ctx *ctx, uint64_t *d_rop, const uint64_t *d_a, const uint64_t *d_b, size_t count);
int mfh_ct_mul_ui(mfh_ctx *ctx, uint64_t *d_rop, const uint64_t *d_a, uint32_t b, size_t count);
int mfh_ct_addmul_ui(mfh_ctx *ctx, uint64_t *d_rop, const uint64_t *d_a, uint32_t b, size_t count);

int mfh_eval_rows(mfh_ctx *ctx, uint64_t off, size_t nrows, const uint8_t *d_c8, const uint32_t *d_coeff0,
                  const uint32_t *d_coeff1, uint64_t *d_rop0, uint64_t *d_rop1, int accumulate);

size_t mfh_resident_row_bytes(const mfh_ctx *ctx);
int mfh_crs_expand(mfh_ctx *ctx, uint64_t off, size_t nrows, const uint8_t *d_c8, void *d_rows_out);
int mfh_crs_image_set_b(mfh_ctx *ctx, size_t first_row, size_t nrows, const uint8_t *d_c8, void *d_rows);
int mfh_eval_rows_resident(mfh_ctx *ctx, const void *d_rows, size_t first_row, size_t nrows, const uint32_t *d_coeff0,
                           const uint32_t *d_coeff1, uint64_t *d_rop0, uint64_t *d_rop1, int accumulate);
int mfh_crs_set_resident(mfh_ctx *ctx, const void *d_rows);
int mfh_crs_set_resident_prefix(mfh_ctx *ctx, const void *d_rows, size_t nrows_resident);
size_t mfh_resident_share_rows(const mfh_ctx *ctx, uint32_t rank, uint32_t world);
int mfh_crs_expand_share(mfh_ctx *ctx, const uint8_t *d_crs_c8, uint32_t rank, uint32_t world, void *d_image);
int mfh_crs_set_resident_share(mfh_ctx *ctx, const void *d_image, uint32_t rank, uint32_t world);

int mfh_encrypt_rows(mfh_ctx *ctx, uint64_t off, size_t nrows, const uint64_t *d_sk, const uint32_t *d_msg,
                     const uint64_t *d_err, uint8_t *d_c8_out);
int mfh_set_encrypt_path(mfh_ctx *ctx, int path);

int mfh_decrypt(mfh_ctx *ctx, const uint64_t *d_sk, const uint64_t *d_cts, size_t count, uint32_t *d_out);
int mfh_set_decrypt_path(mfh_ctx *ctx, int path);
int mfh_decrypt_rows(mfh_ctx *ctx, uint64_t off, size_t nrows, const uint64_t *d_sk, const uint8_t *d_c8, uint32_t *d_out);

int mfh_add_dotp(mfh_ctx *ctx, uint64_t *d_rop, const uint64_t *d_a, const uint64_t *d_b, size_t len);

int mfh_ct_smudge(mfh_ctx *ctx, uint64_t *d_cts, size_t count, const uint8_t *h_mag, size_t maglen, const uint8_t *h_sign);

int mfh_ssp_upload(mfh_ctx *ctx, const void *h_ssp_u64, uint32_t *d_ssp, size_t first_slot, size_t nslots);
int mfh_witness_poly(mfh_ctx *ctx, const uint32_t *d_ssp, const uint8_t *h_witness_bits, uint32_t delta, uint32_t *d_w);

int mfh_ssp_set_prg(mfh_ctx *ctx, uint64_t seed, const uint32_t *d_t);
int mfh_ssp_prg_make_t(mfh_ctx *ctx, uint64_t seed, const uint8_t *h_witness_bits, uint32_t *d_t);
int mfh_ssp_prg_fill(mfh_ctx *ctx, uint64_t seed, size_t first_slot, size_t nslots, uint32_t *d_out);

int mfh_ssp_from_rows(mfh_ctx *ctx, uint32_t nrows, const uint32_t *h_row_ptr, const uint32_t *h_wire, const uint32_t *h_coef, uint32_t *d_ssp);

int mfh_ssp_set_rows(mfh_ctx *ctx, uint32_t nrows, const uint32_t *h_row_ptr, const uint32_t *h_wire, const uint32_t *h_coef, uint32_t lu_max);
int mfh_ssp_rows_fill(mfh_ctx *ctx, size_t first_slot, size_t nslots, uint32_t *d_out);

#define MFH_GATE_XOR 0u
#define MFH_GATE_AND 1u
#define MFH_GATE_OR 2u
#define MFH_GATE_NOT 3u
#define MFH_GATE_MAJ 4u
#define MFH_GATE_SUM3 5u
#define MFH_GATE_CONST0 6u
#define MFH_GATE_CONST1 7u
#define MFH_GATE_WSUM 8u
#define MFH_GATE_WSUM_BIT 9u
#define MFH_GATE_LUT2(tt) (16u + (tt))
#define MFH_CIRCUIT_MAX_WIRES 32767u
#define MFH_CIRCUIT_GLOBAL 1u
typedef struct mfh_circuit mfh_circuit;
int mfh_circuit_create(mfh_ctx *ctx, uint32_t nin, uint32_t ngates, const uint32_t *h_gates, uint32_t nasserts, const uint32_t *h_asserts,
                       mfh_circuit **out);
int mfh_circuit_create_global(mfh_ctx *ctx, uint32_t nin, uint32_t ngates, const uint32_t *h_gates, uint32_t nasserts, const uint32_t *h_asserts,
                              mfh_circuit **out);
int mfh_circuit_create_ex(mfh_ctx *ctx, uint32_t nin, uint32_t ngates, const uint32_t *h_gates, uint32_t nasserts, const uint32_t *h_asserts,
                          uint32_t nequal, const uint32_t *h_equal, uint32_t flags, mfh_circuit **out);
int mfh_circuit_create_out(mfh_ctx *ctx, uint32_t nin, uint32_t ngates, const uint32_t *h_gates, uint32_t nasserts, const uint32_t *h_asserts,
                           uint32_t nequal, const uint32_t *h_equal, uint32_t nout, const uint32_t *h_outputs, uint32_t flags, mfh_circuit **out);
int mfh_circuit_create_sum(mfh_ctx *ctx, uint32_t nin, uint32_t ngates, const uint32_t *h_gates, uint32_t nasserts, const uint32_t *h_asserts,
                           uint32_t nequal, const uint32_t *h_equal, uint32_t nout, const uint32_t *h_outputs, uint32_t nterms_total,
                           const uint32_t *h_terms, uint32_t flags, mfh_circuit **out);
void mfh_circuit_destroy(mfh_circuit *c);
int mfh_circuit_assign(mfh_ctx *ctx, const mfh_circuit *c, uint32_t nstmt, const uint8_t *h_inputs, size_t in_stride, uint8_t *h_witness_bits,
                       size_t bits_stride, uint8_t *h_holds);

int mfh_poly_mul(mfh_ctx *ctx, const uint32_t *d_a, size_t la, const uint32_t *d_b, size_t lb, uint32_t *d_c);
int mfh_poly_add(mfh_ctx *ctx, const uint32_t *d_a, const uint32_t *d_b, size_t count, uint32_t *d_out);
int mfh_poly_prepare_t(mfh_ctx *ctx, const uint32_t *d_t);
int mfh_ssp_prepare(mfh_ctx *ctx, const uint32_t *d_ssp);
int mfh_poly_h(mfh_ctx *ctx, const uint32_t *d_v, uint32_t *d_h);
int mfh_poly_h_multi(mfh_ctx *ctx, const uint32_t *d_v, uint32_t *d_h, uint32_t nb);
int mfh_set_poly_exact(mfh_ctx *ctx, int mode);
long mfh_poly_exact_fallbacks(mfh_ctx *ctx);
int mfh_poly_exact_points(mfh_ctx *ctx, uint32_t *out);
int mfh_set_poly_exact_points(mfh_ctx *ctx, const uint32_t *pts);

int mfh_setup_messages(mfh_ctx *ctx, const uint32_t *d_ssp, uint32_t alpha, uint32_t beta, uint32_t s, uint32_t *d_msg);
int mfh_setup(mfh_ctx *ctx, const uint32_t *d_ssp, uint32_t alpha, uint32_t beta, uint32_t s, const uint64_t *d_sk,
              const uint64_t *d_err, uint8_t *d_crs_c8);
int mfh_setup_image(mfh_ctx *ctx, const uint32_t *d_ssp, uint32_t alpha, uint32_t beta, uint32_t s, const uint64_t *d_sk,
                    const uint64_t *d_err, uint8_t *d_crs_c8, void *d_rows_image);
int mfh_prove(mfh_ctx *ctx, const uint8_t *d_crs_c8, const uint32_t *d_ssp, const uint8_t *h_witness_bits, uint32_t delta,
              const uint8_t *h_smudge_mag, size_t maglen, const uint8_t *h_smudge_sign, uint64_t *d_proof);

int mfh_verify(mfh_ctx *ctx, const uint32_t *d_ssp, uint32_t alpha, uint32_t beta, uint32_t s, const uint64_t *d_sk,
               const uint64_t *d_proofs, size_t count, uint8_t *d_ok);

int mfh_setup_public(mfh_ctx *ctx, const uint32_t *d_ssp, uint32_t alpha, uint32_t beta, uint32_t s, uint32_t lu, const uint64_t *d_sk,
                     const uint64_t *d_err, uint8_t *d_crs_c8, void *d_rows_image);
int mfh_prove_public(mfh_ctx *ctx, const uint8_t *d_crs_c8, const uint32_t *d_ssp, uint32_t lu, const uint8_t *h_bits, uint32_t delta,
                     const uint8_t *h_smudge_mag, size_t maglen, const uint8_t *h_smudge_sign, uint64_t *d_proof);
int mfh_prove_batch_public(mfh_ctx *ctx, const uint8_t *d_crs_c8, const uint32_t *d_ssp, uint32_t lu, uint32_t nproofs, const uint8_t *h_bits,
                           size_t bits_stride, const uint32_t *h_delta, const uint8_t *h_smudge_mag, size_t maglen, const uint8_t *h_smudge_sign,
                           uint64_t *d_proofs);
int mfh_vk_derive(mfh_ctx *ctx, const uint32_t *d_ssp, uint32_t s, uint32_t lu, uint32_t *d_vk);
int mfh_verify_public(mfh_ctx *ctx, const uint32_t *d_vk, uint32_t lu, uint32_t alpha, uint32_t beta, const uint64_t *d_sk, const uint64_t *d_proofs,
                      const uint8_t *h_statements, size_t stmt_stride, size_t count, uint8_t *d_ok);

size_t mfh_crs_mm_image_bytes(const mfh_ctx *ctx);
int mfh_crs_expand_mm(mfh_ctx *ctx, const uint8_t *d_crs_c8, uint8_t *d_image);
int mfh_crs_set_resident_mm(mfh_ctx *ctx, const uint8_t *d_image);
int mfh_set_expand_path(mfh_ctx *ctx, int path);
int mfh_set_batch_image(mfh_ctx *ctx, int enabled);
int mfh_set_batch_slabs(mfh_ctx *ctx, uint32_t nslabs);
int mfh_set_encrypt_chunks(mfh_ctx *ctx, uint32_t chunks);
int mfh_set_eval_path(mfh_ctx *ctx, int path);
int mfh_set_witness_per(mfh_ctx *ctx, uint32_t statements);
int mfh_set_batch_launch(mfh_ctx *ctx, uint32_t groups_per_launch, int merge_regions);
int mfh_set_batch_bw(mfh_ctx *ctx, int merged);
int mfh_set_mm_stream(mfh_ctx *ctx, int map, int persistent, int sync_mode, uint32_t spin_max);
int mfh_set_mm_width(mfh_ctx *ctx, uint32_t per_xcd, int early_chain);
int mfh_set_mm_chunk_rows(mfh_ctx *ctx, uint32_t rows);
int mfh_set_mm_pack(mfh_ctx *ctx, int on);
int mfh_prove_batch(mfh_ctx *ctx, const uint8_t *d_crs_c8, const uint32_t *d_ssp, uint32_t nproofs, const uint8_t *h_witness_bits,
                    size_t bits_stride, const uint32_t *h_delta, const uint8_t *h_smudge_mag, size_t maglen, const uint8_t *h_smudge_sign,
                    uint64_t *d_proofs);
uint32_t mfh_prove_batch_supergroup(const mfh_ctx *ctx);
int mfh_prove_batch_stream_wait(mfh_ctx *ctx, uint32_t upto, void *hip_stream);
size_t mfh_crs_mm_share_bytes(const mfh_ctx *ctx, uint32_t rank, uint32_t world);
int mfh_crs_expand_mm_share(mfh_ctx *ctx, const uint8_t *d_crs_c8, uint32_t rank, uint32_t world, uint8_t *d_image);
int mfh_crs_set_resident_mm_share(mfh_ctx *ctx, const uint8_t *d_image, uint32_t rank, uint32_t world);
int mfh_batch_chain(mfh_ctx *ctx, const uint32_t *d_ssp, uint32_t nstmt, const uint8_t *h_witness_bits, size_t bits_stride, const uint32_t *h_delta,
                    uint32_t *d_w, uint32_t *d_h, uint32_t *d_v);
int mfh_batch_witness_cols(mfh_ctx *ctx, const uint32_t *d_ssp, uint32_t nstmt, const uint8_t *h_witness_bits, size_t bits_stride, const uint32_t *h_delta,
                           uint32_t col0, uint32_t ncols, uint32_t *d_w, size_t w_stride);
int mfh_batch_chain_from_w(mfh_ctx *ctx, const uint32_t *d_ssp, uint32_t nstmt, const uint32_t *d_w, uint32_t *d_h, uint32_t *d_v);
int mfh_prove_batch_partial(mfh_ctx *ctx, const uint8_t *d_crs_c8, uint32_t rank, uint32_t world, uint32_t nstmt, const uint8_t *h_witness_bits,
                            size_t bits_stride, const uint32_t *d_w, const uint32_t *d_h, const uint32_t *d_v, size_t coef_stride, uint64_t *d_partial);
int mfh_prove_batch_finish(mfh_ctx *ctx, const uint8_t *d_crs_c8, uint32_t nstmt, const uint32_t *h_delta, const uint8_t *h_smudge_mag, size_t maglen,
                           const uint8_t *h_smudge_sign, uint64_t *d_proofs);

int mfh_prove_partial(mfh_ctx *ctx, const uint8_t *d_crs_c8, const uint32_t *d_ssp, const uint8_t *h_witness_bits, uint32_t delta,
                      uint32_t rank, uint32_t world, uint64_t *d_partial);
int mfh_prove_finish(mfh_ctx *ctx, uint64_t *d_proof, const uint8_t *h_smudge_mag, size_t maglen, const uint8_t *h_smudge_sign);
int mfh_witness_poly_multi(mfh_ctx *ctx, const uint32_t *d_ssp, uint32_t nstmt, const uint8_t *h_bits, size_t bits_stride, const uint32_t *h_delta,
                           uint32_t *d_w);
int mfh_witness_poly_mm(mfh_ctx *ctx, const uint32_t *d_ssp, uint32_t nstmt, const uint8_t *h_bits, size_t bits_stride, const uint32_t *h_delta,
                        uint32_t *d_w);
int mfh_witness_poly_mm_cols(mfh_ctx *ctx, const uint32_t *d_ssp, uint32_t nstmt, const uint8_t *h_bits, size_t bits_stride, const uint32_t *h_delta,
                             uint32_t col0, uint32_t ncols, uint32_t *d_w, size_t w_stride);
int mfh_witness_lanes(mfh_ctx *ctx, const uint32_t *d_ssp, const uint8_t *h_witness_bits, uint32_t rank, uint32_t world, uint64_t *d_lanes);
int mfh_witness_from_lanes(mfh_ctx *ctx, const uint32_t *d_ssp, const uint64_t *d_lanes, uint32_t delta, uint32_t *d_w);
int mfh_prove_partial_w(mfh_ctx *ctx, const uint8_t *d_crs_c8, const uint32_t *d_ssp, const uint8_t *h_witness_bits, uint32_t delta,
                        uint32_t rank, uint32_t world, const uint64_t *d_wlanes, uint64_t *d_partial);
uint32_t mfh_lanes_per_value(const mfh_ctx *ctx);
int mfh_ct_to_lanes(mfh_ctx *ctx, const uint64_t *d_cts, size_t count, uint64_t *d_lanes);
int mfh_ct_from_lanes(mfh_ctx *ctx, const uint64_t *d_lanes, size_t count, uint64_t *d_cts);

const char *mfh_version(void);
int mfh_digest128(mfh_ctx *ctx, const void *d_buf, size_t nbytes, uint64_t h_digest[2]);
size_t mfh_workspace_bytes(const mfh_ctx *ctx);
int mfh_eval_rows_multi(mfh_ctx *ctx, uint64_t off, size_t nrows, const uint8_t *d_c8, const uint32_t *d_coeffs, uint32_t nvec,
                        uint32_t coeff_bytes, uint64_t *d_rops, int accumulate);

int mfh_set_timing(mfh_ctx *ctx, int enabled);
int mfh_set_overlap(mfh_ctx *ctx, int mode);
int mfh_timing_drain(mfh_ctx *ctx, const char *which, uint64_t *count, double *total_ms, uint64_t *total_rows, float *last_ms);
float mfh_last_kernel_ms(mfh_ctx *ctx, const char *which);
double mfh_timing_busy_ms(const mfh_ctx *ctx);
uint64_t mfh_timing_work_rows(const mfh_ctx *ctx);

#ifdef __cplusplus
}
#endif
```

Baseline: 13760.

## Merge per-supergroup witness passes into one grouped matrix-core launch

Adds a batched witness path that stages all witness bits and deltas to the device once. It computes bit counts for all supergroups in a single kernel and runs one k_witness_mm8q launch whose grid covers every supergroup, instead of one witness pass per supergroup inside each chain. The host smudge staging is split into a separate later copy, and the witness buffers are kept for all supergroups at once. This cuts per-group launch and sync overhead and widens the grid, at the cost of more device memory, which is checked against free memory, and extra event ordering between the streams.

Result: no change. 13830, median of 6 (+0.5%).

```diff
diff --git a/c-lwe-snarks_amd/__init__.py b/c-lwe-snarks_amd/__init__.py
--- a/c-lwe-snarks_amd/__init__.py
+++ b/c-lwe-snarks_amd/__init__.py
@@ -80,7 +80,7 @@
     "mfh_encrypt_rows", "mfh_decrypt", "mfh_ct_smudge", "mfh_ssp_upload", "mfh_witness_poly", "mfh_version",
     "mfh_workspace_bytes", "mfh_last_kernel_ms", "mfh_set_timing", "mfh_set_overlap", "mfh_eval_rows_multi", "mfh_prove_batch", "mfh_crs_mm_image_bytes", "mfh_crs_expand_mm", "mfh_crs_set_resident_mm", "mfh_witness_poly_multi", "mfh_witness_poly_mm", "mfh_poly_h_multi", "mfh_poly_mul", "mfh_poly_add", "mfh_poly_prepare_t",
     "mfh_ssp_prepare", "mfh_poly_h", "mfh_setup_messages", "mfh_setup", "mfh_setup_image", "mfh_crs_image_set_b", "mfh_prove",
-    "mfh_prove_partial", "mfh_prove_finish", "mfh_ct_to_lanes", "mfh_ct_from_lanes", "mfh_lanes_per_value", "mfh_digest128", "mfh_timing_drain", "mfh_timing_busy_ms", "mfh_timing_work_rows", "mfh_set_batch_image", "mfh_set_batch_slabs", "mfh_set_expand_path", "mfh_set_encrypt_path", "mfh_set_batch_launch", "mfh_set_batch_bw", "mfh_set_mm_chunk_rows", "mfh_set_mm_pack", "mfh_set_poly_exact", "mfh_poly_exact_fallbacks", "mfh_poly_exact_points", "mfh_set_poly_exact_points", "mfh_set_mm_stream", "mfh_add_dotp", "mfh_set_encrypt_chunks", "mfh_set_witness_per", "mfh_set_eval_path", "mfh_set_decrypt_path", "mfh_decrypt_rows",
+    "mfh_prove_partial", "mfh_prove_finish", "mfh_ct_to_lanes", "mfh_ct_from_lanes", "mfh_lanes_per_value", "mfh_digest128", "mfh_timing_drain", "mfh_timing_busy_ms", "mfh_timing_work_rows", "mfh_set_batch_image", "mfh_set_batch_slabs", "mfh_set_expand_path", "mfh_set_encrypt_path", "mfh_set_batch_launch", "mfh_set_batch_bw", "mfh_set_batch_witness_merged", "mfh_set_batch_witness_areas", "mfh_set_mm_chunk_rows", "mfh_set_mm_pack", "mfh_set_poly_exact", "mfh_poly_exact_fallbacks", "mfh_poly_exact_points", "mfh_set_poly_exact_points", "mfh_set_mm_stream", "mfh_add_dotp", "mfh_set_encrypt_chunks", "mfh_set_witness_per", "mfh_set_eval_path", "mfh_set_decrypt_path", "mfh_decrypt_rows",
     "mfh_crs_mm_share_bytes", "mfh_crs_expand_mm_share", "mfh_crs_set_resident_mm_share", "mfh_batch_chain", "mfh_batch_witness_cols", "mfh_batch_chain_from_w", "mfh_witness_poly_mm_cols", "mfh_prove_batch_partial", "mfh_prove_batch_finish",
     "mfh_resident_row_bytes", "mfh_crs_expand", "mfh_eval_rows_resident", "mfh_crs_set_resident",
     "mfh_witness_lanes", "mfh_witness_from_lanes", "mfh_prove_partial_w", "mfh_verify",
@@ -183,6 +183,8 @@
         "mfh_set_mm_stream": (i32, [vp, i32, i32, i32, u32]),
         "mfh_set_batch_launch": (i32, [vp, u32, i32]),
         "mfh_set_batch_bw": (i32, [vp, i32]),
+        "mfh_set_batch_witness_merged": (i32, [vp, i32]),
+        "mfh_set_batch_witness_areas": (i32, [vp, u32]),
         "mfh_set_encrypt_path": (i32, [vp, i32]),
         "mfh_set_expand_path": (i32, [vp, i32]),
         "mfh_set_batch_slabs": (i32, [vp, u32]),
@@ -355,6 +357,10 @@
     def set_batch_bw(self, merged=True):
         self._chk(self.lib.mfh_set_batch_bw(self._h, 1 if merged else 0))
 
+    def set_batch_witness_merged(self, merged=True, max_areas=0):
+        self._chk(self.lib.mfh_set_batch_witness_merged(self._h, 1 if merged else 0))
+        self._chk(self.lib.mfh_set_batch_witness_areas(self._h, int(max_areas)))
+
     def set_mm_stream(self, map=0, persistent=False, sync_mode=0, spin_max=64):
         self._chk(self.lib.mfh_set_mm_stream(self._h, int(map), int(persistent), int(sync_mode), int(spin_max)))
 
diff --git a/c-lwe-snarks_amd/csrc/ctx.hpp b/c-lwe-snarks_amd/csrc/ctx.hpp
--- a/c-lwe-snarks_amd/csrc/ctx.hpp
+++ b/c-lwe-snarks_amd/csrc/ctx.hpp
@@ -116,6 +116,8 @@
   uint32_t witness_per = 0;
   uint32_t batch_slabs = 0;
   int batch_bw_merged = 1;
+  int batch_witness_merged = 1;
+  uint32_t batch_witness_areas = 0;
   int batch_merge = 1;
   uint32_t batch_ngl = 8;
   PinBuf pin_rows, pin_cw, pin_smudge;
@@ -270,6 +272,9 @@
                                    uint32_t *d_w);
 extern "C" int mfh_witness_poly_mm_cols(mfh_ctx *c, const uint32_t *d_ssp, uint32_t nstmt, const uint8_t *h_bits, size_t bits_stride, const uint32_t *h_delta,
                                         uint32_t col0, uint32_t ncols, uint32_t *d_w, size_t w_stride);
+bool witness_groups_ok(mfh_ctx *c, const uint32_t *d_ssp);
+int witness_poly_mm_groups(mfh_ctx *c, const uint32_t *d_ssp, uint32_t nsg, uint32_t per, uint32_t total, const uint8_t *d_cw, size_t cw_stride,
+                           size_t delta_off, uint32_t *d_w, size_t w_area_stride);
 extern "C" int mfh_poly_h_multi(mfh_ctx *c, const uint32_t *d_v, uint32_t *d_h, uint32_t nb);
 int expand_mm_region(mfh_ctx *c, uint64_t off, uint32_t nrows, const uint8_t *c8, uint8_t *image);
 int encrypt_rows_mm(mfh_ctx *c, uint64_t off, size_t nrows, const uint64_t *sk, const uint32_t *msg, const uint64_t *err, uint8_t *c8);
diff --git a/c-lwe-snarks_amd/csrc/evalmm.hip b/c-lwe-snarks_amd/csrc/evalmm.hip
--- a/c-lwe-snarks_amd/csrc/evalmm.hip
+++ b/c-lwe-snarks_amd/csrc/evalmm.hip
@@ -954,6 +954,11 @@
   uint32_t KS;
   uint64_t wstride;
 };
+struct WGroups {
+  uint32_t nsg;
+  uint32_t per, total;
+  uint64_t frag_stride , cd_stride , w_stride ;
+};
 template <int MT>
 __global__ __launch_bounds__(256) void k_witness_mm(const v4i *__restrict__ sspfrag, const v4i *__restrict__ bitfrag, uint32_t nrowsel ,
                                                     uint32_t ksteps_per_chunk, uint32_t d, int *__restrict__ part, WCols wc) {
@@ -1205,14 +1210,31 @@
 }
 __global__ __launch_bounds__(512) void k_witness_mm8q(const v4i *__restrict__ sspfrag, const v4i *__restrict__ bitfrag, uint32_t nrowsel ,
                                                       uint32_t ksteps_per_chunk, uint32_t d, int *__restrict__ part, const uint32_t *__restrict__ tpoly ,
-                                                      const uint32_t *__restrict__ cnt_delta, uint32_t nstmt, uint32_t *__restrict__ w_out, WCols wc) {
+                                                      const uint32_t *__restrict__ cnt_delta, uint32_t nstmt, uint32_t *__restrict__ w_out, WCols wc, WGroups G) {
   constexpr int MT = 8, RING = 4, PF = 4;
   __shared__ v4i bits[RING][MT][64];
   __shared__ uint32_t xch[2][3][16][64];
   const uint32_t tid = threadIdx.x, lane = tid & 63, wave = tid >> 6;
   const uint32_t r32 = lane & 31, h = lane >> 5;
   const uint32_t tile = wave >> 2, pl = wave & 3;
-  const uint32_t ktl = blockIdx.x * 2 + tile, kt = wc.kt0 + ktl;
+  uint32_t bx = blockIdx.x;
+  if (G.nsg > 1) {
+    const uint32_t npair = gridDim.x / G.nsg;
+    uint32_t sgi;
+    if (npair % 8 == 0) {
+      const uint32_t y = bx >> 3;
+      sgi = y % G.nsg;
+      bx = (y / G.nsg) * 8 + (bx & 7);
+    } else {
+      sgi = bx % G.nsg;
+      bx /= G.nsg;
+    }
+    bitfrag += sgi * G.frag_stride;
+    cnt_delta += sgi * G.cd_stride;
+    w_out += sgi * G.w_stride;
+    nstmt = min(G.per, G.total - sgi * G.per);
+  }
+  const uint32_t ktl = bx * 2 + tile, kt = wc.kt0 + ktl;
   const uint32_t K0 = blockIdx.y * ksteps_per_chunk, K1 = min((nrowsel + 31) / 32, K0 + ksteps_per_chunk);
   v16i acc[MT];
 #pragma unroll
@@ -1347,6 +1369,25 @@
   }
   const uint64_t P = MFH_P;
   w_out[(uint64_t)b * wstride + k] = (uint32_t)((val % P + (uint64_t)t[k] * delta % P) % P);
+}
+__global__ void k_witness_cnt(const uint8_t *__restrict__ cw, size_t cw_stride, size_t delta_off, uint32_t bstride, uint32_t nrowsel, uint32_t per, uint32_t total,
+                              uint32_t *__restrict__ cd, size_t cd_stride) {
+  const uint32_t b = blockIdx.x, g = blockIdx.y, lane = threadIdx.x;
+  if ((uint64_t)g * per + b >= total) return;
+  const uint8_t *area = cw + (size_t)g * cw_stride, *bits = area + (size_t)b * bstride;
+  const uint32_t nb = (nrowsel + 7) / 8;
+  uint32_t cnt = 0;
+  for (uint32_t i = lane; i < nb; i += 64) {
+    uint32_t x = bits[i];
+    if (i == nb - 1 && (nrowsel & 7)) x &= (1u << (nrowsel & 7)) - 1;
+    cnt += __popc(x);
+  }
+#pragma unroll
+  for (int o = 32; o; o >>= 1) cnt += __shfl_xor(cnt, o);
+  if (lane == 0) {
+    cd[(size_t)g * cd_stride + 2 * b] = cnt;
+    cd[(size_t)g * cd_stride + 2 * b + 1] = reinterpret_cast<const uint32_t *>(area + delta_off)[b];
+  }
 }
 
 }
@@ -1728,6 +1769,18 @@
 }
 int mfh_crs_set_resident_mm(mfh_ctx *c, const uint8_t *d_image) { return mfh_crs_set_resident_mm_share(c, d_image, 0, 1); }
 
+static int ssp_frag_ensure(mfh_ctx *c, const uint32_t *d_ssp) {
+  const uint32_t d = c->P.d, nrowsel = c->P.m - 1, ksteps = (nrowsel + 31) / 32;
+  const size_t sfrag_b = (size_t)ksteps * 32 * d * 4;
+  if (c->ssp_frag_src == d_ssp && c->ssp_frag.cap >= sfrag_b) return MFH_OK;
+  if (int rc0 = dev_reserve(c, c->ssp_frag, sfrag_b)) return rc0;
+  const uint64_t nthreads = (uint64_t)ksteps * (d / 32) * 256;
+  hipLaunchKernelGGL(k_ssp_frag, dim3((uint32_t)((nthreads + 255) / 256)), dim3(256), 0, c->stream, d_ssp, nrowsel, d, c->ssp_frag.as<uint32_t>());
+  HIP_TRY(c, hipGetLastError());
+  c->ssp_frag_src = d_ssp;
+  return MFH_OK;
+}
+
 int mfh_witness_poly_mm_cols(mfh_ctx *c, const uint32_t *d_ssp, uint32_t nstmt, const uint8_t *h_bits, size_t bits_stride, const uint32_t *h_delta,
                              uint32_t col0, uint32_t ncols, uint32_t *d_w, size_t w_stride) {
   if (!c || !h_bits || !h_delta || !d_w || nstmt == 0 || nstmt > 256) return MFH_EINVAL;
@@ -1751,14 +1804,8 @@
   const uint32_t nrowsel = m - 1, ksteps = (nrowsel + 31) / 32;
   const bool fused = MT == 8 && src.dense && m < 65536 && (nc >= 16384 || ksteps <= 64);
   const uint32_t nchunks = fused ? 1u : std::min(ksteps, 4u), kpc = (ksteps + nchunks - 1) / nchunks;
-  const size_t sfrag_b = (size_t)ksteps * 32 * d * 4;
-  if (src.dense && (c->ssp_frag_src != d_ssp || c->ssp_frag.cap < sfrag_b)) {
-    if (int rc0 = dev_reserve(c, c->ssp_frag, sfrag_b)) return rc0;
-    const uint64_t nthreads = (uint64_t)ksteps * (d / 32) * 256;
-    hipLaunchKernelGGL(k_ssp_frag, dim3((uint32_t)((nthreads + 255) / 256)), dim3(256), 0, c->stream, d_ssp, nrowsel, d, c->ssp_frag.as<uint32_t>());
-    HIP_TRY(c, hipGetLastError());
-    c->ssp_frag_src = d_ssp;
-  }
+  if (src.dense)
+    if (int rc0 = ssp_frag_ensure(c, d_ssp)) return rc0;
   const size_t packed = (size_t)nstmt * bits_stride, head_b = ((packed + 8 + 256 * 8 + 255) & ~(size_t)255);
   const size_t frag_b = (size_t)ksteps * MT * 1024, part_b = (size_t)nchunks * 4 * 32 * MT * nc * 4;
   const size_t rk_b = src.dense ? 0 : (((size_t)ksteps * 32 * 4 + 255) & ~(size_t)255);
@@ -1795,7 +1842,7 @@
     else hipLaunchKernelGGL(k_witness_mm_prg<4>, grid, dim3(256), 0, c->stream, d_rk, (const v4i *)d_frag, nrowsel, kpc, nc, d_part, wc);
   } else if (MT == 8) {
     hipLaunchKernelGGL(k_witness_mm8q, dim3(nc / 64, (ksteps + kpc - 1) / kpc), dim3(512), 0, c->stream, c->ssp_frag.as<const v4i>(), (const v4i *)d_frag, nrowsel, kpc, nc,
-                       fused ? (int *)nullptr : d_part, tpoly, d_cd, nstmt, d_w, wc);
+                       fused ? (int *)nullptr : d_part, tpoly, d_cd, nstmt, d_w, wc, WGroups{1, 0, 0, 0, 0, 0});
     if (fused) {
       HIP_TRY(c, hipGetLastError());
       return MFH_OK;
@@ -1815,6 +1862,39 @@
   return MFH_OK;
 }
 
+}
+
+bool witness_groups_ok(mfh_ctx *c, const uint32_t *d_ssp) {
+  return d_ssp && !ssp_is_rows(c, d_ssp) && c->P.d % 128 == 0 && c->P.m >= 2 && c->P.m < 65536;
+}
+int witness_poly_mm_groups(mfh_ctx *c, const uint32_t *d_ssp, uint32_t nsg, uint32_t per, uint32_t total, const uint8_t *d_cw, size_t cw_stride,
+                           size_t delta_off, uint32_t *d_w, size_t w_area_stride) {
+  if (!c || !d_cw || !d_w || nsg < 2 || per == 0 || per > 256 || (uint64_t)(nsg - 1) * per >= total || (uint64_t)nsg * per < total) return MFH_EINVAL;
+  if (!witness_groups_ok(c, d_ssp)) return MFH_EUNSUPPORTED;
+  mf::SspSrc src;
+  if (int rc0 = ssp_src(c, d_ssp, src)) return rc0;
+  const uint32_t d = c->P.d, nrowsel = c->P.m - 1, ksteps = (nrowsel + 31) / 32, MT = 8;
+  HIP_TRY(c, hipSetDevice(c->device));
+  if (int rc0 = ssp_frag_ensure(c, d_ssp)) return rc0;
+  const size_t cd_b = 256 * 8, frag_b = (size_t)ksteps * MT * 1024;
+  if (int rc = wws_reserve(c, (size_t)nsg * (cd_b + frag_b))) return rc;
+  uint32_t *d_cd = c->wws.as<uint32_t>();
+  int8_t *d_frag = c->wws.as<int8_t>() + (size_t)nsg * cd_b;
+  const uint32_t bstride = (nrowsel + 7) / 8;
+  hipLaunchKernelGGL(k_witness_cnt, dim3(per, nsg), dim3(64), 0, c->stream, d_cw, cw_stride, delta_off, bstride, nrowsel, per, total, d_cd, cd_b / 4);
+  for (uint32_t g = 0; g < nsg; g++)
+    hipLaunchKernelGGL(k_witness_bits, dim3((uint32_t)((frag_b / 16 + 255) / 256)), dim3(256), 0, c->stream, d_cw + (size_t)g * cw_stride, (size_t)bstride,
+                       std::min(per, total - g * per), nrowsel, ksteps, MT, d_frag + (size_t)g * frag_b);
+  const WCols wc = {0, ksteps, (uint64_t)d};
+  const WGroups G = {nsg, per, total, (uint64_t)(frag_b / 16), (uint64_t)(cd_b / 4), (uint64_t)w_area_stride};
+  hipLaunchKernelGGL(k_witness_mm8q, dim3(d / 64 * nsg, 1), dim3(512), 0, c->stream, c->ssp_frag.as<const v4i>(), (const v4i *)d_frag, nrowsel, ksteps, d, (int *)nullptr,
+                     src.t, d_cd, 0u, d_w, wc, G);
+  HIP_TRY(c, hipGetLastError());
+  return MFH_OK;
+}
+
+extern "C" {
+
 int mfh_witness_poly_mm(mfh_ctx *c, const uint32_t *d_ssp, uint32_t nstmt, const uint8_t *h_bits, size_t bits_stride, const uint32_t *h_delta,
                         uint32_t *d_w) {
   if (!c) return MFH_EINVAL;
diff --git a/c-lwe-snarks_amd/csrc/mfhip.hip b/c-lwe-snarks_amd/csrc/mfhip.hip
--- a/c-lwe-snarks_amd/csrc/mfhip.hip
+++ b/c-lwe-snarks_amd/csrc/mfhip.hip
@@ -1100,6 +1100,17 @@
   return MFH_OK;
 }
 
+int mfh_set_batch_witness_merged(mfh_ctx *c, int merged) {
+  if (!c) return MFH_EINVAL;
+  c->batch_witness_merged = merged != 0;
+  return MFH_OK;
+}
+int mfh_set_batch_witness_areas(mfh_ctx *c, uint32_t max_areas) {
+  if (!c) return MFH_EINVAL;
+  c->batch_witness_areas = max_areas;
+  return MFH_OK;
+}
+
 int mfh_set_batch_image(mfh_ctx *c, int en) {
   if (!c) return MFH_EINVAL;
   c->batch_image = en != 0;
diff --git a/c-lwe-snarks_amd/csrc/snark.hip b/c-lwe-snarks_amd/csrc/snark.hip
--- a/c-lwe-snarks_amd/csrc/snark.hip
+++ b/c-lwe-snarks_amd/csrc/snark.hip
@@ -561,21 +561,28 @@
   B.SCZ = (int64_t *)(base + whv_b + cw_pad * ncw + sm_b + 256 + ctl * 8);
   return MFH_OK;
 }
+enum class Stage { All, Witness, Smudge };
 int batch_stage_host(mfh_ctx *c, const BatchScratch &B, uint32_t nproofs, const uint8_t *h_bits, size_t bits_stride, const uint32_t *h_delta,
-                     const uint8_t *h_mag, size_t maglen, const uint8_t *h_sign, uint32_t SG) {
+                     const uint8_t *h_mag, size_t maglen, const uint8_t *h_sign, uint32_t SG, Stage part = Stage::All) {
   const uint32_t m = c->P.m, nsg = (nproofs + SG - 1) / SG;
   const uint32_t bstride = (m + 6) / 8, KW = 2 * (c->P.logq / 64);
   if (maglen + 4 > (size_t)KW * 4) { c->err = "smudge magnitude too wide"; return MFH_EINVAL; }
-  const size_t total = (size_t)((uint8_t *)B.SMS - B.CW) + (size_t)nproofs * 5;
-  uint8_t *st = (uint8_t *)pin_acquire(c, c->pin_cw, total);
+  const size_t total = (size_t)((uint8_t *)B.SMS - B.CW) + (size_t)nproofs * 5, smu_off = (size_t)((uint8_t *)B.SMU - B.CW);
+  uint8_t *st = part == Stage::Smudge ? (uint8_t *)c->pin_cw.p : (uint8_t *)pin_acquire(c, c->pin_cw, total);
   if (!st) return MFH_ENOMEM;
-  for (uint32_t g = 0; g < nsg; g++) {
-    const uint32_t s0 = g * SG, sg = std::min(SG, nproofs - s0);
-    uint8_t *a = st + (size_t)g * B.cw_stride;
-    for (uint32_t b = 0; b < sg; b++) memcpy(a + (size_t)b * bstride, h_bits + (size_t)(s0 + b) * bits_stride, bstride);
-    memcpy(a + B.cw_delta_off, h_delta + s0, (size_t)sg * 4);
-  }
-  uint32_t *up = (uint32_t *)(st + ((uint8_t *)B.SMU - B.CW));
+  if (part != Stage::Smudge)
+    for (uint32_t g = 0; g < nsg; g++) {
+      const uint32_t s0 = g * SG, sg = std::min(SG, nproofs - s0);
+      uint8_t *a = st + (size_t)g * B.cw_stride;
+      for (uint32_t b = 0; b < sg; b++) memcpy(a + (size_t)b * bstride, h_bits + (size_t)(s0 + b) * bits_stride, bstride);
+      memcpy(a + B.cw_delta_off, h_delta + s0, (size_t)sg * 4);
+    }
+  if (part == Stage::Witness) {
+    HIP_TRY(c, hipMemcpyAsync(B.CW, st, smu_off, hipMemcpyHostToDevice, c->stream));
+    pin_release(c, c->pin_cw);
+    return MFH_OK;
+  }
+  uint32_t *up = (uint32_t *)(st + smu_off);
   for (size_t i = 0; i < (size_t)nproofs * 5; i++) {
     uint64_t carry = 0;
     for (uint32_t l = 0; l < KW; l++) {
@@ -588,7 +595,8 @@
     }
   }
   memcpy(st + ((uint8_t *)B.SMS - B.CW), h_sign, (size_t)nproofs * 5);
-  HIP_TRY(c, hipMemcpyAsync(B.CW, st, total, hipMemcpyHostToDevice, c->stream));
+  if (part == Stage::Smudge) HIP_TRY(c, hipMemcpyAsync(B.SMU, st + smu_off, total - smu_off, hipMemcpyHostToDevice, c->stream));
+  else HIP_TRY(c, hipMemcpyAsync(B.CW, st, total, hipMemcpyHostToDevice, c->stream));
   pin_release(c, c->pin_cw);
   return MFH_OK;
 }
@@ -658,7 +666,8 @@
 };
 
 int batch_chain_launch(mfh_ctx *c, const mf::SspSrc &src, const uint32_t *d_ssp, uint32_t sg, const uint8_t *h_bits, size_t bits_stride,
-                       const uint32_t *h_delta, uint32_t *W, uint32_t *H, uint32_t *V, hipEvent_t ev_witness = nullptr, const PubBatch *pub = nullptr) {
+                       const uint32_t *h_delta, uint32_t *W, uint32_t *H, uint32_t *V, hipEvent_t ev_witness = nullptr, const PubBatch *pub = nullptr,
+                       bool have_w = false ) {
   const uint32_t d = c->P.d;
   int rc = MFH_OK;
   auto witness_pass = [&](const uint8_t *bits, size_t stride, const uint32_t *delta, uint32_t *out) -> int {
@@ -676,7 +685,7 @@
     }
     return MFH_OK;
   };
-  rc = witness_pass(h_bits, bits_stride, h_delta, W);
+  if (!have_w) rc = witness_pass(h_bits, bits_stride, h_delta, W);
   if (rc) return rc;
   const bool pub_pass = pub && pub->lu > kPubDirect;
   if (pub_pass) {
@@ -948,7 +957,17 @@
       }
     }
   }
-  const uint32_t nbuf = nsl > 1 ? nsg : 2;
+  bool wmerged = nsl == 1 && c->batch_witness_merged && will_stream && nsg > 1 && !pub && !c->witness_per && witness_groups_ok(c, d_ssp);
+  if (wmerged) {
+    size_t max_areas = c->batch_witness_areas;
+    if (!max_areas) {
+      size_t mem_free = 0, mem_total = 0;
+      if (hipMemGetInfo(&mem_free, &mem_total) != hipSuccess) mem_free = 0;
+      max_areas = (mem_free + c->d_batch.cap) / 4 / ((size_t)3 * BSG * d * 4);
+    }
+    wmerged = nsg <= max_areas;
+  }
+  const uint32_t nbuf = nsl > 1 || wmerged ? nsg : 2;
   while (c->ev_sgdone.size() < nsg) {
     hipEvent_t e;
     HIP_TRY(c, hipEventCreateWithFlags(&e, hipEventDisableTiming));
@@ -984,13 +1003,21 @@
     OnStream chain(c, chain_stream);
     const PubBatch psg = pub ? pub->at(s0) : PubBatch{};
     int r = batch_chain_launch(c, src, d_ssp, sg, h_witness_bits + (size_t)s0 * bits_stride, bits_stride, h_delta + s0, WALL, HALL, VALL, c->ev_wdone[sgi % nbuf],
-                               pub ? &psg : nullptr);
+                               pub ? &psg : nullptr, wmerged);
     if (r) return r;
     HIP_TRY(c, hipEventRecord(c->ev_cdone[sgi % nbuf], chain_stream));
     return MFH_OK;
   };
   HIP_TRY(c, hipEventRecord(c->ev_chain, main_stream));
   HIP_TRY(c, hipStreamWaitEvent(chain_stream, c->ev_chain, 0));
+  if (wmerged) {
+    OnStream chain(c, chain_stream);
+    rc = batch_stage_host(c, B, nproofs, h_witness_bits, bits_stride, h_delta, h_smudge_mag, maglen, h_smudge_sign, SG, Stage::Witness);
+    if (rc) return rc;
+    HIP_TRY(c, hipEventRecord(c->ev_chain_done, chain_stream));
+    rc = witness_poly_mm_groups(c, d_ssp, nsg, SG, nproofs, B.CW, B.cw_stride, B.cw_delta_off, B.WHV, (size_t)3 * BSG * d);
+    if (rc) return rc;
+  }
   rc = launch_chain(0);
   if (rc) return rc;
   if (nsl > 1) {
@@ -1043,7 +1070,8 @@
   ImageGuard transient{c, false};
   rc = batch_transient_image(c, d_crs_c8, nproofs, 0, 1, transient);
   if (rc) return rc;
-  rc = batch_stage_host(c, B, nproofs, h_witness_bits, bits_stride, h_delta, h_smudge_mag, maglen, h_smudge_sign, SG);
+  if (wmerged) HIP_TRY(c, hipStreamWaitEvent(main_stream, c->ev_chain_done, 0));
+  rc = batch_stage_host(c, B, nproofs, h_witness_bits, bits_stride, h_delta, h_smudge_mag, maglen, h_smudge_sign, SG, wmerged ? Stage::Smudge : Stage::All);
   if (rc) return rc;
   rc = batch_ct_t(c, d_crs_c8, B);
   if (rc) return rc;
diff --git a/include/mfhip.h b/include/mfhip.h
--- a/include/mfhip.h
+++ b/include/mfhip.h
@@ -151,6 +151,8 @@
 int mfh_set_witness_per(mfh_ctx *ctx, uint32_t statements);
 int mfh_set_batch_launch(mfh_ctx *ctx, uint32_t groups_per_launch, int merge_regions);
 int mfh_set_batch_bw(mfh_ctx *ctx, int merged);
+int mfh_set_batch_witness_merged(mfh_ctx *ctx, int merged);
+int mfh_set_batch_witness_areas(mfh_ctx *ctx, uint32_t max_areas);
 int mfh_set_mm_stream(mfh_ctx *ctx, int map, int persistent, int sync_mode, uint32_t spin_max);
 int mfh_set_mm_width(mfh_ctx *ctx, uint32_t per_xcd, int early_chain);
 int mfh_set_mm_chunk_rows(mfh_ctx *ctx, uint32_t rows);
```
